# ariasanovsky/azdopt

Measured on AMD Instinct MI355X. Metric: node_expansions_per_s, higher is better.
Workload: dtype f32

## Files before the change

azdopt_amd/__init__.py:

```python
from ._lib import ACT_NONE, ACT_RELU, ACT_SIGMOID, AzdError, build, lib
from .model import ActionModel, HashStreamModel, NablaModel, TrivialModel
from .optimizer import ArgminData, DenseAhArgminData, DenseArgminData, DenseInvArgminData, DenseInvsArgminData, DenseInvxArgminData, NablaOptimizer, RamseyArgminData, TreeView, tree_capacities
from . import sinks
from .space import Layered
from .space import DenseGraphSpace, InvariantCost, InvariantCostS, InvariantCostX
from .space import ActionMultiset, ActionOrderIndependent, ActionSequence, ActionSet, OrderedActionSet, ActionsNeverRepeat, RamseySpaceNoEdgeRecolor, ROTModifyParentsOnce


def device_count():
    return lib().azd_device_count()
```

azdopt_amd/_lib.py:

```python
import ctypes as C
import os
import subprocess

_HERE = os.path.dirname(os.path.abspath(__file__))
LIB_PATH = os.environ.get("AZD_LIB", os.path.join(_HERE, "libazdopt_amd.so"))
_LIB = None

CTR = dict(EXPANSIONS=0, TERMINALS=1, TRANSPOSITIONS=2, VISITED_STEPS=3, SELECT_CALLS=4, SUM_DEG=5,
           SUM_ACTIONS=6, CASCADE_NODES=7, NEW_PREDS=8, ROOT_EXHAUSTED=9, MAX_FRONTIER=10, MAX_DEPTH=11,
           CURIOSITY_PAIRS=12, EVAL_LAYER_CLOCKS=13, TICKS_ADD_ACTIONS=14, FAILED=15, TICKS_TOTAL=16, TICKS_SELECT=17, TICKS_LOOKUP=18, TICKS_NEWNODE=19,
           TICKS_CASCADE=20, TICKS_MAX_CALL=21, TICKS_LAMBDA=22, TICKS_MATCHING=23, TICKS_WAIT=24, EVAL_BATCHES=25, EVAL_ROWS=26, EVAL_TILES=27, TICKS_TILES=28, TICKS_BATCH=29, TICKS_TILE_SETUP=30, TICKS_TILE_KLOOP=31)
CTR_COUNT = 32

ACT_NONE, ACT_RELU, ACT_SIGMOID = 0, 1, 2
ENGINE_NO_PERSISTENT_STEP = 1
ENGINE_ASYNC_STEP = 2
ENGINE_BARRIER_STEP = 4
ENGINE_POOL_STEP = 8
ENGINE_DENSE_AH = 32
ENGINE_RAMSEY_U64 = 16
ENGINE_EXT_POOL_STEP = 64
ENGINE_DENSE_AH_WIDE = 256
ENGINE_EXT_POOL_F32 = 128
ENGINE_DENSE_INV = 1024
# ... 192 lines not shown
    sig("azd_device_count", C.c_int)
    sig("azd_c21_state_dim", C.c_int, C.c_int)
    sig("azd_c21_action_dim", C.c_int, C.c_int)
    sig("azd_c21_key_words", C.c_int, C.c_int)
    sig("azd_c21_generate_roots", C.c_int, C.c_uint64, C.c_uint64, C.c_uint64, C.c_int, C.c_int, C.c_int, C.c_int, vp, vp)
    sig("azd_evaluator_create_mlp", C.c_int, C.POINTER(vp), C.c_int, C.c_int, C.c_int, C.c_int, vp, C.c_int, C.c_int,
        C.POINTER(AdamConfig), C.c_uint64)
    sig("azd_evaluator_create_trivial", C.c_int, C.POINTER(vp), C.c_int, C.c_int, C.c_int)
    sig("azd_evaluator_create_hash_stream", C.c_int, C.POINTER(vp), C.c_int, C.c_int, C.c_int, C.c_uint64, C.c_uint64)
    sig("azd_evaluator_destroy", C.c_int, vp)
    sig("azd_evaluator_write_predictions", C.c_int, vp, C.c_int, vp, vp)
    sig("azd_evaluator_update_model", C.c_int, vp, C.c_int, vp, vp, vp, f32p)
    sig("azd_evaluator_write_predictions_dev", C.c_int, vp, C.c_int, vp, vp, vp)
    sig("azd_evaluator_update_model_dev", C.c_int, vp, C.c_int, vp, vp, vp, f32p, vp)
    sig("azd_evaluator_set_weight_storage", C.c_int, vp, C.c_int)
    sig("azd_evaluator_num_params", C.c_int64, vp)
    sig("azd_evaluator_get_params", C.c_int, vp, vp)
    sig("azd_evaluator_set_params", C.c_int, vp, vp)
    sig("azd_evaluator_calls", C.c_uint64, vp)
    sig("azd_engine_create", C.c_int, C.POINTER(vp), C.POINTER(EngineConfig), vp)
    sig("azd_engine_destroy", C.c_int, vp)
    sig("azd_engine_par_new", C.c_int, vp, vp, vp)
    sig("azd_engine_par_roll_out_episodes", C.c_int, vp, vp, C.c_int, C.c_uint32, C.c_int, i32p)
    sig("azd_engine_run_ahead", C.c_int, vp, vp, C.c_int, C.c_uint32, C.c_int, i32p)
    sig("azd_engine_par_update_model", C.c_int, vp, C.c_uint32, f32p)
    sig("azd_engine_par_update_model_sharded", C.c_int, vp, C.c_uint32, vp, f32p)
    sig("azd_engine_par_reset_trees", C.c_int, vp, vp, vp)
    sig("azd_engine_argmin_data", C.c_int, vp, C.POINTER(Argmin))
    sig("azd_engine_agent_counters", C.c_int, vp, vp)
    sig("azd_engine_agent_counters_per_agent", C.c_int, vp)
    sig("azd_engine_pool_agent_finish", C.c_int, vp, vp)
    sig("azd_engine_pool_groups", C.c_int, vp, vp, vp, vp)
    sig("azd_engine_ramsey_argmin_data", C.c_int, vp, C.POINTER(RamseyArgmin))
    sig("azd_engine_ramsey_wide_argmin_data", C.c_int, vp, C.POINTER(RamseyWideArgmin))
    sig("azd_engine_ramsey_argmin_any", C.c_int, vp, vp, C.c_int, vp, C.c_int, vp, f32p, i32p, C.POINTER(C.c_uint32))
    sig("azd_engine_ramsey_agent_counts", C.c_int, vp, C.c_int, vp, vp)
    sig("azd_ramsey_state_dim", C.c_int, C.c_int, C.c_int)
    sig("azd_ramsey_action_dim", C.c_int, C.c_int, C.c_int)
    sig("azd_ramsey_key_words", C.c_int, C.c_int, C.c_int)
    sig("azd_ramsey_generate_roots", C.c_int, C.c_uint64, C.c_uint64, C.c_uint64, C.c_int, C.c_int, C.c_int, C.c_int,
        C.c_int, vp, vp)
    sig("azd_ramsey_generate_roots_weighted", C.c_int, C.c_uint64, C.c_uint64, C.c_uint64, C.c_int, C.c_int, C.c_int, C.c_int,
        C.c_int, vp, vp, vp)
    sig("azd_engine_set_root_policy", C.c_int, vp, C.POINTER(RootPolicy))
    sig("azd_engine_get_root_policy", C.c_int, vp, C.POINTER(RootPolicy))
    sig("azd_root_policy_check", C.c_int, C.c_int, C.c_int, C.POINTER(RootPolicy))
    sig("azd_engine_root_policy_report", C.c_int, vp, vp, vp, vp)
    sig("azd_dense_state_dim", C.c_int, C.c_int)
    sig("azd_dense_action_dim", C.c_int, C.c_int)
    sig("azd_dense_key_words", C.c_int, C.c_int)
    sig("azd_dense_generate_roots", C.c_int, C.c_uint64, C.c_uint64, C.c_uint64, C.c_int, C.c_int, C.c_int, C.c_int, C.c_double, vp, vp)
    sig("azd_engine_dense_argmin_data", C.c_int, vp, C.POINTER(DenseArgmin))
    sig("azd_c21_modify_roots", C.c_int, vp, C.c_uint64, C.c_uint64, C.c_int, C.c_int, vp, vp)
    sig("azd_c21_modify_roots_dev", C.c_int, vp, C.c_uint64, C.c_uint64, C.c_int, C.c_int, vp, vp)
    sig("azd_engine_par_reset_trees_c21", C.c_int, vp, C.c_uint64, C.c_uint64, C.c_int, C.c_int)
    sig("azd_engine_modify_roots_dev", C.c_int, vp, C.c_uint64, C.c_uint64, C.c_int, C.c_int, vp, vp)
    sig("azd_engine_par_reset_trees_policy", C.c_int, vp, C.c_uint64, C.c_uint64, C.c_int, C.c_int)
    sig("azd_engine_par_new_begin", C.c_int, vp, vp, vp)
    sig("azd_engine_par_new_end", C.c_int, vp, vp)
    sig("azd_engine_roll_out_begin", C.c_int, vp, vp, C.c_int, C.c_uint32)
    sig("azd_engine_roll_out_end", C.c_int, vp, vp, i32p)
    sig("azd_engine_reset_begin", C.c_int, vp, vp, vp)
    sig("azd_engine_reset_end", C.c_int, vp, vp)
    sig("azd_engine_observe", C.c_int, vp, C.c_uint32, vp, vp, vp)
    sig("azd_engine_observe_dev", C.c_int, vp, C.c_uint32, C.POINTER(vp), C.POINTER(vp), C.POINTER(vp))
    sig("azd_engine_read_state_vecs", C.c_int, vp, vp)
    sig("azd_engine_read_predictions", C.c_int, vp, vp)
    sig("azd_engine_debug_tile_forward", C.c_int, vp, vp, vp, C.c_int)
    sig("azd_engine_tree_sizes", C.c_int, vp, C.c_int, i32p, i32p, i32p)
    sig("azd_engine_export_tree", C.c_int, vp, C.c_int, *([vp] * 13))
    sig("azd_engine_agent_state", C.c_int, vp, C.c_int, vp, vp, vp, C.POINTER(C.c_uint32), C.POINTER(C.c_double), i32p)
    sig("azd_engine_counters", C.c_int, vp, vp)
    sig("azd_engine_set_timing", C.c_int, vp, C.c_int)
    sig("azd_engine_timing", C.c_int, vp, C.POINTER(C.c_double), C.POINTER(C.c_double), u64p)
    sig("azd_engine_stream", vp, vp)
    sig("azd_engine_step_form", C.c_int, vp, i32p, C.POINTER(C.c_char_p))
    sig("azd_engine_pool_split", C.c_int, vp, i32p, i32p)
    sig("azd_engine_pool_utilisation", C.c_int, vp, C.POINTER(C.c_double), C.POINTER(C.c_double))
    sig("azd_debug_probe_xcc", C.c_int, C.c_int, vp, C.c_int)
    sig("azd_debug_hash_stream_via_evaluators", C.c_int, vp, C.c_int)
    sig("azd_debug_ext_pool_plan", C.c_int, C.POINTER(EngineConfig), i32p, C.POINTER(C.c_size_t))
    sig("azd_debug_mlp_gradients", C.c_int, vp, C.c_int, vp, vp, vp, vp, f32p)
    sig("azd_debug_write_predictions_gathered", C.c_int, vp, C.c_int, vp, C.c_int, vp, C.c_int, vp)
    sig("azd_debug_probe_math", C.c_int, C.c_int, vp, vp, C.c_int)
    sig("azd_debug_gemm_bf16", C.c_int, C.c_int, C.c_int, C.c_int, C.c_int, vp, vp, vp, vp, C.c_int, C.c_int, C.c_int, C.c_int, f32p)
    sig("azd_debug_probe_cost", C.c_int, C.c_int, vp, C.c_int, C.c_int, C.c_int, C.c_int, vp, vp, f32p)
    sig("azd_debug_probe_dense_cost", C.c_int, C.c_int, vp, C.c_int, C.c_int, vp, C.c_int, vp, vp, vp, vp)
    sig("azd_dense_ah_cost", C.c_int, vp, C.c_int, C.POINTER(DenseAhCost))
    sig("azd_engine_dense_ah_argmin_data", C.c_int, vp, C.POINTER(DenseAhArgmin))
    sig("azd_engine_dense_ah_agent_cost", C.c_int, vp, C.c_int, C.POINTER(DenseAhCost))
    sig("azd_debug_probe_ah_cost", C.c_int, C.c_int, vp, C.c_int, C.c_int, C.c_int, vp, f32p)
    sig("azd_dense_ah_cost_wide", C.c_int, vp, C.c_int, C.POINTER(DenseAhCost))
    sig("azd_engine_dense_ah_wide_argmin_data", C.c_int, vp, C.POINTER(DenseAhWideArgmin))
    sig("azd_debug_probe_ah_cost_wide", C.c_int, C.c_int, vp, C.c_int, C.c_int, C.c_int, vp, f32p)
    sig("azd_dense_inv_cost", C.c_int, vp, C.c_int, C.POINTER(DenseInvRecipe), C.POINTER(DenseInvCost))
    sig("azd_debug_probe_inv_cost", C.c_int, C.c_int, vp, C.c_int, C.c_int, C.c_int, C.POINTER(DenseInvRecipe), vp, f32p)
    sig("azd_dense_inv_cost_wide", C.c_int, vp, C.c_int, C.POINTER(DenseInvRecipe), C.POINTER(DenseInvCost))
    sig("azd_debug_probe_inv_cost_wide", C.c_int, C.c_int, vp, C.c_int, C.c_int, C.c_int, C.POINTER(DenseInvRecipe), vp, f32p)
    sig("azd_engine_dense_inv_wide_argmin_data", C.c_int, vp, C.POINTER(DenseInvWideArgmin))
    sig("azd_dense_invx_cost", C.c_int, vp, C.c_int, C.POINTER(DenseInvxRecipe), C.POINTER(DenseInvxCost))
    sig("azd_debug_probe_invx_cost", C.c_int, C.c_int, vp, C.c_int, C.c_int, C.c_int, C.POINTER(DenseInvxRecipe), vp, f32p)
    sig("azd_dense_invx_cost_wide", C.c_int, vp, C.c_int, C.POINTER(DenseInvxRecipe), C.POINTER(DenseInvxCost))
    sig("azd_debug_probe_invx_cost_wide", C.c_int, C.c_int, vp, C.c_int, C.c_int, C.c_int, C.POINTER(DenseInvxRecipe), vp, f32p)
    sig("azd_engine_dense_invx_wide_argmin_data", C.c_int, vp, C.POINTER(DenseInvxWideArgmin))
    sig("azd_engine_set_dense_invx_recipe", C.c_int, vp, C.POINTER(DenseInvxRecipe))
    sig("azd_engine_dense_invx_argmin_data", C.c_int, vp, C.POINTER(DenseInvxArgmin))
    sig("azd_engine_dense_invx_agent_cost", C.c_int, vp, C.c_int, C.POINTER(DenseInvxCost))
    sig("azd_dense_invs_cost", C.c_int, vp, C.c_int, C.POINTER(DenseInvsRecipe), C.POINTER(DenseInvsCost))
    sig("azd_dense_invs_spectrum", C.c_int, vp, C.c_int, C.c_int, vp)
    sig("azd_debug_probe_invs_cost", C.c_int, C.c_int, vp, C.c_int, C.c_int, C.c_int, C.POINTER(DenseInvsRecipe), vp, f32p)
    sig("azd_dense_invs_cost_wide", C.c_int, vp, C.c_int, C.POINTER(DenseInvsRecipe), C.POINTER(DenseInvsCost))
    sig("azd_dense_invs_spectrum_wide", C.c_int, vp, C.c_int, C.c_int, vp)
    sig("azd_debug_probe_invs_cost_wide", C.c_int, C.c_int, vp, C.c_int, C.c_int, C.c_int, C.POINTER(DenseInvsRecipe), vp, f32p)
    sig("azd_engine_dense_invs_wide_argmin_data", C.c_int, vp, C.POINTER(DenseInvsWideArgmin))
    sig("azd_engine_set_dense_invs_recipe", C.c_int, vp, C.POINTER(DenseInvsRecipe))
    sig("azd_engine_dense_invs_argmin_data", C.c_int, vp, C.POINTER(DenseInvsArgmin))
    sig("azd_engine_dense_invs_agent_cost", C.c_int, vp, C.c_int, C.POINTER(DenseInvsCost))
    sig("azd_engine_set_dense_inv_recipe", C.c_int, vp, C.POINTER(DenseInvRecipe))
    sig("azd_engine_dense_inv_argmin_data", C.c_int, vp, C.POINTER(DenseInvArgmin))
    sig("azd_engine_dense_inv_agent_cost", C.c_int, vp, C.c_int, C.POINTER(DenseInvCost))
    sig("azd_debug_probe_math_f64", C.c_int, C.c_int, vp, vp, C.c_int)
    _LIB = L
    return L


def check(status, where):
    if status != 0:
        raise AzdError(status, where)


def ptr(a):
    return a.ctypes.data_as(C.c_void_p)
```

azdopt_amd/csrc/dense_kernels.hip:

```cpp
#include <hip/hip_runtime.h>

#include "bf16.h"
#include "space_ops.h"

namespace azd {

#include "tree_core.inc"
#include "space_dense.inc"

#include "root_policy.inc"

#define AZD_TU_POOL_EXT 1
#define AZD_TU_POOL_SEARCH 1
#include "persistent_step.inc"
#include "async_step.inc"
#include "pool_step.inc"

#include "launchers.inc"

AZD_PHASE_ENTRIES(DISPATCH_DKW)
AZD_DENSE_NO_RESIDENT_ENTRIES
#define DENSE_POOL_LDS "pool step: 16 searcher waves' blocks and scratch do not fit the CU's 160 KB of LDS (more than 640 slots per root)"
AZD_POOL_SEARCH_ENTRIES(DISPATCH_DKW, PERSIST_WAVES, "pool step: more than 65536 agents or nodes per tree", DENSE_POOL_LDS, DENSE_POOL_LDS)
const SpaceOps &dense_ops() {
    static const SpaceOps ops = {{AZD_PHASE_OPS, no_argmin_one, no_resident, nullptr}, {no_resident, nullptr}, {no_pool, nullptr, nullptr},
                                 {AZD_POOL_SEARCH_OPS(PERSIST_WAVES)}};
    return ops;
}

void launch_ext_take(const PoolArgs &pool, uint32_t *rows, uint32_t *home, uint32_t *n, unsigned long long *t0, void *stream) {
    k_ext_take<<<dim3(1), dim3(POOL_XCDS * 64), 0, (hipStream_t)stream>>>(pool, rows, home, n, t0);
}
__global__ void k_park(Arenas a, const uint32_t *__restrict__ resume, const int n_calls, const int round, const int park) {
    const int t = blockIdx.x * blockDim.x + threadIdx.x;
    if (t >= a.B) return;
    uint32_t f = a.flags[t] & ~(uint32_t)FLAG_PARKED;
    if (park) {
        const uint32_t r = resume[t];
        const bool sits_out = round < 0 ? (r >> 31) == 0u : (int)(r & 0x7FFFFFFFu) + round >= n_calls;
        if (sits_out) f |= (uint32_t)FLAG_PARKED;
    }
    a.flags[t] = f;
}
void launch_park(const Arenas &a, const uint32_t *resume, int n_calls, int round, int park, void *stream) {
    k_park<<<dim3((a.B + 255) / 256), dim3(256), 0, (hipStream_t)stream>>>(a, resume, n_calls, round, park);
}
__global__ void k_log_candidates_resume(Arenas a, unsigned long long *__restrict__ log_key, const uint32_t *__restrict__ resume, const int n_calls,
                                        const int round) {
    const int t = blockIdx.x * blockDim.x + threadIdx.x;
    if (t >= a.B) return;
    const uint32_t node = a.cand_node[t];
    const int call = (int)(resume[t] & 0x7FFFFFFFu) + round;
    if (node != NONE && a.flags[t] == 0 && call < n_calls) {
        const unsigned long long key = ((unsigned long long)ordf(a.cand_c[t]) << 32) | ((unsigned long long)((uint32_t)t & 0xFFFFu) << 16) |
                                       (unsigned long long)(node & 0xFFFFu);
        atomicMin(&log_key[call], key);
        a.cand_node[t] = NONE;
    }
}
void launch_log_candidates_resume(const Arenas &a, unsigned long long *log_key, const uint32_t *resume, int n_calls, int round, void *stream) {
    k_log_candidates_resume<<<dim3((a.B + 255) / 256), dim3(256), 0, (hipStream_t)stream>>>(a, log_key, resume, n_calls, round);
}
void launch_ext_hash_rows(const PersistArgs *d_args, const uint32_t *rows, const uint32_t *n, uint32_t cap, float *h_theta, void *stream) {
    k_ext_hash_rows<<<dim3(cap), dim3(256), 0, (hipStream_t)stream>>>(d_args, rows, n, h_theta);
}
void launch_ext_deliver(const PoolArgs &pool, const Arenas &a, const uint32_t *rows, const uint32_t *home, const uint32_t *n, uint32_t cap,
                        const unsigned long long *t0, void *stream) {
    k_ext_deliver<<<dim3((cap + 255) / 256), dim3(256), 0, (hipStream_t)stream>>>(pool, a, rows, home, n, t0);
}
void launch_probe_dense_cost(const uint64_t *d_adj, int n, int count, const uint16_t *d_toggles, int n_toggles, double *d_lam, int *d_mu,
                             uint8_t *d_mate, int *d_hooks, void *stream) {
    k_probe_dense_cost<2><<<dim3(count), dim3(64), 0, (hipStream_t)stream>>>(d_adj, n, count, d_toggles, n_toggles, d_lam, d_mu, d_mate, d_hooks);
}

}
```

azdopt_amd/csrc/engine.hip:

```cpp
#include "engine_impl.h"

namespace azd {
thread_local std::string g_last_error;

int hip_fail(hipError_t e, const char *what) {
    g_last_error = std::string(what) + ": " + hipGetErrorString(e);
    if (e == hipErrorNoDevice || e == hipErrorInvalidDevice) return AZD_ERR_NO_DEVICE;
    if (e == hipErrorOutOfMemory) return AZD_ERR_OUT_OF_MEMORY;
    return AZD_ERR_HIP;
}

int device_ok(int device) {
    int n = 0;
    hipError_t e = hipGetDeviceCount(&n);
    if (e != hipSuccess || n <= 0) {
        g_last_error = "no HIP device visible (this library has no CPU fallback)";
        return AZD_ERR_NO_DEVICE;
    }
    if (device < 0 || device >= n) {
        g_last_error = "device ordinal out of range";
        return AZD_ERR_INVALID_ARGUMENT;
    }
    return AZD_OK;
}
// ... 700 lines not shown
    if (dense) {
        e->dense_slots = 64 * a.KW;
        e->kw_host = azd::dense_key_words(cfg->n);
    } else if (ramsey) {
        e->kw_host = azd::ramsey_key_words(cfg->n, a.C);
        e->ramsey_slots = tier->cap_from_slots ? cfg->max_slots : azd::MAX_NODE_ACTIONS / (a.C - 1);
    }
    if (dense || (cfg->flags & AZD_ENGINE_EXT_POOL_STEP)) e->ext = tier->ext;
    e->ext_f32 = (cfg->flags & AZD_ENGINE_EXT_POOL_F32) != 0;
    if (ev && (ev->state_dim != a.S || ev->action_dim != a.A)) {
        azd::g_last_error = "evaluator dimensions do not match the space";
        return AZD_ERR_INVALID_ARGUMENT;
    }
    static_assert(AZD_RAMSEY_U64_NODE_ACTIONS == 64 * azd::RAMSEY_U64_CH, "node capacity of the 64-bit Ramsey tier");
    static_assert(AZD_DENSE_MAX_SLOTS <= 2047 && azd::MAX_NODE_ACTIONS <= 2047, "actions per node must fit PredRec's 11-bit count");
    static_assert(AZD_MAX_NODE_CAPACITY == 65536 && AZD_MAX_ARC_CAPACITY == 65535 && AZD_MAX_PREDICTION_CAPACITY == (1 << 20), "limits of the packed records");
    {
        const char *bad = nullptr;
        static thread_local char msg[256];
        const long per_node = dense ? (long)e->dense_slots : ramsey ? (long)std::min(a.E, e->ramsey_slots) * (a.C - 1) : (long)a.A;
        if (a.node_cap > (uint32_t)AZD_MAX_NODE_CAPACITY) snprintf(msg, sizeof msg, "node_capacity %u is beyond the record format (<= %d)", a.node_cap, AZD_MAX_NODE_CAPACITY), bad = msg;
        else if (a.arc_cap > (uint32_t)AZD_MAX_ARC_CAPACITY) snprintf(msg, sizeof msg, "arc_capacity %u is beyond the record format (<= %d)", a.arc_cap, AZD_MAX_ARC_CAPACITY), bad = msg;
        else if (a.pred_cap > (uint32_t)AZD_MAX_PREDICTION_CAPACITY) snprintf(msg, sizeof msg, "prediction_capacity %u is beyond the record format (<= %d)", a.pred_cap, AZD_MAX_PREDICTION_CAPACITY), bad = msg;
        else if (a.A > 4096) snprintf(msg, sizeof msg, "ACTION_DIM %d is beyond the record format (<= 4096)", a.A), bad = msg;
        else if (per_node > 2047) snprintf(msg, sizeof msg, "%ld legal actions per node are beyond the record format (<= 2047)", per_node), bad = msg;
        if (bad) {
            azd::g_last_error = bad;
            return AZD_ERR_INVALID_ARGUMENT;
        }
    }
    const size_t B = (size_t)a.B;
    AZD_ST(e->stream.create());
    AZD_ST(e->alloc(&a.nodes, B * a.node_cap));
    AZD_ST(e->alloc(&a.keys, B * a.node_cap * a.KW));
    AZD_ST(e->alloc(&a.arcs, B * a.arc_cap));
    AZD_ST(e->alloc(&a.preds, B * a.pred_cap));
    AZD_ST(e->alloc(&a.pred_g, B * a.pred_cap));
    AZD_ST(e->alloc(&a.ht, B * a.ht_cap));
    AZD_ST(e->alloc(&a.root_parents, B * azd::PARENTS_STRIDE));
    AZD_ST(e->alloc(&a.cur_parents, B * azd::PARENTS_STRIDE));
    AZD_ST(e->alloc(&a.root_perm, B * a.KW));
    AZD_ST(e->alloc(&a.cur_perm, B * a.KW));
    AZD_ST(e->alloc(&a.cur_path, B * a.KW));
    AZD_ST(e->alloc(&a.cur_lambda, (size_t)tier->cost_f64 * B + (size_t)tier->cost_tail_f64));
    AZD_ST(e->alloc(&a.cur_mu, (size_t)tier->cost_i32 * B));
    AZD_ST(e->alloc(&a.state_pos, B));
    AZD_ST(e->alloc(&a.n_nodes, B));
    AZD_ST(e->alloc(&a.n_arcs, B));
    AZD_ST(e->alloc(&a.n_preds, B));
    AZD_ST(e->alloc(&a.flags, B));
    a.fr_lds = (uint32_t)azd::FRONTIER_CAP;
    if (const char *v = getenv("AZD_DEBUG_FRONTIER_LDS")) {
        const int k = atoi(v);
        if (k >= 64 && k <= azd::FRONTIER_CAP && k % 64 == 0) a.fr_lds = (uint32_t)k;
    }
    if (ramsey) AZD_ST(e->alloc(&a.fr_spill, B * 4 * a.node_cap));
    AZD_ST(e->alloc(&a.cand_c, B));
    AZD_ST(e->alloc(&a.cand_node, B));
    AZD_ST(e->alloc(&a.counters, B * azd::NUM_COUNTERS));
    AZD_ST(e->alloc(&a.state_vecs, B * a.S));
    AZD_ST(e->alloc(&a.h_theta, B * a.A));
    a.obs = a.h_theta;
    AZD_ST(e->alloc(&a.weights, B * a.A));
    AZD_ST(e->alloc(&a.argmin, 1));
    AZD_ST(e->alloc(&a.status, 1));
    if (a.layers > 1) AZD_ST(e->alloc(&a.cur_seq, B * azd::MAX_NODE_ACTIONS));
    AZD_ST(e->alloc(&a.cur_stack, B * azd::PATH_STACK));
    if (dense) {
        AZD_ST(e->alloc(&a.root_adj, B * 64));
        AZD_ST(e->alloc(&a.cur_adj, B * 64));
        AZD_ST(e->alloc(&a.root_aid, B * (size_t)e->dense_slots));
        AZD_ST(e->alloc(&e->d_stage_slots, B * (size_t)((a.E + 63) / 64)));
        static_assert(sizeof(azd::DenseAhArgminRec) <= sizeof(azd::DenseArgminRec) && sizeof(azd::DenseAhWideArgminRec) <= sizeof(azd::DenseArgminRec) &&
                          sizeof(azd::DenseInvArgminRec) <= sizeof(azd::DenseArgminRec) && sizeof(azd::DenseInvWideArgminRec) <= 2 * sizeof(azd::DenseArgminRec) &&
                          sizeof(azd::DenseInvxArgminRec) <= sizeof(azd::DenseArgminRec) && sizeof(azd::DenseInvxWideArgminRec) <= 2 * sizeof(azd::DenseArgminRec) &&
                          sizeof(azd::DenseInvsArgminRec) <= sizeof(azd::DenseArgminRec) && sizeof(azd::DenseInvsWideArgminRec) <= 2 * sizeof(azd::DenseArgminRec),
                      "an AH or INV engine's argmin record lives in argmin_d's allocation");
        AZD_ST(e->alloc(&a.argmin_d, (tier->argmin_bytes + sizeof(azd::DenseArgminRec) - 1) / sizeof(azd::DenseArgminRec)));
        if (tier->id == TIER_DENSE) AZD_ST(e->alloc(&a.node_mate, B * (size_t)a.node_cap * 64));
        if (ev && ev->input16_pitch() >= a.S) {
            a.S16 = ev->input16_pitch();
            AZD_ST(e->alloc(&a.state_vecs16, B * (size_t)a.S16));
            if (hipMemset(a.state_vecs16, 0, B * (size_t)a.S16 * 2) != hipSuccess) return AZD_ERR_HIP;
        }
    }
    if (ramsey) {
        AZD_ST(e->alloc(&a.root_nbr, B * tier->nbr_words));
        AZD_ST(e->alloc(&a.cur_nbr, B * tier->nbr_words));
        AZD_ST(e->alloc(&a.root_counts, B * (size_t)a.C * a.E));
        AZD_ST(e->alloc(&a.cur_counts, B * (size_t)a.C * a.E));
        AZD_ST(e->alloc(&a.root_tot, B * 4));
        AZD_ST(e->alloc(&a.cur_tot, B * 4));
        AZD_ST(e->alloc(&a.argmin_r, e->argmin_r_recs()));
        if (e->ext && ev && ev->input16_pitch() >= a.S && ev->input16_pitch() % 8 == 0) {
            e->ext_s16_pitch = ev->input16_pitch();
            AZD_ST(e->alloc(&e->ext_s16, B * (size_t)e->ext_s16_pitch));
            if (hipMemset(e->ext_s16, 0, B * (size_t)e->ext_s16_pitch * 2) != hipSuccess) return AZD_ERR_HIP;
        }
    }
    e->persist_enabled = (cfg->flags & AZD_ENGINE_NO_PERSISTENT_STEP) == 0;
    e->barrier_step = (cfg->flags & AZD_ENGINE_BARRIER_STEP) != 0;
    e->graph_enabled = getenv("AZD_NO_CALL_GRAPH") == nullptr;
    e->pool_step = (cfg->flags & AZD_ENGINE_POOL_STEP) != 0 ||
                   ((cfg->flags & (AZD_ENGINE_ASYNC_STEP | AZD_ENGINE_BARRIER_STEP)) == 0 && cfg->batch >= 256);
    if (const char *env = getenv("AZD_STEP_FORM")) {
        if (!strcmp(env, "pool")) e->pool_step = true, e->barrier_step = false;
        else if (!strcmp(env, "async")) e->pool_step = false, e->barrier_step = false;
        else if (!strcmp(env, "barrier")) e->pool_step = false, e->barrier_step = true;
    }
    {
        hipDeviceProp_t prop;
        e->n_cus = hipGetDeviceProperties(&prop, cfg->device) == hipSuccess ? prop.multiProcessorCount : 256;
        uint32_t qcap = 128;
        while (qcap < 2u * (uint32_t)a.B) qcap <<= 1;
        e->pool.qcap = qcap;
        e->pool_slot_words = (size_t)4 * azd::POOL_XCDS * qcap;
        AZD_ST(e->alloc(&e->pool.ctl, 1));
        AZD_ST(e->alloc(&e->pool.ready_slots, e->pool_slot_words));
        e->pool.eval_slots = e->pool.ready_slots + (size_t)2 * azd::POOL_XCDS * qcap;
        AZD_ST(e->alloc(&e->pool.join, B));
        AZD_ST(e->alloc(&e->pool.pend, B));
        AZD_ST(e->alloc(&e->pool.stamp, B));
        AZD_ST(e->alloc(&e->pool.post_call, B));
        AZD_ST(e->alloc(&e->d_resume, B));
        AZD_ST(e->alloc(&e->d_call_ctr, (size_t)azd_engine::MAX_SUBS));
        if (e->ext) {
            AZD_ST(e->alloc(&e->d_ext_rows, B * azd_engine::EXT_STREAMS));
            AZD_ST(e->alloc(&e->d_ext_home, B * azd_engine::EXT_STREAMS));
            AZD_ST(e->alloc(&e->d_ext_n, (size_t)azd_engine::EXT_STREAMS));
            AZD_ST(e->alloc(&e->d_ext_t0, (size_t)azd_engine::EXT_STREAMS));
        }
    }
    e->log_calls = 1024;
    {
        const size_t n_wg = (B + 15) / 16;
        AZD_ST(e->alloc(&e->d_pargs, 1));
        AZD_ST(e->h_pargs.alloc(1));
        AZD_ST(e->alloc(&e->d_log_key, (size_t)e->log_calls * n_wg));
        AZD_ST(e->alloc(&e->d_log_node, (size_t)e->log_calls * n_wg));
        AZD_ST(e->alloc(&e->pool.win_count, (size_t)e->log_calls));
        AZD_ST(e->alloc(&e->d_argmin_side, 1));
        if (ramsey) AZD_ST(e->alloc(&e->d_argmin_r_side, e->argmin_r_recs()));
        AZD_ST(e->h_win_log.alloc((size_t)e->log_calls, hipHostMallocCoherent));
        AZD_ST(e->h_win_flag.alloc((size_t)e->log_calls, hipHostMallocCoherent));
        e->pool.win_log = e->h_win_log;
        e->pool.win_flag = e->h_win_flag;
    }
    AZD_ST(e->alloc(&e->d_stage_parents, B * (size_t)(dense ? 8 * a.n : ramsey ? a.E : a.n)));
    AZD_ST(e->alloc(&e->d_stage_perm, B * (size_t)(dense ? 17 * a.KW : a.KW)));
    if (!dense) e->d_stage_slots = e->d_stage_perm;
    AZD_ST(e->alloc(&e->d_root_report, B * 3));
    e->root_args.report = e->d_root_report;
    AZD_ST(e->h_status.alloc(1));
    AZD_ST(e->root_report.alloc(B * 3));
    AZD_ST(e->h_argmin.alloc(1));
    hipError_t he = hipMemsetAsync(a.counters, 0, B * azd::NUM_COUNTERS * 8, e->stream);
    if (he == hipSuccess) he = hipMemsetAsync(a.status, 0, sizeof(azd::StatusRec), e->stream);
    if (he == hipSuccess) he = hipMemsetAsync(a.argmin, 0, sizeof(azd::ArgminRec), e->stream);
    if (he == hipSuccess) he = hipMemsetAsync(a.flags, 0, B * 4, e->stream);
    if (he == hipSuccess) he = hipMemsetAsync(a.h_theta, 0, B * a.A * 4, e->stream);
    if (he == hipSuccess) he = hipMemsetAsync(a.state_vecs, 0, B * a.S * 4, e->stream);
    if (he == hipSuccess) he = hipMemsetAsync(a.weights, 0, B * a.A * 4, e->stream);
    if (he == hipSuccess && ramsey) he = hipMemsetAsync(a.argmin_r, 0, e->argmin_r_recs() * sizeof(azd::RamseyArgminRec), e->stream);
    if (he == hipSuccess && ramsey) he = hipMemsetAsync(e->d_argmin_r_side, 0, e->argmin_r_recs() * sizeof(azd::RamseyArgminRec), e->stream);
    if (he == hipSuccess) he = hipStreamSynchronize(e->stream);
    if (he != hipSuccess) return azd::hip_fail(he, "engine init memset");
// ... 195 lines not shown
```

azdopt_amd/csrc/engine_impl.h:

```cpp
#pragma once
#include <hip/hip_runtime.h>

#include <dlfcn.h>

#include <algorithm>
#include <climits>
#include <cstdio>
#include <cstring>
#include <functional>
#include <memory>
#include <new>
#include <string>
#include <vector>

#include "../../include/azdopt_amd.h"
#include "c21_host.h"
#include "engine_types.h"
#include "evaluator.h"
#include "space_ops.h"

struct ExtPoolForm {
    int waves_min, waves_knob_max;
    bool needs_pool_step;
    bool keep_quarter_free;
// ... 34 lines not shown
    std::vector<int16_t> tile_host;
    std::vector<uint32_t> lds_host;
    int ensure(hipStream_t stream, size_t want_slots, size_t want_x_floats, size_t want_flag_words) {
        if (!tile || !lds) {
            tile_host.clear(), lds_host.clear();
            AZD_ST(azd::alloc_set(tile, (size_t)8 * 128 * 4, lds, (size_t)8 * 128 * 4));
        }
        if (want_slots > slots || want_x_floats > x_floats || want_flag_words > flag_words) {
            AZD_HIP(hipStreamSynchronize(stream));
            slots = x_floats = flag_words = 0;
            AZD_ST(azd::alloc_set(desc, want_slots * 64, cnt, want_slots * 8 * 32, x, want_x_floats, flag, want_flag_words));
            slots = want_slots, x_floats = want_x_floats, flag_words = want_flag_words;
        }
        return AZD_OK;
    }
};

struct azd_engine {
    azd_engine_config cfg;
    azd::Arenas a;
    const azd::SpaceOps *ops = nullptr;
    const TierDesc *tier = nullptr;
    bool inv_recipe_set = false;
    azd::DenseInvRecipe inv_recipe{};
    azd::DenseInvxRecipe invx_recipe{};
    azd::DenseInvsRecipe invs_recipe{};
    bool inv_recipe_locked = false;
    azd_evaluator *ev = nullptr;
    azd::Stream stream;
    azd::DevArena allocs;
    uint8_t *d_stage_parents = nullptr;
    uint64_t *d_stage_perm = nullptr;
    azd::Pinned<azd::StatusRec> h_status;
    azd::Pinned<azd::ArgminRec> h_argmin;
    unsigned long long seen_improved = 0;
    bool timing = false;
    double rollout_ms = 0, evaluator_ms = 0;
    uint64_t rollout_launches = 0;
    std::vector<azd::Event> ev_pool;
    std::vector<std::pair<int, std::pair<azd::Event, azd::Event>>> ev_inflight;
    bool initialised = false;
    bool persist_enabled = true;
    bool barrier_step = false;
    azd::PersistArgs *d_pargs = nullptr;
    azd::Pinned<azd::PersistArgs> h_pargs;
    azd::PersistArgs pargs_sent{};
    bool pargs_valid = false;
    bool log_clean = false;
    bool pool_clean = false;
    bool pool_failed = false;
    bool counters_by_wave = false;
    uint32_t *d_resume = nullptr;
    EvalGroupMem grp;
    unsigned long long *d_log_key = nullptr;
    uint32_t *d_log_node = nullptr;
    int log_calls = 0;
    azd::GraphExec call_graph;
    azd::TolTable call_graph_tol{};
    uint64_t call_graph_layout = 0;
    bool graph_enabled = true;
    static constexpr int MAX_SUBS = 8;
    azd::Stream sub_stream[MAX_SUBS];
    azd::Event sub_fork, sub_join[MAX_SUBS];
    azd::GraphExec sub_graph[MAX_SUBS];
    int sub_graph_n = 0;
    uint32_t *d_call_ctr = nullptr;
    static constexpr int EXT_STREAMS = 2;
    static constexpr int EXT_IN_FLIGHT = 4;
    azd::Stream ext_stream[EXT_STREAMS];
    azd::GraphExec ext_graph[EXT_STREAMS];
    uint64_t ext_graph_layout = 0;
    int ext_graph_n = 0;
    bool ext_unsupported = false;
    bool ext_f32 = false;
    uint64_t ext_unsupported_layout = 0;
    uint32_t *d_ext_rows = nullptr, *d_ext_home = nullptr, *d_ext_n = nullptr;
    unsigned long long *d_ext_t0 = nullptr;
    int ext_depth = 2;
    azd::Event ext_done, ext_fork, ext_ring[EXT_STREAMS][EXT_IN_FLIGHT];
    unsigned long long ext_iterations = 0;
    const struct ExtPoolForm *ext = nullptr;
    uint16_t *ext_s16 = nullptr;
    int ext_s16_pitch = 0;
    int kw_host = 0;
    int ramsey_slots = 0;
    int dense_slots = 0;
    uint64_t *d_stage_slots = nullptr;
    azd_root_policy root_policy{AZD_ROOT_RULE_THRESHOLD, 0, {0.0, 0.0, 0.0, 0.0}};
    azd::RootPolicyArgs root_args{};
    uint32_t *d_root_report = nullptr;
    azd::Pinned<uint32_t> root_report;
    bool root_report_valid = false;
    std::vector<uint64_t> dense_packed;
    std::vector<uint64_t> ramsey_perm_pad;
    bool pool_step = false;
    azd::PoolArgs pool{};
    size_t pool_slot_words = 0;
    int n_cus = 0;
    int pool_eval_wgs = 0, pool_search_wgs = 0;
    int pool_grp_g = 0, pool_grp_groups = 0, pool_grp_w = 0;
    int pool_search_waves = 0;
    double pool_util_eval = 0, pool_util_search = 0;
    struct {
        int n_eval = 0;
        int updates = 0;
    } pool_fb;
    struct Window {
        bool open = false;
        bool drained = false;
        bool lumped = false;
        int n = 0, consumed = 0;
        azd::TolTable tol{};
        uint32_t best_ord = 0;
        unsigned long long best_key = ~0ull;
        unsigned long long side_key = ~0ull;
        unsigned long long base_improved = 0;
        unsigned long long reported = 0;
        azd::FusedEval fe{};
        azd::PoolArgs pool{};
    } win;
    azd::Pinned<unsigned long long> h_win_log;
    azd::Pinned<uint32_t> h_win_flag;
    azd::ArgminRec *d_argmin_side = nullptr;
    azd::RamseyArgminRec *d_argmin_r_side = nullptr;
    size_t argmin_r_recs() const { return (tier->argmin_bytes + sizeof(azd::RamseyArgminRec) - 1) / sizeof(azd::RamseyArgminRec); }
    azd::DevBuf<float> d_pool;
    size_t pool_rows = 0;
    int step_form = 0;
    std::string step_reason;

    ~azd_engine() {
        (void)hipSetDevice(cfg.device);
        for (const azd::Stream &s : sub_stream)
            if (s) (void)hipStreamSynchronize(s);
        for (const azd::Stream &s : ext_stream)
            if (s) (void)hipStreamSynchronize(s);
        if (stream) (void)hipStreamSynchronize(stream);
    }
    template <typename T>
    int alloc(T **p, size_t count) {
        return allocs.alloc(p, count);
    }
    azd::Event get_event() {
        azd::Event e;
        if (!ev_pool.empty()) {
            e = std::move(ev_pool.back());
            ev_pool.pop_back();
        } else (void)e.create();
        return e;
    }
    void time_begin(int kind) {
        if (!timing) return;
        azd::Event b = get_event(), en = get_event();
        (void)hipEventRecord(b, stream);
        ev_inflight.emplace_back(kind, std::make_pair(std::move(b), std::move(en)));
    }
    void time_end() {
        if (!timing) return;
        (void)hipEventRecord(ev_inflight.back().second.second, stream);
    }
    void time_collect() {
        for (auto &it : ev_inflight) {
            float ms = 0.f;
            (void)hipEventElapsedTime(&ms, it.second.first, it.second.second);
            if (it.first == 0) {
                rollout_ms += ms;
// ... 43 lines not shown
```

azdopt_amd/csrc/engine_probes.hip:

```cpp
#include "engine_impl.h"

template <class Cost, class Recipe, class Check, class Launch>
static int probe_dense_cost(const char *name, const char *tag, int device, const uint64_t *adj, int n, int count, int reps, const Recipe *recipe,
                            void *out, float *ms, Check check, Launch launch) {
    if (!out || count <= 0 || reps <= 0) {
        azd::g_last_error = std::string(name) + ": out / count / reps";
        return AZD_ERR_INVALID_ARGUMENT;
    }
    for (int i = 0; i < count; ++i)
        AZD_ST(check(adj ? adj + (size_t)i * (n > 0 ? n : 0) : nullptr, i));
    AZD_ST(azd::device_ok(device));
    AZD_HIP(hipSetDevice(device));
    azd::DevBuf<uint64_t> d_adj;
    azd::DevBuf<Cost> d_out;
    azd::DevBuf<Recipe> d_recipe;
    azd::Event e0, e1;
    AZD_ST(azd::alloc_set(d_adj, (size_t)count * n, d_out, (size_t)count, d_recipe, (size_t)(recipe ? 1 : 0)));
    AZD_ST(e0.create());
    AZD_ST(e1.create());
    AZD_HIP(hipMemcpy(d_adj, adj, (size_t)count * n * 8, hipMemcpyHostToDevice));
    if (recipe) {
        AZD_HIP(hipMemcpy(d_recipe, recipe, sizeof(Recipe), hipMemcpyHostToDevice));
    }
    launch(d_adj, n, count, 1, d_recipe, d_out, nullptr);
    AZD_HIP(hipEventRecord(e0, nullptr));
    launch(d_adj, n, count, reps, d_recipe, d_out, nullptr);
    AZD_HIP(hipEventRecord(e1, nullptr));
    hipError_t he = hipDeviceSynchronize();
    float t = 0.f;
    if (he == hipSuccess) he = hipEventElapsedTime(&t, e0, e1);
    if (he == hipSuccess) he = hipMemcpy(out, d_out, (size_t)count * sizeof(Cost), hipMemcpyDeviceToHost);
    if (he != hipSuccess) return azd::hip_fail(he, tag);
    if (ms) *ms = t;
    return AZD_OK;
}

extern "C" {

int azd_debug_mlp_gradients(azd_evaluator *ev, int batch, const float *states, const float *observations, const float *action_weights,
                            float *grads_out, float *loss) {
    if (!ev || batch <= 0 || !states || !observations || !action_weights || !grads_out) return AZD_ERR_INVALID_ARGUMENT;
    AZD_ST(ev->ensure_staging(batch));
    size_t sb = (size_t)batch * ev->state_dim * 4, pb = (size_t)batch * ev->action_dim * 4;
    AZD_HIP(hipMemcpyAsync(ev->d_states, states, sb, hipMemcpyHostToDevice, ev->own_stream));
    AZD_HIP(hipMemcpyAsync(ev->d_obs, observations, pb, hipMemcpyHostToDevice, ev->own_stream));
    AZD_HIP(hipMemcpyAsync(ev->d_w, action_weights, pb, hipMemcpyHostToDevice, ev->own_stream));
    return ev->debug_gradients(batch, ev->d_states, ev->d_obs, ev->d_w, grads_out, loss, ev->own_stream);
}
int azd_debug_write_predictions_gathered(azd_evaluator *ev, int max_rows, const uint32_t *rows, int n_rows, const float *states, int n_state_rows,
                                         float *predictions) {
    if (!ev || max_rows < 1 || n_rows < 0 || n_rows > max_rows || (n_rows > 0 && !rows) || !states || n_state_rows < 1 || !predictions)
        return AZD_ERR_INVALID_ARGUMENT;
    for (int i = 0; i < n_rows; ++i)
        if (rows[i] >= (uint32_t)n_state_rows) {
            azd::g_last_error = "azd_debug_write_predictions_gathered: a row index is not below n_state_rows";
            return AZD_ERR_INVALID_ARGUMENT;
        }
    return ev->debug_write_predictions_gathered(max_rows, rows, n_rows, states, n_state_rows, predictions);
}
int azd_debug_hash_stream_via_evaluators(azd_evaluator *ev, int on) { return ev ? ev->debug_serve_from_pool(on) : AZD_ERR_INVALID_ARGUMENT; }
int azd_engine_debug_tile_forward(azd_engine *e, const float *states, float *predictions, int rows) {
    if (!e || !states || !predictions || rows < 1) return AZD_ERR_INVALID_ARGUMENT;
    AZD_ENTER(e);
    azd::FusedEval fe;
    azd::PoolArgs pool = e->pool;
    uint32_t dyn_stride = 0;
    size_t dyn_bytes = 0;
    const char *why = "";
    if (e->a.space == azd::SPACE_DENSE || !e->ev->fused_desc(&fe) || fe.kind != 3 || !e->ops->pool_plan(e->a, fe, &pool, &dyn_stride, &dyn_bytes, &why)) {
        azd::g_last_error = "debug_tile_forward: needs the c21 or the Ramsey space with an MLP evaluator the pool step can serve";
        return AZD_ERR_INVALID_ARGUMENT;
    }
    azd::DevBuf<float> d_in, d_out;
    AZD_ST(azd::alloc_set(d_in, (size_t)rows * e->a.S, d_out, (size_t)rows * e->a.A));
    const char *what = "hipMemcpyAsync";
    hipError_t he = hipMemcpyAsync(d_in, states, (size_t)rows * e->a.S * 4, hipMemcpyHostToDevice, e->stream);
    if (he == hipSuccess) what = "k_tile_forward", he = azd::launch_tile_forward(fe, pool, rows, d_in, d_out, e->stream);
    if (he == hipSuccess) what = "hipMemcpyAsync", he = hipMemcpyAsync(predictions, d_out, (size_t)rows * e->a.A * 4, hipMemcpyDeviceToHost, e->stream);
    if (he == hipSuccess) what = "hipStreamSynchronize", he = hipStreamSynchronize(e->stream);
    else (void)hipStreamSynchronize(e->stream);
    return he == hipSuccess ? AZD_OK : azd::hip_fail(he, what);
}
int azd_debug_probe_xcc(int device, uint32_t *out, int n_blocks) {
    if (!out || n_blocks <= 0) return AZD_ERR_INVALID_ARGUMENT;
    AZD_ST(azd::device_ok(device));
    AZD_HIP(hipSetDevice(device));
    azd::DevBuf<uint32_t> d;
    AZD_ST(d.alloc((size_t)n_blocks));
    azd::launch_probe_xcc(d, n_blocks, nullptr);
    hipError_t he = hipDeviceSynchronize();
    if (he == hipSuccess) he = hipMemcpy(out, d, (size_t)n_blocks * 4, hipMemcpyDeviceToHost);
    if (he != hipSuccess) return azd::hip_fail(he, "probe_xcc");
    return AZD_OK;
}
int azd_debug_ext_pool_plan(const azd_engine_config *cfg, int *waves, size_t *lds_bytes) {
    if (!cfg || !waves || !lds_bytes) return AZD_ERR_INVALID_ARGUMENT;
    AZD_ST(check_engine_config(cfg));
    const bool ah_wide = (cfg->flags & (AZD_ENGINE_DENSE_AH_WIDE | AZD_ENGINE_DENSE_INV_WIDE | AZD_ENGINE_DENSE_INVX_WIDE | AZD_ENGINE_DENSE_INVS_WIDE)) != 0;
    const bool dense_f32 = cfg->space_id == AZD_SPACE_DENSE && (cfg->flags & AZD_ENGINE_EXT_POOL_F32) != 0;
    if (!(cfg->flags & AZD_ENGINE_EXT_POOL_STEP) && !ah_wide && !dense_f32) {
        azd::g_last_error = "azd_debug_ext_pool_plan: the configuration does not set AZD_ENGINE_EXT_POOL_STEP";
        return AZD_ERR_INVALID_ARGUMENT;
    }
    const TierDesc *const tier = engine_tier(cfg);
    azd::Arenas a;
    engine_shape(cfg, tier, &a);
    const azd::SpaceOps *ops = tier->ops;
    const ExtPoolForm *xf = tier->ext;
    if (!xf) {
        azd::g_last_error = "azd_debug_ext_pool_plan: the configuration's tier has no searcher-only pool step";
        return AZD_ERR_UNSUPPORTED;
    }
    const char *why = "";
    uint32_t dyn_stride = 0;
    size_t dyn_bytes = 0;
    int w = ops->waves_max;
    while (w > xf->waves_min && !ops->pool_search_plan(a, w, &dyn_stride, &dyn_bytes, &why)) w -= 1;
    if (!ops->pool_search_plan(a, w, &dyn_stride, &dyn_bytes, &why)) {
        azd::g_last_error = why;
        return AZD_ERR_UNSUPPORTED;
    }
    *waves = w;
    *lds_bytes = dyn_bytes + azd::POOL_SEARCH_STATIC_LDS;
    return AZD_OK;
}
int azd_debug_probe_math(int device, const float *in, float *out, int n) {
    if (!in || !out || n <= 0) return AZD_ERR_INVALID_ARGUMENT;
    AZD_ST(azd::device_ok(device));
    AZD_HIP(hipSetDevice(device));
    azd::DevBuf<float> d_in, d_out;
    AZD_ST(azd::alloc_set(d_in, (size_t)n * 2, d_out, (size_t)n * 4));
    AZD_HIP(hipMemcpy(d_in, in, (size_t)n * 8, hipMemcpyHostToDevice));
    azd::launch_probe_math(d_in, d_out, n, nullptr);
    hipError_t he = hipDeviceSynchronize();
    if (he == hipSuccess) he = hipMemcpy(out, d_out, (size_t)n * 16, hipMemcpyDeviceToHost);
    if (he != hipSuccess) return azd::hip_fail(he, "probe_math");
    return AZD_OK;
}

int azd_debug_probe_cost(int device, const uint8_t *parents, int n, int count, int reps, int full, double *lambda_1,
                         int *matching_size, float *ms) {
// ... 297 lines not shown
```

azdopt_amd/csrc/engine_rollout.hip:

```cpp
#include "engine_impl.h"

static uint32_t host_ordf(float f) {
    f = f + 0.0f;
    uint32_t u;
    memcpy(&u, &f, 4);
    return (u & 0x80000000u) ? ~u : (u | 0x80000000u);
}
static bool pool_feedback_on() { return knob_int("AZD_POOL_FEEDBACK", 1) != 0; }
static int fill_tol(TolTable &t, const uint32_t *tol, int n_tol, uint32_t dflt) {
    if (n_tol < 0 || n_tol > MAX_TOL || (n_tol > 0 && !tol)) return AZD_ERR_INVALID_ARGUMENT;
    for (int i = 0; i < MAX_TOL; ++i) t.tol[i] = i < n_tol ? tol[i] : dflt;
    t.n_tol = n_tol;
    t.tol_default = dflt;
    return AZD_OK;
}

extern "C" {

int azd_engine_roll_out_begin(azd_engine *e, const uint32_t *tol, int n_tol, uint32_t dflt) {
    if (!e || !e->initialised) return AZD_ERR_INVALID_ARGUMENT;
    AZD_ENTER(e);
    azd::TolTable t;
    AZD_ST(fill_tol(t, tol, n_tol, dflt));
    e->time_begin(0);
// ... 99 lines not shown
    e->log_clean = true;
    return AZD_OK;
}
static azd::StepLaunch step_launch(const azd_engine *e, int k, azd::PoolCtl *ctl, const uint32_t *resume, bool hashed, bool window = false, bool groups = false) {
    azd::StepLaunch sl;
    sl.n_calls = k;
    sl.log_key = e->d_log_key;
    sl.resume = resume;
    sl.ctl = ctl;
    sl.hashed = hashed ? 1 : 0;
    sl.window = window ? 1 : 0;
    sl.groups = groups ? 1 : 0;
    return sl;
}
static int capture_graph(hipStream_t stream, const std::function<int()> &body, azd::GraphExec *exec) {
    hipGraph_t g = nullptr;
    hipGraphExec_t x = nullptr;
    AZD_HIP(hipStreamBeginCapture(stream, hipStreamCaptureModeThreadLocal));
    const int st = body();
    const hipError_t he = hipStreamEndCapture(stream, &g);
    if (st) {
        if (g) (void)hipGraphDestroy(g);
        return st;
    }
    if (he != hipSuccess) return azd::hip_fail(he, "hipStreamEndCapture");
    const hipError_t hi = hipGraphInstantiate(&x, g, nullptr, nullptr, 0);
    (void)hipGraphDestroy(g);
    if (hi != hipSuccess) return azd::hip_fail(hi, "hipGraphInstantiate");
    exec->adopt(x);
    return AZD_OK;
}

static int pool_clear(azd_engine *e, const azd::PoolArgs &pool) {
    AZD_HIP(hipMemsetAsync(pool.ctl, 0, sizeof(azd::PoolCtl), e->stream));
    AZD_HIP(hipMemsetAsync(pool.ready_slots, 0, e->pool_slot_words * sizeof(uint32_t), e->stream));
    AZD_HIP(hipMemsetAsync(pool.join, 0, (size_t)e->a.B * sizeof(uint32_t), e->stream));
    e->pool_clean = true;
    return AZD_OK;
}

static int pool_finish_launch(azd_engine *e, const azd::FusedEval &fe, const azd::PoolArgs &pool, int k, bool *took_over,
                              uint32_t *as_out, size_t *ab_out) {
    *took_over = false;
    AZD_ST(fetch_status(e));
    if (e->h_status->pool_ticks > 0 && !e->h_status->pool_abort) {
        const double T = (double)e->h_status->pool_ticks;
        e->pool_util_eval = e->pool_eval_wgs > 0 ? (double)e->h_status->pool_eval_busy / (T * e->pool_eval_wgs) : 0.0;
        e->pool_util_search = e->pool_search_waves > 0 ? (double)e->h_status->pool_search_busy / (T * e->pool_search_waves) : 0.0;
    }
    if (!e->h_status->pool_abort) return AZD_OK;
    e->pool_clean = false;
    e->log_clean = false;
    e->pool_failed = true;
    e->pool_step = false;
    uint32_t as = 0;
    size_t ab = 0;
    const char *why_t = "";
    if (!e->ops->async_plan(e->a, fe, &as, &ab, &why_t)) {
        e->time_collect();
        azd::g_last_error = std::string("pool step: a queue wait ran into its bound, and the asynchronous step cannot take over: ") + why_t;
        return AZD_ERR_UNREACHABLE;
    }
    azd::launch_pool_resume_scan(e->a, pool, k, e->d_resume, e->stream);
    AZD_ST(pool_clear(e, pool));
    const azd::StepLaunch sl = step_launch(e, k, nullptr, e->d_resume, fe.kind == 4);
    e->time_begin(0);
    e->ops->launch_async(e->a, e->d_pargs, sl, fe.params, fe.wpk, as, ab, e->stream);
    e->time_end();
    e->log_clean = true;
    e->step_form = AZD_STEP_ASYNC;
    e->step_reason = "pool step aborted (a queue wait ran into its bound: no evaluator or searcher workgroup made progress); "
                     "the asynchronous step took the launch over and serves this engine from here on";
    *took_over = true;
    *as_out = as;
    *ab_out = ab;
    return AZD_OK;
}

struct ExtPlan {
    azd::Arenas a;
    azd::FusedEval fe;
    azd::PoolArgs pool;
    bool hashed, f32_rows;
    const char *r_needs_rows;
    int waves, n_search, n_ext;
    uint32_t dyn_stride;
    size_t dyn_bytes;
};
static int ext_plan(azd_engine *e, int n_calls, ExtPlan *out, bool *runs) {
    *runs = false;
    const ExtPoolForm &xf = *e->ext;
    azd::Arenas ax = e->a;
    if (e->ext_s16) {
        ax.state_vecs16 = e->ext_s16;
        ax.S16 = e->ext_s16_pitch;
    }
    const azd::Arenas &a = ax;
    const bool f32_rows = e->ext_f32;
    const char *const r_needs_rows = f32_rows ? xf.r_needs_rows : xf.r_needs_bf16;
    if (f32_rows && e->ext_unsupported && e->ext_unsupported_layout != e->ev->layout_version) e->ext_unsupported = false;
    const char *why = "";
    uint32_t dyn_stride = 0;
    size_t dyn_bytes = 0;
    int waves = knob_int(xf.env_waves, e->ops->waves_max);
    if (waves < xf.waves_min || waves > xf.waves_knob_max) {
        azd::g_last_error = xf.e_waves_range;
        return AZD_ERR_INVALID_ARGUMENT;
    }
    const bool knobs = getenv(xf.env_wgs) || getenv(xf.env_waves);
    auto pool_plan = e->ops->pool_search_plan;
    while (waves > xf.waves_min && !pool_plan(a, waves, &dyn_stride, &dyn_bytes, &why)) waves -= 1;
    azd::FusedEval fe;
    const bool hashed = e->ev->fused_desc(&fe) && fe.kind == 4;
    const bool configured = (e->pool_step || !xf.needs_pool_step) && e->persist_enabled;
    if (!configured || e->pool_failed || e->ext_unsupported || (!a.state_vecs16 && !hashed && !f32_rows) ||
        n_calls < 1 || !pool_plan(a, waves, &dyn_stride, &dyn_bytes, &why)) {
        e->step_reason = !configured       ? xf.r_not_configured
                         : e->pool_failed ? xf.r_failed_before
                         : ((!a.state_vecs16 && !hashed && !f32_rows) || e->ext_unsupported) ? r_needs_rows
                                                                                 : why;
        return AZD_OK;
    }
    const int per_cu = e->ops->pool_search_resident(a, waves, dyn_bytes);
    int n_search = (2 * a.B + waves - 1) / waves;
    if (n_search > e->n_cus * 8 / waves) n_search = e->n_cus * 8 / waves;
    if (xf.keep_quarter_free && n_search > e->n_cus - e->n_cus / 4) n_search = e->n_cus - e->n_cus / 4;
    n_search = knob_pos(xf.env_wgs, n_search);
    if (per_cu >= 1 && knobs && n_search > e->n_cus - e->n_cus / 4) {
        static thread_local char msg[256];
        snprintf(msg, sizeof msg, "%s / %s: %d searcher workgroups of %d waves would sit on %d of %d CUs; "
                 "the evaluator's GEMM launches need at least a quarter of the chip free (at most %d workgroups)", xf.env_wgs, xf.env_waves, n_search, waves,
                 n_search < e->n_cus ? n_search : e->n_cus, e->n_cus, e->n_cus - e->n_cus / 4);
        azd::g_last_error = msg;
        return AZD_ERR_INVALID_ARGUMENT;
    }
    if (per_cu < 1 || n_search > e->n_cus * per_cu * 7 / 8) n_search = per_cu < 1 ? 0 : e->n_cus * per_cu * 7 / 8;
    if (n_search < 1) {
        e->step_reason = xf.r_no_wg;
        return AZD_OK;
    }
    int n_ext = knob_int(xf.env_streams, xf.streams);
    n_ext = n_ext < 1 ? 1 : n_ext > azd_engine::EXT_STREAMS ? azd_engine::EXT_STREAMS : n_ext;
    azd::PoolArgs pool = e->pool;
    pool.n_eval = 0;
    pool.ready_lanes = 0;
    pool.n_express = 0;
    pool.express_waves = 0;
    pool.express_shift = 0;
    pool.early_post = knob_int("AZD_POOL_EARLY_POST", xf.early_post);
    pool.eval_stride = pool.eval_out_off = 0;
    pool.eval_rows = 0;
    pool.debug_abort_call = (uint32_t)knob_int("AZD_POOL_DEBUG_ABORT_CALL", 0);
    if (!hashed) {
        memset(&fe, 0, sizeof(fe));
        fe.kind = 3;
    }
    *out = ExtPlan{ax, fe, pool, hashed, f32_rows, r_needs_rows, waves, n_search, n_ext, dyn_stride, dyn_bytes};
    *runs = true;
    return AZD_OK;
}
static int ext_graphs(azd_engine *e, const ExtPlan &xp, bool *served) {
    *served = true;
    if (!xp.hashed) AZD_ST(e->ev->ensure_rows(xp.n_ext * xp.a.B));
    int rounds = knob_int(e->ext->env_rounds, 4);
    rounds = rounds < 1 ? 1 : rounds > 16 ? 16 : rounds;
    const uint64_t layout = e->ev->layout_version + (xp.hashed ? 1ull << 63 : 0ull) + ((uint64_t)rounds << 56);
    if (e->ext_graph_n != xp.n_ext || e->ext_graph_layout != layout) {
        for (azd::GraphExec &g : e->ext_graph) g.reset();
        e->ext_graph_n = 0;
        for (int x = 0; x < xp.n_ext; ++x) {
            uint32_t *rows = e->d_ext_rows + (size_t)x * xp.a.B, *home = e->d_ext_home + (size_t)x * xp.a.B, *cnt = e->d_ext_n + x;
            const int st_x = capture_graph(e->ext_stream[x], [&]() -> int {
                int st_g = AZD_OK;
                for (int r = 0; r < rounds && st_g == AZD_OK; ++r) {
                    azd::launch_ext_take(xp.pool, rows, home, cnt, e->d_ext_t0 + x, e->ext_stream[x]);
                    if (xp.hashed) azd::launch_ext_hash_rows(e->d_pargs, rows, cnt, (uint32_t)xp.a.B, xp.a.h_theta, e->ext_stream[x]);
                    else {
                        st_g = xp.a.state_vecs16 ? e->ev->write_predictions_gathered(rows, cnt, xp.a.B, xp.a.state_vecs16, xp.a.S16, xp.a.h_theta, e->ext_stream[x], x * xp.a.B)
                                              : AZD_ERR_UNSUPPORTED;
                        if (st_g == AZD_ERR_UNSUPPORTED && xp.f32_rows)
                            st_g = e->ev->write_predictions_gathered_f32(rows, cnt, xp.a.B, xp.a.state_vecs, xp.a.S, xp.a.h_theta, e->ext_stream[x], x * xp.a.B);
                    }
                    azd::launch_ext_deliver(xp.pool, xp.a, rows, home, cnt, (uint32_t)xp.a.B, e->d_ext_t0 + x, e->ext_stream[x]);
                }
                return st_g;
            }, &e->ext_graph[x]);
            if (st_x == AZD_ERR_UNSUPPORTED) {
                e->ext_unsupported = true;
                e->ext_unsupported_layout = e->ev->layout_version;
                e->step_reason = xp.r_needs_rows;
                *served = false;
                return AZD_OK;
            }
            if (st_x) return st_x;
        }
        e->ext_graph_n = xp.n_ext;
        e->ext_graph_layout = layout;
    }
    return AZD_OK;
}
static int ext_recover(azd_engine *e, const azd::TolTable &t, const ExtPlan &xp, int k) {
    const azd::Arenas &a = e->a;
    e->pool_failed = true;
    e->log_clean = false;
    azd::launch_pool_resume_scan(a, xp.pool, k, e->d_resume, e->stream);
    std::vector<uint32_t> res((size_t)a.B);
    AZD_HIP(hipMemcpyAsync(res.data(), e->d_resume, res.size() * 4, hipMemcpyDeviceToHost, e->stream));
    AZD_HIP(hipStreamSynchronize(e->stream));
    AZD_ST(pool_clear(e, xp.pool));
    int rounds = 0;
    bool any_pending = false;
    for (uint32_t r : res) {
        const int rem = k - (int)(r & 0x7FFFFFFFu);
        rounds = rem > rounds ? rem : rounds;
        any_pending = any_pending || (r >> 31) != 0u;
    }
    auto evaluate_rows = [&]() -> int {
        if (xp.hashed) {
            azd::g_last_error = e->ext->e_abort_hashed;
            return AZD_ERR_UNREACHABLE;
        }
        const uint64_t calls_before = e->ev->calls;
        const int s2 = e->ev->write_predictions_dev16(a.B, a.state_vecs, a.state_vecs16, a.S16, a.h_theta, e->stream);
        e->ev->calls = calls_before;
        return s2;
    };
    if (any_pending) {
        azd::launch_park(a, e->d_resume, k, -1, 1, e->stream);
        AZD_ST(evaluate_rows());
        e->ops->add_actions(a, 0, e->stream);
    }
    for (int r = 0; r < rounds; ++r) {
        azd::launch_park(a, e->d_resume, k, r, 1, e->stream);
        e->ops->rollout(a, t, e->stream);
        AZD_ST(evaluate_rows());
        e->ops->add_actions(a, 0, e->stream);
        azd::launch_log_candidates_resume(a, e->d_log_key, e->d_resume, k, r, e->stream);
    }
    azd::launch_park(a, e->d_resume, k, 0, 0, e->stream);
    e->ops->argmin_log(a, k, e->d_log_key, e->stream);
    e->log_clean = true;
    AZD_HIP(hipGetLastError());
    AZD_ST(fetch_status(e));
    e->step_form = AZD_STEP_PER_CALL;
    e->step_reason = e->ext->r_aborted;
    return AZD_OK;
}
static int ext_run_launches(azd_engine *e, const azd::TolTable &t, int n_calls, const ExtPlan &xp, int *left_out) {
    const ExtPoolForm &xf = *e->ext;
    int depth = knob_int(xf.env_depth, e->ext_depth);
    depth = depth < 1 ? 1 : depth > azd_engine::EXT_IN_FLIGHT ? azd_engine::EXT_IN_FLIGHT : depth;
    int left = n_calls;
    while (left > 0) {
        const int k = left < e->log_calls ? left : e->log_calls;
        AZD_ST(send_pargs(e, xp.a, t, xp.fe, xp.pool));
        AZD_ST(pool_clear(e, xp.pool));
        AZD_ST(ensure_log_clean(e));
        AZD_HIP(hipMemsetAsync(e->d_ext_n, 0, sizeof(uint32_t) * azd_engine::EXT_STREAMS, e->stream));
        AZD_HIP(hipEventRecord(e->ext_fork, e->stream));
        for (int x = 0; x < xp.n_ext; ++x) AZD_HIP(hipStreamWaitEvent(e->ext_stream[x], e->ext_fork, 0));
        const azd::StepLaunch sl = step_launch(e, k, xp.pool.ctl, nullptr, xp.hashed);
        e->time_begin(0);
        e->ops->launch_pool_search(xp.a, e->d_pargs, sl, xp.n_search, xp.waves, xp.dyn_stride, xp.dyn_bytes, e->stream);
#ifndef AZD_PHASE_PROFILE
        e->counters_by_wave = true;
#endif
        e->time_end();
        AZD_HIP(hipGetLastError());
        AZD_HIP(hipEventRecord(e->ext_done, e->stream));
        e->pool_clean = false;
        unsigned long long it = 0;
        for (;;) {
            const hipError_t q = hipEventQuery(e->ext_done);
            if (q == hipSuccess) break;
            if (q != hipErrorNotReady) return azd::hip_fail(q, "hipEventQuery");
            const int x = (int)(it % (unsigned long long)xp.n_ext);
            const unsigned long long round = it / (unsigned long long)xp.n_ext;
            hipEvent_t slot = e->ext_ring[x][round % (unsigned long long)depth];
            if (round >= (unsigned long long)depth) AZD_HIP(hipEventSynchronize(slot));
            AZD_HIP(hipGraphLaunch(e->ext_graph[x], e->ext_stream[x]));
            AZD_HIP(hipEventRecord(slot, e->ext_stream[x]));
            it += 1;
        }
        for (int x = 0; x < xp.n_ext; ++x) AZD_HIP(hipStreamSynchronize(e->ext_stream[x]));
        e->ext_iterations += it;
        if (getenv(xf.env_debug)) fprintf(stderr, "%s: %d calls, %d searcher workgroups, %llu evaluator replays\n", xf.debug_tag, k, xp.n_search, it);
        left -= k;
        e->ev->calls += (uint64_t)k;
        AZD_ST(fetch_status(e));
        if (e->h_status->pool_ticks > 0) {
            const double T = (double)e->h_status->pool_ticks;
            e->pool_util_eval = (double)e->h_status->pool_eval_busy / (T * xp.n_ext);
            e->pool_util_search = (double)e->h_status->pool_search_busy / (T * e->pool_search_waves);
        }
        if (e->h_status->pool_abort) {
            *left_out = left;
            return ext_recover(e, t, xp, k);
        }
    }
    return AZD_OK;
}
static int ext_pool_run(azd_engine *e, const azd::TolTable &t, int n_calls, bool *ran, int *left_out) {
    *ran = false;
    *left_out = 0;
    ExtPlan xp;
    bool go = false;
    int st = ext_plan(e, n_calls, &xp, &go);
    if (st || !go) return st;
    if (!e->ext_done) AZD_ST(e->ext_done.create(hipEventDisableTiming));
    if (!e->ext_fork) AZD_ST(e->ext_fork.create(hipEventDisableTiming));
    for (int x = 0; x < xp.n_ext; ++x) {
        if (!e->ext_stream[x]) AZD_ST(e->ext_stream[x].create(hipStreamNonBlocking));
        for (int i = 0; i < azd_engine::EXT_IN_FLIGHT; ++i)
            if (!e->ext_ring[x][i]) AZD_ST(e->ext_ring[x][i].create(hipEventDisableTiming));
    }
    st = ext_graphs(e, xp, &go);
    if (st || !go) return st;
    e->step_form = AZD_STEP_POOL;
    e->step_reason.clear();
    e->pool_eval_wgs = 0;
    e->pool_search_wgs = xp.n_search;
    e->pool_search_waves = xp.n_search * xp.waves;
    e->ext_iterations = 0;
    AZD_ST(ext_run_launches(e, t, n_calls, xp, left_out));
    *ran = true;
    return AZD_OK;
}
struct PoolKnobs { int eval_wgs, search_wgs, ready_lanes, express_wgs, express_waves, express_shift, early_post; };
static int pool_split(int n_cus, const azd::Arenas &a, const azd::FusedEval &fe, int n_calls, int capacity, int fb_n_eval, const PoolKnobs &k, azd::PoolArgs *pool) {
    const int B = a.B;
    int cap = 0;
    auto clamp_eval = [&](int v) {
        const int want_search = (B + 7) / 8;
        const int most = want_search < n_cus / 2 ? n_cus - want_search : n_cus / 2;
        v = v > cap ? cap : v;
        v = v > most ? most : v;
        return v < 1 ? 1 : v;
    };
    int n_eval = 0;
    if (fe.kind >= 3) {
        double flop = 0;
        if (fe.kind == 3)
            for (int l = 0; l < fe.n_layers; ++l) flop += 2.0 * fe.dims[l] * fe.dims[l + 1];
        else flop = 2.0 * 256.0 * (a.S + 512.0 + a.A);
        const double eval_us_per_row = flop / (256.0 * 2400.0) / (fe.bf16 ? 1.85 : 1.0) / 0.33;
        const double search_us_per_call = a.space == azd::SPACE_RAMSEY ? 3.6 : 3.65;
        n_eval = (int)(n_cus * eval_us_per_row / (eval_us_per_row + search_us_per_call) + 0.5);
        if (pool->eval_rows > 16 && B >= 6144) n_eval = (int)(n_eval * 0.91 + 0.5);
        cap = (B + 3) / 4 + 1;
        n_eval = clamp_eval(n_eval);
        if (fb_n_eval > 0) n_eval = clamp_eval(fb_n_eval);
        if (n_calls <= 64 && fe.kind == 3) n_eval = clamp_eval(n_eval + n_eval / 7);
        if (k.eval_wgs > 0) n_eval = k.eval_wgs;
    }
    int n_search = n_cus - n_eval;
    const int want = (B + 7) / 8;
    n_search = n_search > want ? want : n_search;
    n_search = n_search < 1 ? 1 : n_search;
    if (k.search_wgs > 0) n_search = k.search_wgs;
    if (fe.kind < 3) n_eval = 0;
    if (n_eval + n_search > capacity) {
        if (n_eval > capacity / 2) n_eval = capacity / 2;
        if (fe.kind >= 3 && n_eval < 1) n_eval = 1;
        n_search = capacity - n_eval;
    }
    pool->n_eval = n_eval;
    pool->ready_lanes = k.ready_lanes;
// ... 465 lines not shown
```

azdopt_amd/csrc/engine_types.h:

```cpp
#pragma once
#include <stddef.h>
#include <stdint.h>

namespace azd {

constexpr uint32_t NONE = 0xFFFFFFFFu;
constexpr int PARENTS_STRIDE = 32;
constexpr int MAX_N = 24;
constexpr int MAX_KW = 6;
constexpr int PATH_SET = 0, PATH_SEQUENCE = 1;
constexpr int SPACE_C21 = 1, SPACE_RAMSEY = 2, SPACE_DENSE = 3;
constexpr int PRED_CHUNKS = 2;
constexpr int MAX_NODE_ACTIONS = 64 * PRED_CHUNKS;
constexpr int RAMSEY_U64_KW = 36;
constexpr int RAMSEY_U64_CH = 8;
constexpr int FRONTIER_CAP = 256;
constexpr int PATH_STACK = 32;
constexpr int MAX_TOL = 32;
constexpr int NUM_COUNTERS = 32;

struct __attribute__((aligned(16))) NodeRec {
    float c_star;
    uint32_t nt_ex;
    float c;
// ... 163 lines not shown
struct DenseInvsArgminRec {
    uint64_t adj[32];
    uint64_t permitted[8];
    double inv[21];
    int32_t dist_k;
    uint32_t computed;
    float cost, eval;
    int32_t agent;
    uint32_t node;
};
struct DenseInvsWideArgminRec {
    uint64_t adj[64];
    uint64_t permitted[32];
    double inv[21];
    int32_t dist_k;
    uint32_t computed;
    float cost, eval;
    int32_t agent;
    uint32_t node;
};
static_assert(sizeof(DenseInvxWideArgminRec) == 920 && sizeof(DenseInvsWideArgminRec) == 960,
              "the largest dense argmin records: argmin_d is sized from the tier's argmin_bytes");

struct StatusRec {
    unsigned long long improved;
    unsigned long long expansions;
    unsigned long long failed;
    unsigned long long pool_abort;
    unsigned long long pool_eval_busy, pool_search_busy, pool_ticks, pool_pad;
};

struct Arenas {
    NodeRec *nodes;
    uint64_t *keys;
    ArcRec *arcs;
    PredRec *preds;
    float *pred_g;
    uint32_t *ht;
    uint32_t node_cap, arc_cap, pred_cap, ht_cap;
    uint8_t *root_parents;
    uint64_t *root_perm;
    uint8_t *cur_parents;
    uint64_t *cur_perm;
    uint64_t *cur_path;
    double *cur_lambda;
    int32_t *cur_mu;
    uint32_t *state_pos;
    uint32_t *n_nodes, *n_arcs, *n_preds;
    uint32_t *flags;
    uint32_t fr_lds;
    uint32_t *fr_spill;
    float *cand_c;
    uint32_t *cand_node;
    unsigned long long *counters;
    float *state_vecs;
    uint16_t *state_vecs16;
    int S16;
    float *h_theta;
    float *obs;
    float *weights;
    ArgminRec *argmin;
    StatusRec *status;
    int n, A, S, KW, B;
    int t0, tn;
    float eval_slope;
    double lam_lo, lam_hi;
    int space;
    int C, E;
    int sizes[4];
    float cweights[4];
    uint32_t *root_nbr, *cur_nbr;
    int32_t *root_counts, *cur_counts;
    int32_t *root_tot, *cur_tot;
    RamseyArgminRec *argmin_r;
    uint64_t *root_adj, *cur_adj;
    uint16_t *root_aid;
    uint32_t dense_p24;
    DenseArgminRec *argmin_d;
    uint8_t *node_mate;
    int path_kind;
    int layers, S_inner;
    uint16_t *cur_seq;
    uint32_t *cur_stack;
};

constexpr int ROOT_RULE_THRESHOLD = 0, ROOT_RULE_BEST = 1;
constexpr int ROOT_BRANCH_FRESH = 0, ROOT_BRANCH_STAGNANT = 1, ROOT_BRANCH_IMPROVED = 2;
struct RootPolicyArgs {
    int rule;
    int weighted;
    uint64_t color_thr[3];
    uint32_t *report;
};

struct FusedEval {
    int kind;
    uint64_t seed, first_agent, call_base;
    const float *params;
    int n_layers;
    int dims[8];
    int final_act;
    int max_hidden;
    int hid[2];
    long long w_off[7], b_off[7];
    int bf16;
    const uint16_t *w16;
    const void *wpk;
    long long p_off[7];
};

struct TolTable {
    uint32_t tol[MAX_TOL];
    int n_tol;
    uint32_t tol_default;
};

constexpr int POOL_XCDS = 8;
struct PoolQ {
    uint32_t head, pad0[31];
    uint32_t tail, pad1[31];
};
struct PoolCtl {
    uint32_t claim_next, pad0[31];
    uint32_t done_agents, pad1[31];
    uint32_t abort, pad2[31];
    PoolQ ready[2][POOL_XCDS];
    PoolQ evalq[2][POOL_XCDS];
    struct {
        uint32_t v, pad[31];
    } sum_calls[POOL_XCDS], claimed[POOL_XCDS],
      done_x[POOL_XCDS],
      max_lag[POOL_XCDS];
    unsigned long long eval_busy;
    unsigned long long search_busy;
    unsigned long long t_first;
    unsigned long long t_last;
};
struct PendRec {
    uint32_t pos;
    float c;
    uint32_t n_preds;
    uint32_t call;
};
struct PoolArgs {
    PoolCtl *ctl;
    uint32_t *ready_slots;
    uint32_t *eval_slots;
    int ready_lanes;
    int n_express;
    uint32_t express_waves;
    uint32_t express_shift;
    int early_post;
    uint32_t qcap;
    uint32_t *join;
    PendRec *pend;
    unsigned long long *stamp;
    int n_eval;
    uint32_t eval_stride;
    uint32_t eval_out_off;
    uint32_t eval_rows;
    uint32_t *post_call;
    int grp_g, grp_w, grp_groups;
    const int16_t *grp_tile;
    const uint32_t *grp_lds;
    uint32_t *grp_desc;
    uint32_t *grp_cnt;
// ... 28 lines not shown
```

azdopt_amd/csrc/evaluator.h:

```cpp
#pragma once
#include <hip/hip_runtime.h>
#include <stdint.h>

#include <string>

#include "../../include/azdopt_amd.h"
#include "engine_types.h"
#include "hip_own.h"

struct azd_evaluator {
    int device = 0;
    int state_dim = 0;
    int action_dim = 0;
    uint64_t calls = 0;
    uint64_t layout_version = 0;
    azd::DevBuf<float> d_states, d_preds, d_obs, d_w;
    int staged_batch = 0;
    azd::Stream own_stream;

    virtual ~azd_evaluator() = default;
    virtual int write_predictions_dev(int batch, const float *d_s, float *d_p, hipStream_t st) = 0;
    virtual int update_model_dev(int batch, const float *d_s, const float *d_o, const float *d_w, float *loss,
                                 hipStream_t st) = 0;
    virtual int write_predictions_dev16(int batch, const float *d_s, const uint16_t * , int , float *d_p, hipStream_t st) {
        return write_predictions_dev(batch, d_s, d_p, st);
    }
    virtual int input16_pitch() { return 0; }
    virtual int write_predictions_rows(int row0, int count, const float *d_s, const uint16_t *d_s16, int pitch16, float *d_p, hipStream_t st) {
        return write_predictions_dev16(count, d_s + (size_t)row0 * state_dim, d_s16 ? d_s16 + (size_t)row0 * pitch16 : nullptr, pitch16,
                                       d_p + (size_t)row0 * action_dim, st);
    }
    virtual bool rows_concurrent() { return false; }
    virtual int ensure_rows(int ) { return AZD_OK; }
    virtual int write_predictions_gathered(const uint32_t * , const uint32_t * , int , const uint16_t * ,
                                           int , float * , hipStream_t , int  = 0) {
        return AZD_ERR_UNSUPPORTED;
    }
    virtual int write_predictions_gathered_f32(const uint32_t * , const uint32_t * , int , const float * ,
                                               int , float * , hipStream_t , int  = 0) {
        return AZD_ERR_UNSUPPORTED;
    }
    virtual int debug_write_predictions_gathered(int , const uint32_t * , int , const float * ,
                                                 int , float * ) {
        return AZD_ERR_UNSUPPORTED;
    }
    virtual bool fused_desc(azd::FusedEval *) { return false; }
    virtual bool replayable(int ) { return false; }
    virtual int64_t num_params() { return 0; }
    virtual int get_params(float *) { return AZD_ERR_UNSUPPORTED; }
    virtual int set_params(const float *) { return AZD_ERR_UNSUPPORTED; }
    virtual int set_weight_storage(int) { return AZD_ERR_UNSUPPORTED; }
    virtual int debug_serve_from_pool(int) { return AZD_ERR_UNSUPPORTED; }
    virtual int debug_gradients(int, const float *, const float *, const float *, float *, float *, hipStream_t) { return AZD_ERR_UNSUPPORTED; }
    int ensure_staging(int batch);
};

namespace azd {
azd_evaluator *make_mlp_evaluator(int device, int max_batch, int state_dim, int action_dim, const int *hidden,
                                  int n_hidden, int final_act, const azd_adam_config *adam, uint64_t seed, int *status);
}
```

azdopt_amd/csrc/mlp_kernels.hip:

```cpp
#include <hip/hip_runtime.h>

#include <cmath>
#include <cstring>
#include <new>
#include <vector>

#include "c21_host.h"
#include "bf16.h"
#include "evaluator.h"

namespace azd {

typedef float f32x16 __attribute__((ext_vector_type(16)));

constexpr int BM = 64, BN = 64, BK = 16;
constexpr int LDS_LD = BM + 4;

enum { EPI_NONE = 0, EPI_BIAS_ACT = 1, EPI_RELU_MASK = 2, EPI_BIAS_ACT_BF16 = 3 };

template <bool A_KC, bool B_KC>
__global__ __launch_bounds__(256) void k_gemm(const float *__restrict__ A, int lda, const float *__restrict__ B, int ldb,
                                              float *__restrict__ C, int ldc, int M, int N, int K_all, int epi, int act,
                                              const float *__restrict__ bias, const float *__restrict__ aux, int ldaux,
                                              int k_split, size_t c_split_stride) {
// ... 130 lines not shown
    const float *xa = X + (size_t)(m0 + arow) * ldx + akof;
    const uint16_t *wb = W + (size_t)(n0 + srow) * ldw + skof;
    const bool a_ok = m0 + arow < M, b_ok = n0 + srow < N;
    float4 ra[AQ];
    uint2 rb[4];
    auto fetch = [&](int k0) {
#pragma unroll
        for (int q = 0; q < AQ; ++q)
            ra[q] = (a_ok && k0 + akof + 4 * q < K) ? *reinterpret_cast<const float4 *>(xa + k0 + 4 * q) : make_float4(0.f, 0.f, 0.f, 0.f);
#pragma unroll
        for (int q = 0; q < 4; ++q)
            rb[q] = (b_ok && k0 + skof + 4 * q < K) ? *reinterpret_cast<const uint2 *>(wb + k0 + 4 * q) : make_uint2(0u, 0u);
    };
    auto stash = [&]() {
        uint32_t pa[2 * AQ];
#pragma unroll
        for (int q = 0; q < AQ; ++q) {
            pa[2 * q] = bf16_bits(ra[q].x) | (bf16_bits(ra[q].y) << 16);
            pa[2 * q + 1] = bf16_bits(ra[q].z) | (bf16_bits(ra[q].w) << 16);
        }
        uint4 *da = reinterpret_cast<uint4 *>(sA + arow * GB_LD + akof);
#pragma unroll
        for (int q = 0; q < AQ / 2; ++q) da[q] = make_uint4(pa[4 * q], pa[4 * q + 1], pa[4 * q + 2], pa[4 * q + 3]);
        uint4 *db = reinterpret_cast<uint4 *>(sB + srow * GB_LD + skof);
        db[0] = make_uint4(rb[0].x, rb[0].y, rb[1].x, rb[1].y);
        db[1] = make_uint4(rb[2].x, rb[2].y, rb[3].x, rb[3].y);
    };
    f32x16 acc[MI][2];
#pragma unroll
    for (int i = 0; i < MI; ++i)
#pragma unroll
        for (int j = 0; j < 2; ++j)
#pragma unroll
            for (int r = 0; r < 16; ++r) acc[i][j][r] = 0.f;
    fetch(0);
    for (int k0 = 0; k0 < K; k0 += GB_K) {
        stash();
        __syncthreads();
        if (k0 + GB_K < K) fetch(k0 + GB_K);
        const int fr = lane & 31, fh = (lane >> 5) * 8;
#pragma unroll
        for (int ks = 0; ks < GB_K; ks += 16) {
            bf16x8_t fa[MI], fb[2];
#pragma unroll
            for (int i = 0; i < MI; ++i) {
                const uint4 va = *reinterpret_cast<const uint4 *>(sA + (wm * 32 * MI + i * 32 + fr) * GB_LD + ks + fh);
                __builtin_memcpy(&fa[i], &va, 16);
            }
#pragma unroll
            for (int j = 0; j < 2; ++j) {
                const uint4 vb = *reinterpret_cast<const uint4 *>(sB + (wn * 64 + j * 32 + fr) * GB_LD + ks + fh);
                __builtin_memcpy(&fb[j], &vb, 16);
            }
#pragma unroll
            for (int i = 0; i < MI; ++i)
#pragma unroll
                for (int j = 0; j < 2; ++j) acc[i][j] = __builtin_amdgcn_mfma_f32_32x32x16_bf16(fa[i], fb[j], acc[i][j], 0, 0, 0);
        }
        __syncthreads();
    }
#pragma unroll
    for (int j = 0; j < 2; ++j) {
        const int col = n0 + wn * 64 + j * 32 + (lane & 31);
        if (col >= N) continue;
        const float bj = bias ? bias[col] : 0.f;
#pragma unroll
        for (int i = 0; i < MI; ++i)
#pragma unroll
            for (int r = 0; r < 16; ++r) {
                const int row = m0 + wm * 32 * MI + i * 32 + (r & 3) + 8 * (r >> 2) + 4 * (lane >> 5);
                if (row < M) {
                    float v = acc[i][j][r] + bj;
                    if (act == AZD_ACT_RELU) v = v > 0.f ? v : 0.f;
                    else if (act == AZD_ACT_SIGMOID) v = 1.0f / (1.0f + expf(-v));
                    if (round_out) v = bf16_round(v);
                    Y[(size_t)row * ldy + col] = v;
                }
            }
    }
}

#include "gemm_bf16_glds.inc"
#include "gemm_bf16_hidden2.inc"
#include "gemm_f32_gathered.inc"

__global__ void k_quantize_bf16(const float *__restrict__ p, size_t n, uint16_t *__restrict__ w16, float *__restrict__ q) {
    size_t i = (size_t)blockIdx.x * blockDim.x + threadIdx.x;
    if (i >= n) return;
    const uint32_t b = bf16_bits(p[i]);
    w16[i] = (uint16_t)b;
    q[i] = __uint_as_float(b << 16);
}
__global__ void k_pack_weights(const float *__restrict__ W, int K, int N, float *__restrict__ dst32, uint16_t *__restrict__ dst16) {
    const int steps = (K + 15) >> 4, tiles = (N + 15) >> 4;
    const size_t n = (size_t)tiles * steps * 256;
    const size_t e = (size_t)blockIdx.x * blockDim.x + threadIdx.x;
    if (e >= n) return;
    const int i = (int)(e & 3), lane = (int)((e >> 2) & 63);
    const size_t js = e >> 8;
    const int s = (int)(js % (size_t)steps), j = (int)(js / (size_t)steps);
    const int row = 16 * j + (lane & 15), k = 16 * s + 4 * (lane >> 4) + i;
    const float v = (row < N && k < K) ? W[(size_t)row * K + k] : 0.f;
    if (dst16) dst16[e] = (uint16_t)bf16_bits(v);
    else dst32[e] = v;
}
__global__ void k_round_bf16(const float *__restrict__ in, size_t n, float *__restrict__ out) {
    size_t i = (size_t)blockIdx.x * blockDim.x + threadIdx.x;
    if (i < n) out[i] = bf16_round(in[i]);
}

__global__ void k_block_sum(const float *__restrict__ x, size_t n, float *__restrict__ partial) {
    __shared__ float s[256];
    float acc = 0.f;
    for (size_t i = (size_t)blockIdx.x * blockDim.x + threadIdx.x; i < n; i += (size_t)gridDim.x * blockDim.x) acc += x[i];
    s[threadIdx.x] = acc;
    __syncthreads();
    for (int off = 128; off > 0; off >>= 1) {
        if ((int)threadIdx.x < off) s[threadIdx.x] += s[threadIdx.x + off];
        __syncthreads();
    }
    if (threadIdx.x == 0) partial[blockIdx.x] = s[0];
}
__global__ void k_final_sum(const float *__restrict__ partial, int n, float *__restrict__ out) {
    __shared__ float s[256];
    float acc = 0.f;
    for (int i = threadIdx.x; i < n; i += blockDim.x) acc += partial[i];
    s[threadIdx.x] = acc;
    __syncthreads();
    for (int off = 128; off > 0; off >>= 1) {
        if ((int)threadIdx.x < off) s[threadIdx.x] += s[threadIdx.x + off];
        __syncthreads();
    }
    if (threadIdx.x == 0) *out = s[0];
}
__global__ void k_loss_delta(const float *__restrict__ pred, const float *__restrict__ obs, const float *__restrict__ w,
                             const float *__restrict__ wsum, size_t n, int act, float *__restrict__ delta,
                             float *__restrict__ partial) {
    __shared__ float s[256];
    const float ws = *wsum;
    float acc = 0.f;
    for (size_t i = (size_t)blockIdx.x * blockDim.x + threadIdx.x; i < n; i += (size_t)gridDim.x * blockDim.x) {
        float wt = w[i] / ws;
        float p = pred[i];
        float d = p - obs[i];
        acc += wt * d * d;
        float dp = 2.0f * wt * d;
        if (act == AZD_ACT_SIGMOID) dp *= p * (1.0f - p);
        else if (act == AZD_ACT_RELU) dp = p > 0.f ? dp : 0.f;
        delta[i] = dp;
    }
    s[threadIdx.x] = acc;
    __syncthreads();
    for (int off = 128; off > 0; off >>= 1) {
        if ((int)threadIdx.x < off) s[threadIdx.x] += s[threadIdx.x + off];
        __syncthreads();
    }
    if (threadIdx.x == 0) partial[blockIdx.x] = s[0];
}
__global__ __launch_bounds__(1024) void k_col_sum(const float *__restrict__ dz, int M, int N, float *__restrict__ out, int rows_per) {
    __shared__ float s[16][65];
    const int tx = threadIdx.x & 63, ty = threadIdx.x >> 6;
    const int j = blockIdx.x * 64 + tx;
    const int r0 = (int)blockIdx.y * rows_per;
    const int r1 = (r0 + rows_per < M) ? r0 + rows_per : M;
    out += (size_t)blockIdx.y * N;
    float acc = 0.f;
// ... 151 lines not shown
                l += 1;
                continue;
            }
            void *y = last ? (void *)d_p : (void *)(d_act16[(size_t)l + 1] + (size_t)act_row0 * kp[(size_t)l + 1]);
            launch_gemm16(st, x16, kp[(size_t)l], d_w16p + wp_off[(size_t)l], kp[(size_t)l], y, last ? dims[(size_t)L] : kp[(size_t)l + 1], batch,
                          dims[(size_t)l + 1], kp[(size_t)l], last ? final_act : AZD_ACT_RELU, last ? 0 : 1, d_params + b_off[(size_t)l], n_cus, 0,
                          (!last && d_part) ? d_part + (size_t)act_row0 * kp[(size_t)l + 1] : nullptr, part_stride);
            if (!last) x16 = d_act16[(size_t)l + 1] + (size_t)act_row0 * kp[(size_t)l + 1];
        }
        AZD_HIP(hipGetLastError());
        return AZD_OK;
    }
    int forward(int batch, const float *d_s, float *d_p, hipStream_t st, bool quant = false) {
        const float *x = d_s;
        const float *P = quant ? d_params_q : d_params;
        if (quant && d_w16p && !getenv("AZD_GEMM_OLD")) return forward16(batch, d_s, nullptr, d_p, st);
        bool mfma16 = quant;
        for (int l = 0; l < L && mfma16; ++l) mfma16 = dims[(size_t)l] % 4 == 0 && w_off[(size_t)l] % 4 == 0;
        if (mfma16) {
            for (int l = 0; l < L; ++l) {
                float *y = (l == L - 1) ? d_p : d_act[(size_t)l + 1];
                const int K = dims[(size_t)l], N = dims[(size_t)l + 1];
                const int nb = (N + GB_N - 1) / GB_N;
                const bool small = (size_t)nb * ((batch + 127) / 128) < (size_t)gemm_small_below;
                if (small)
                    k_gemm_bf16<1><<<dim3(nb, (batch + 63) / 64), dim3(256), 0, st>>>(x, K, d_w16 + w_off[(size_t)l], K, y, N, batch, N, K,
                                                                                     (l == L - 1) ? final_act : AZD_ACT_RELU, l < L - 1 ? 1 : 0,
                                                                                     d_params + b_off[(size_t)l]);
                else
                    k_gemm_bf16<2><<<dim3(nb, (batch + 127) / 128), dim3(256), 0, st>>>(x, K, d_w16 + w_off[(size_t)l], K, y, N, batch, N, K,
                                                                                       (l == L - 1) ? final_act : AZD_ACT_RELU, l < L - 1 ? 1 : 0,
                                                                                       d_params + b_off[(size_t)l]);
                x = y;
            }
            AZD_HIP(hipGetLastError());
            return AZD_OK;
        }
        if (quant) {
            const size_t n = (size_t)batch * dims[0];
            k_round_bf16<<<(unsigned)((n + 255) / 256), 256, 0, st>>>(d_s, n, d_xq);
            x = d_xq;
        }
        for (int l = 0; l < L; ++l) {
            float *y = (l == L - 1) ? d_p : d_act[(size_t)l + 1];
            int act = (l == L - 1) ? final_act : AZD_ACT_RELU;
            const int epi = (quant && l < L - 1) ? EPI_BIAS_ACT_BF16 : EPI_BIAS_ACT;
            gemm<true, true>(st, x, dims[(size_t)l], P + w_off[(size_t)l], dims[(size_t)l], y, dims[(size_t)l + 1], batch,
                             dims[(size_t)l + 1], dims[(size_t)l], epi, act, d_params + b_off[(size_t)l], nullptr, 0);
            x = y;
        }
        AZD_HIP(hipGetLastError());
        return AZD_OK;
    }

    int write_predictions_dev(int batch, const float *d_s, float *d_p, hipStream_t st) override {
        AZD_HIP(hipSetDevice(device));
        int s = ensure_batch(batch);
        if (s) return s;
        calls += 1;
        return forward(batch, d_s, d_p, st, bf16);
    }

    int write_predictions_dev16(int batch, const float *d_s, const uint16_t *d_s16, int pitch16, float *d_p, hipStream_t st) override {
        if (!bf16 || !d_w16p || !d_s16 || pitch16 != kp[0] || getenv("AZD_GEMM_OLD")) return write_predictions_dev(batch, d_s, d_p, st);
        AZD_HIP(hipSetDevice(device));
        int s = ensure_batch(batch);
        if (s) return s;
        calls += 1;
        return forward16(batch, d_s, d_s16, d_p, st);
    }
    int input16_pitch() override { return (bf16 && d_w16p) ? kp[0] : 0; }
    int write_predictions_rows(int row0, int count, const float *d_s, const uint16_t *d_s16, int pitch16, float *d_p, hipStream_t st) override {
        if (!rows_concurrent() || row0 + count > cap_batch) return azd_evaluator::write_predictions_rows(row0, count, d_s, d_s16, pitch16, d_p, st);
        AZD_HIP(hipSetDevice(device));
        const uint16_t *x16 = (d_s16 && pitch16 == kp[0]) ? d_s16 + (size_t)row0 * pitch16 : nullptr;
        return forward16(count, d_s + (size_t)row0 * state_dim, x16, d_p + (size_t)row0 * action_dim, st, row0);
    }
    bool rows_concurrent() override { return bf16 && d_w16p && !getenv("AZD_GEMM_OLD"); }
    int ensure_rows(int rows) override {
        AZD_HIP(hipSetDevice(device));
        return ensure_batch(rows);
    }
    int write_predictions_gathered(const uint32_t *d_rows, const uint32_t *d_count, int max_rows, const uint16_t *d_s16, int pitch16, float *d_p,
                                   hipStream_t st, int act_row0) override {
        if (!rows_concurrent() || !d_s16 || pitch16 != kp[0]) return AZD_ERR_UNSUPPORTED;
        if (act_row0 + max_rows > cap_batch) return AZD_ERR_CAPACITY;
        AZD_HIP(hipSetDevice(device));
        const uint16_t *x16 = d_s16;
        for (int l = 0; l < L; ++l) {
            const bool last = l == L - 1;
            if (hidden_pair(l)) {
                uint16_t *y2 = d_act16[(size_t)l + 2] + (size_t)act_row0 * HF_H;
                launch_hidden2<true>(st, x16, HF_H, d_w16p + wp_off[(size_t)l], d_w16p + wp_off[(size_t)l + 1], HF_H, d_params + b_off[(size_t)l],
                                     d_params + b_off[(size_t)l + 1], y2, HF_H, max_rows, d_count);
                x16 = y2;
                l += 1;
                continue;
            }
            void *y = last ? (void *)d_p : (void *)(d_act16[(size_t)l + 1] + (size_t)act_row0 * kp[(size_t)l + 1]);
            launch_gemm16_ext(st, x16, kp[(size_t)l], d_w16p + wp_off[(size_t)l], kp[(size_t)l], y, last ? dims[(size_t)L] : kp[(size_t)l + 1], max_rows,
                              dims[(size_t)l + 1], kp[(size_t)l], last ? final_act : AZD_ACT_RELU, last ? 0 : 1, d_params + b_off[(size_t)l], n_cus, d_count,
                              l == 0 ? d_rows : nullptr, last ? d_rows : nullptr,
                              (!last && d_part) ? d_part + (size_t)act_row0 * kp[(size_t)l + 1] : nullptr, part_stride);
            if (!last) x16 = d_act16[(size_t)l + 1] + (size_t)act_row0 * kp[(size_t)l + 1];
        }
        AZD_HIP(hipGetLastError());
        return AZD_OK;
    }

    int write_predictions_gathered_f32(const uint32_t *d_rows, const uint32_t *d_count, int max_rows, const float *d_s, int pitch, float *d_p,
                                       hipStream_t st, int act_row0) override {
        if (bf16) return AZD_ERR_UNSUPPORTED;
        if (!d_s || !d_p || max_rows < 1 || act_row0 < 0 || pitch < dims[0]) return AZD_ERR_INVALID_ARGUMENT;
        if (act_row0 + max_rows > cap_batch) return AZD_ERR_CAPACITY;
        AZD_HIP(hipSetDevice(device));
        const float *x = d_s;
        int ldx = pitch;
        for (int l = 0; l < L; ++l) {
            const bool last = l == L - 1;
            const int N = dims[(size_t)l + 1];
            float *y = last ? d_p : d_act[(size_t)l + 1] + (size_t)act_row0 * N;
            launch_gemm_f32_gathered(st, x, ldx, d_params + w_off[(size_t)l], dims[(size_t)l], y, N, max_rows, N, dims[(size_t)l], last ? final_act : AZD_ACT_RELU,
                                     d_params + b_off[(size_t)l], d_count, l == 0 ? d_rows : nullptr, last ? d_rows : nullptr);
            x = y;
            ldx = N;
        }
        AZD_HIP(hipGetLastError());
        return AZD_OK;
    }
    int debug_write_predictions_gathered(int max_rows, const uint32_t *rows, int n_rows, const float *states, int n_state_rows, float *predictions) override {
        AZD_HIP(hipSetDevice(device));
        int s = ensure_batch(max_rows);
        if (s) return s;
        const size_t sb = (size_t)n_state_rows * dims[0] * 4, pb = (size_t)n_state_rows * dims[(size_t)L] * 4;
        DevBuf<float> d_s, d_p;
        DevBuf<uint32_t> d_r;
        DevBuf<uint16_t> d_s16;
        const uint32_t count = (uint32_t)n_rows;
        AZD_ST(alloc_set(d_s, sb / 4, d_p, pb / 4, d_r, (size_t)max_rows + 1));
        hipError_t he = hipMemcpy(d_s, states, sb, hipMemcpyHostToDevice);
        if (he == hipSuccess) he = hipMemcpy(d_p, predictions, pb, hipMemcpyHostToDevice);
        if (he == hipSuccess && n_rows > 0) he = hipMemcpy(d_r, rows, (size_t)n_rows * 4, hipMemcpyHostToDevice);
        if (he == hipSuccess) he = hipMemcpy(d_r + max_rows, &count, 4, hipMemcpyHostToDevice);
        if (he != hipSuccess) return hip_fail(he, "azd_debug_write_predictions_gathered: staging");
        if (bf16) {
            AZD_ST(d_s16.alloc((size_t)n_state_rows * kp[0]));
            const size_t n = (size_t)n_state_rows * (kp[0] / 4);
            k_rows_to_bf16<<<(unsigned)((n + 255) / 256), 256, 0, nullptr>>>(d_s, dims[0], n_state_rows, dims[0], d_s16, kp[0]);
        }
        s = bf16 ? write_predictions_gathered(d_r, d_r + max_rows, max_rows, d_s16, kp[0], d_p, nullptr, 0)
                 : write_predictions_gathered_f32(d_r, d_r + max_rows, max_rows, d_s, dims[0], d_p, nullptr, 0);
        if (s == AZD_OK) {
            he = hipDeviceSynchronize();
            if (he == hipSuccess) he = hipMemcpy(predictions, d_p, pb, hipMemcpyDeviceToHost);
            if (he != hipSuccess) s = hip_fail(he, "azd_debug_write_predictions_gathered");
        }
        return s;
    }

    int update_model_dev(int batch, const float *d_s, const float *d_o, const float *d_w, float *loss, hipStream_t st) override {
        AZD_HIP(hipSetDevice(device));
        int s = gradients(batch, d_s, d_o, d_w, st);
        if (s) return s;
        return adam_step(loss, st);
    }
    int gradients(int batch, const float *d_s, const float *d_o, const float *d_w, hipStream_t st) {
        int s = ensure_batch(batch);
        if (s) return s;
        s = forward(batch, d_s, d_pred_train, st);
        if (s) return s;
        const int A = dims[(size_t)L];
        const size_t n = (size_t)batch * A;
        const int nb = 256;
        k_block_sum<<<nb, 256, 0, st>>>(d_w, n, d_partial);
        k_final_sum<<<1, 256, 0, st>>>(d_partial, nb, d_scalars);
        k_loss_delta<<<nb, 256, 0, st>>>(d_pred_train, d_o, d_w, d_scalars, n, final_act, d_delta_a, d_partial);
        k_final_sum<<<1, 256, 0, st>>>(d_partial, nb, d_scalars + 1);
        float *dz = d_delta_a, *dx = d_delta_b;
        for (int l = L - 1; l >= 0; --l) {
            const int in = dims[(size_t)l], out = dims[(size_t)l + 1];
            const float *x = (l == 0) ? d_s : d_act[(size_t)l];
            gemm_dw(st, dz, out, x, in, d_grads + w_off[(size_t)l], batch, d_split, MAX_SPLITS);
            {
                int parts = (batch + GEMM_SPLIT_K - 1) / GEMM_SPLIT_K;
                parts = parts > MAX_SPLITS ? MAX_SPLITS : parts;
                if (parts <= 1) k_col_sum<<<(out + 63) / 64, 1024, 0, st>>>(dz, batch, out, d_grads + b_off[(size_t)l], batch);
                else {
                    const int rows_per = (batch + parts - 1) / parts;
                    parts = (batch + rows_per - 1) / rows_per;
                    k_col_sum<<<dim3((out + 63) / 64, parts), 1024, 0, st>>>(dz, batch, out, d_split, rows_per);
                    k_sum_splits<<<(out + 255) / 256, 256, 0, st>>>(d_split, (size_t)out, parts, d_grads + b_off[(size_t)l]);
                }
            }
            if (l > 0) {
                gemm<true, false>(st, dz, out, d_params + w_off[(size_t)l], in, dx, in, batch, in, out, EPI_RELU_MASK, 0, nullptr, x, in);
                float *tmp = dz;
                dz = dx;
                dx = tmp;
            }
        }
        AZD_HIP(hipGetLastError());
        return AZD_OK;
    }
    int adam_step(float *loss, hipStream_t st) {
        t += 1;
        float bc1 = 1.0f - std::pow(adam.beta1, (float)t), bc2 = 1.0f - std::pow(adam.beta2, (float)t);
        k_adam<<<(unsigned)((n_params + 255) / 256), 256, 0, st>>>(d_params, d_grads, d_m, d_v, (size_t)n_params, adam.lr, adam.beta1,
                                                                  adam.beta2, adam.eps, adam.l2, bc1, bc2);
        if (bf16) requantize(st);
        repack(st);
        AZD_HIP(hipGetLastError());
        AZD_HIP(hipMemcpyAsync(h_scalars, d_scalars, 2 * sizeof(float), hipMemcpyDeviceToHost, st));
        AZD_HIP(hipStreamSynchronize(st));
        if (loss) *loss = h_scalars[1];
        return AZD_OK;
    }
    int debug_gradients(int batch, const float *d_s, const float *d_o, const float *d_w, float *grads_out, float *loss, hipStream_t st) override {
        AZD_HIP(hipSetDevice(device));
        int s = gradients(batch, d_s, d_o, d_w, st);
        if (s) return s;
        AZD_HIP(hipMemcpyAsync(grads_out, d_grads, (size_t)n_params * 4, hipMemcpyDeviceToHost, st));
        AZD_HIP(hipMemcpyAsync(h_scalars, d_scalars, 2 * sizeof(float), hipMemcpyDeviceToHost, st));
        AZD_HIP(hipStreamSynchronize(st));
        if (loss) *loss = h_scalars[1];
        return AZD_OK;
    }

    bool replayable(int batch) override { return batch <= cap_batch; }
    bool fused_desc(FusedEval *f) override {
        memset(f, 0, sizeof(*f));
        if (L > 7) return false;
        f->kind = 3;
        f->params = d_params;
// ... 90 lines not shown
static int mlp_init(MlpEvaluator *m, uint64_t seed) {
    AZD_HIP(hipSetDevice(m->device));
    const size_t np = (size_t)m->n_params;
    AZD_ST(alloc_set(m->d_params, np, m->d_grads, np, m->d_m, np, m->d_v, np, m->d_partial, 256, m->d_scalars, 4, m->h_scalars, 4));
    AZD_HIP(hipMemset(m->d_grads, 0, (size_t)m->n_params * 4));
    AZD_HIP(hipMemset(m->d_m, 0, (size_t)m->n_params * 4));
    AZD_HIP(hipMemset(m->d_v, 0, (size_t)m->n_params * 4));
    std::vector<float> h((size_t)m->n_params);
    for (int l = 0; l < m->L; ++l) {
        int in = m->dims[(size_t)l], out = m->dims[(size_t)l + 1];
        float bound = 1.0f / std::sqrt((float)in);
        for (int64_t i = 0; i < (int64_t)in * out; ++i) {
            uint64_t r = stream_key(seed, 0x6d6c7057ull, (uint64_t)l, (uint64_t)i);
            float u = (float)(r >> 40) * (1.0f / 16777216.0f);
            h[(size_t)(m->w_off[(size_t)l] + i)] = (2.0f * u - 1.0f) * bound;
        }
        for (int i = 0; i < out; ++i) {
            uint64_t r = stream_key(seed, 0x6d6c7062ull, (uint64_t)l, (uint64_t)i);
            float u = (float)(r >> 40) * (1.0f / 16777216.0f);
            h[(size_t)(m->b_off[(size_t)l] + i)] = (2.0f * u - 1.0f) * bound;
        }
    }
    AZD_HIP(hipMemcpy(m->d_params, h.data(), h.size() * 4, hipMemcpyHostToDevice));
    m->p_off.assign((size_t)m->L, 0);
    m->n_packed = 0;
    for (int l = 0; l < m->L; ++l) {
        m->p_off[(size_t)l] = m->n_packed;
        m->n_packed += (int64_t)((m->dims[(size_t)l + 1] + 15) / 16) * ((m->dims[(size_t)l] + 15) / 16) * 256;
    }
    AZD_ST(m->d_wpk.alloc((size_t)m->n_packed + 2048));
    AZD_HIP(hipMemset(m->d_wpk, 0, (size_t)m->n_packed * 4 + 8192));
    {
        size_t big = 0;
        for (int l = 0; l < m->L; ++l) {
            const size_t n = (size_t)m->dims[(size_t)l] * m->dims[(size_t)l + 1];
            big = n > big ? n : big;
        }
        AZD_ST(m->d_split.alloc(big * MlpEvaluator::MAX_SPLITS));
    }
    m->repack(nullptr);
    AZD_HIP(hipDeviceSynchronize());
    return m->ensure_batch(m->max_batch);
}

azd_evaluator *make_mlp_evaluator(int device, int max_batch, int state_dim, int action_dim, const int *hidden, int n_hidden,
                                  int final_act, const azd_adam_config *adam, uint64_t seed, int *status) {
    MlpEvaluator *m = new (std::nothrow) MlpEvaluator();
    if (!m) {
        *status = AZD_ERR_OUT_OF_MEMORY;
        return nullptr;
    }
    m->device = device;
    m->state_dim = state_dim;
    m->action_dim = action_dim;
    m->L = n_hidden + 1;
    m->dims.push_back(state_dim);
    for (int i = 0; i < n_hidden; ++i) m->dims.push_back(hidden[i]);
    m->dims.push_back(action_dim);
    m->final_act = final_act;
    if (const char *env = getenv("AZD_GEMM_SMALL_BELOW")) m->gemm_small_below = atoi(env);
    if (const char *env = getenv("AZD_MLP_FUSE_HIDDEN")) m->fuse_hidden2 = atoi(env) != 0;
    m->adam = *adam;
    m->max_batch = max_batch;
    int64_t off = 0;
    for (int l = 0; l < m->L; ++l) {
        m->w_off.push_back(off);
        off += (int64_t)m->dims[(size_t)l] * m->dims[(size_t)l + 1];
        m->b_off.push_back(off);
        off += m->dims[(size_t)l + 1];
    }
    m->n_params = off;
    int st = mlp_init(m, seed);
    if (st) {
        delete m;
        *status = st;
        return nullptr;
    }
    *status = AZD_OK;
    return m;
}

}

extern "C" int azd_debug_gemm_bf16(int device, int M, int N, int Kp, const void *d_a, const void *d_w, const float *d_bias, void *d_y, int ldy,
                                   int out_bf16, int act, int reps, float *ms) {
    if (M <= 0 || N <= 0 || Kp <= 0 || Kp % 64 != 0 || !d_a || !d_w || !d_y || reps < 1) return AZD_ERR_INVALID_ARGUMENT;
    AZD_HIP(hipSetDevice(device));
    hipDeviceProp_t prop;
    AZD_HIP(hipGetDeviceProperties(&prop, device));
    azd::Stream st;
    AZD_ST(st.create());
    azd::Event e0, e1;
    AZD_ST(e0.create());
    AZD_ST(e1.create());
    const int force_bn = getenv("AZD_GEMM16_BN") ? atoi(getenv("AZD_GEMM16_BN")) : 0;
    azd::launch_gemm16(st, (const uint16_t *)d_a, Kp, (const uint16_t *)d_w, Kp, d_y, ldy, M, N, Kp, act, out_bf16, d_bias, prop.multiProcessorCount, force_bn);
    AZD_HIP(hipEventRecord(e0, st));
    for (int r = 0; r < reps; ++r)
        azd::launch_gemm16(st, (const uint16_t *)d_a, Kp, (const uint16_t *)d_w, Kp, d_y, ldy, M, N, Kp, act, out_bf16, d_bias, prop.multiProcessorCount, force_bn);
    AZD_HIP(hipEventRecord(e1, st));
    AZD_HIP(hipStreamSynchronize(st));
    AZD_HIP(hipGetLastError());
    float t = 0.f;
    AZD_HIP(hipEventElapsedTime(&t, e0, e1));
    if (ms) *ms = t / (float)reps;
    return AZD_OK;
}
```

azdopt_amd/csrc/space_dense.inc:

```

constexpr int DENSE_MAX_N = 64;

template <int KW_>
struct DenseLds {
    uint64_t adj[DENSE_MAX_N];
    double x[DENSE_MAX_N];
    uint64_t slotmask[32];
    uint16_t aid[64 * KW_];
    uint8_t mate[DENSE_MAX_N];
    unsigned long long ctr[NUM_COUNTERS];
    uint16_t seq[4];
    uint32_t stack[PATH_STACK];
};

__device__ __forceinline__ void dense_from_colex(const int pos, int &mx, int &mn) {
    int v = (int)((sqrtf(8.0f * (float)pos + 1.0f) + 1.0f) * 0.5f);
    while (v * (v - 1) / 2 > pos) --v;
    while (v * (v + 1) / 2 <= pos) ++v;
    mx = v;
    mn = pos - v * (v - 1) / 2;
}
__device__ __forceinline__ int dense_colex(const int mx, const int mn) { return mx * (mx - 1) / 2 + mn; }

template <class L>
// ... 359 lines not shown
    }
    __device__ static __forceinline__ uint32_t bit_action(const Lds &s, const uint32_t bit) { return s.aid[bit]; }
    __device__ static __forceinline__ void act(const Arenas &a, Lds &s, const uint32_t, St &st, const uint32_t aid) {
        const uint32_t r = key_bit(s, aid);
        int mx, mn;
        dense_from_colex((int)(aid % (uint32_t)a.E), mx, mn);
        if (LANE == 0) {
            s.adj[mx] ^= 1ull << mn;
            s.adj[mn] ^= 1ull << mx;
        }
#pragma unroll
        for (int w = 0; w < KW; ++w)
            if ((int)(r >> 6) == w) st.rem[w] &= ~(1ull << (r & 63u));
        WAVE_SYNC();
    }
    static constexpr bool EVALUATE_TAKES_HOOK = true;
    __device__ static __forceinline__ float evaluate(const Arenas &a, Lds &s, const uint32_t dyn, St &st, const int t) {
        return evaluate_hooked(a, s, dyn, st, t, DenseNoHook{});
    }
    template <class Hook>
    __device__ static __forceinline__ float evaluate_hooked(const Arenas &a, Lds &s, const uint32_t dyn, St &st, const int t, Hook &&hook) {
        return Cost::evaluate(a, s, st, t, hook);
    }
    __device__ static __forceinline__ void legal_ranks(const Arenas &a, const Lds &s, const St &st, uint64_t (&legal)[KW]) {
#pragma unroll
        for (int w = 0; w < KW; ++w) {
            bool ok = false;
            if ((st.rem[w] >> LANE) & 1ull) {
                const uint32_t aid = s.aid[w * 64 + LANE];
                if (aid < (uint32_t)a.E) ok = true;
                else {
                    int mx, mn;
                    dense_from_colex((int)(aid - (uint32_t)a.E), mx, mn);
                    ok = !dense_is_cut_edge(s, mx, mn);
                }
            }
            legal[w] = __ballot(ok);
        }
    }
    __device__ static __forceinline__ bool terminal(const Arenas &a, Lds &s, const uint32_t, const St &st) {
        uint64_t legal[KW];
        legal_ranks(a, s, st, legal);
        return mask_empty<KW>(legal);
    }
    __device__ static __forceinline__ void open_slots(const Arenas &a, Lds &s, const St &st) {
        if (LANE < 32) s.slotmask[LANE] = 0;
        LDS_SYNC();
#pragma unroll
        for (int w = 0; w < KW; ++w)
            if ((st.rem[w] >> LANE) & 1ull) {
                const uint32_t slot = (uint32_t)s.aid[w * 64 + LANE] % (uint32_t)a.E;
                atomicOr((unsigned long long *)&s.slotmask[slot >> 6], 1ull << (slot & 63u));
            }
        LDS_SYNC();
    }
    __device__ static void write_vec(const Arenas &a, Lds &s, const uint32_t, const St &st, float *row) {
        const int E = a.E;
        open_slots(a, s, st);
        for (int e = LANE; e < E; e += 64) {
            int mx, mn;
            dense_from_colex(e, mx, mn);
            const bool present = (s.adj[mx] >> mn) & 1ull;
            const bool open = (s.slotmask[e >> 6] >> (e & 63)) & 1ull;
            row[e] = present ? 1.0f : 0.0f;
            row[E + e] = (open && !present) ? 1.0f : 0.0f;
            row[2 * E + e] = (open && present) ? 1.0f : 0.0f;
        }
        if (LANE == 0) row[3 * E] = (float)mask_count<KW>(st.rem) / (float)E;
    }
    __device__ static void write_vec16(const Arenas &a, Lds &s, const uint32_t, const St &st, uint16_t *row) {
        const int E = a.E;
        for (int e = LANE; e < E; e += 64) {
            int mx, mn;
            dense_from_colex(e, mx, mn);
            const bool present = (s.adj[mx] >> mn) & 1ull;
            const bool open = (s.slotmask[e >> 6] >> (e & 63)) & 1ull;
            row[e] = present ? (uint16_t)0x3F80u : (uint16_t)0;
            row[E + e] = (open && !present) ? (uint16_t)0x3F80u : (uint16_t)0;
            row[2 * E + e] = (open && present) ? (uint16_t)0x3F80u : (uint16_t)0;
        }
        if (LANE == 0) row[3 * E] = (uint16_t)bf16_bits((float)mask_count<KW>(st.rem) / (float)E);
    }
    static constexpr bool ROWS_DIRECT = true;
    __device__ static void write_rows_direct(const Arenas &a, Lds &s, const uint32_t, const St &st, float *row, uint16_t *row16) {
        const int E = a.E, S = 3 * E + 1;
        open_slots(a, s, st);
        unsigned long long *P = reinterpret_cast<unsigned long long *>(s.x);
        if (LANE < 32) P[LANE] = 0ull;
        LDS_SYNC();
        if (LANE >= 1 && LANE < a.n) {
            const unsigned long long bits = s.adj[LANE] & ((1ull << LANE) - 1ull);
            const int base = LANE * (LANE - 1) / 2, w = base >> 6, sh = base & 63;
            if (bits) {
                atomicOr(&P[w], bits << sh);
                if (sh && (bits >> (64 - sh))) atomicOr(&P[w + 1], bits >> (64 - sh));
            }
        }
        LDS_SYNC();
        const float last = (float)mask_count<KW>(st.rem) / (float)E;
        auto bits8 = [](const unsigned long long *map, const int e) __attribute__((always_inline)) -> uint32_t {
            const int w = e >> 6, sh = e & 63;
            const unsigned long long lo = map[w], hi = map[w + 1];
            return (uint32_t)((sh ? (lo >> sh) | (hi << (64 - sh)) : lo) & 0xFFull);
        };
        auto rule = [](const int sec, const uint32_t pb, const uint32_t ob) __attribute__((always_inline)) -> uint32_t {
            return sec == 0 ? pb : sec == 1 ? (ob & ~pb) : (ob & pb);
        };
        const unsigned long long *O = reinterpret_cast<const unsigned long long *>(s.slotmask);
        const uint32_t p_first = (uint32_t)(P[0] & 0xFFull), o_first = (uint32_t)(O[0] & 0xFFull);
        for (int i0 = 8 * LANE; i0 < S; i0 += 8 * 64) {
            const int sec0 = i0 >= 2 * E ? 2 : i0 >= E ? 1 : 0, e0 = i0 - sec0 * E;
            const int n_in = E - e0 < 8 ? E - e0 : 8;
            const int n_bits = 3 * E - i0 < 8 ? 3 * E - i0 : 8;
            uint32_t b = rule(sec0, bits8(P, e0), bits8(O, e0));
            if (n_in < 8) b = (b & ((1u << n_in) - 1u)) | (rule(sec0 + 1, p_first, o_first) << n_in);
            b &= (1u << n_bits) - 1u;
            if ((S & 3) == 0) {
#pragma unroll
                for (int h = 0; h < 2; ++h)
                    if (i0 + 4 * h < S) {
                        azd_f32x4 w;
#pragma unroll
                        for (int q = 0; q < 4; ++q) w[q] = i0 + 4 * h + q == 3 * E ? last : ((b >> (4 * h + q)) & 1u) ? 1.0f : 0.0f;
                        st_sc1_x4(row + i0 + 4 * h, w);
                    }
            } else if (i0 + 8 <= 3 * E) {
#pragma unroll
                for (int q = 0; q < 8; ++q) st_sc1_f32(row + i0 + q, __uint_as_float(((b >> q) & 1u) * 0x3F800000u));
            } else {
#pragma unroll
                for (int q = 0; q < 8; ++q)
                    if (i0 + q < S) st_sc1_f32(row + i0 + q, i0 + q == 3 * E ? last : ((b >> q) & 1u) ? 1.0f : 0.0f);
            }
            if (row16) {
                azd_f32x4 w;
                uint32_t h[4];
#pragma unroll
                for (int q = 0; q < 4; ++q) h[q] = ((((b >> (2 * q)) & 3u) * 0x8001u) & 0x10001u) * 0x3F80u;
                if (i0 <= 3 * E && 3 * E < i0 + 8) {
                    const int q = 3 * E - i0;
#pragma unroll
                    for (int qq = 0; qq < 4; ++qq)
                        if (qq == (q >> 1)) h[qq] |= bf16_bits(last) << (16 * (q & 1));
                }
                __builtin_memcpy(&w, h, 16);
                st_sc1_x4(reinterpret_cast<float *>(row16 + i0), w);
            }
        }
        LDS_SYNC();
    }

    template <bool SC1 = false>
    __device__ static __forceinline__ void add_actions(const Arenas &a, Lds &s, const int t, const RolloutOut *hint, RolloutOut * ) {
        St st;
        s.adj[LANE] = a.cur_adj[(size_t)t * DENSE_MAX_N + LANE];
        load_tables(a, t, s);
#pragma unroll
        for (int w = 0; w < KW; ++w) st.rem[w] = a.cur_perm[(size_t)t * KW + w];
        WAVE_SYNC();
        uint64_t legal[KW];
        legal_ranks(a, s, st, legal);
        const uint32_t cnt = (uint32_t)mask_count<KW>(legal);
        const uint32_t begin = hint ? hint->n_preds : a.n_preds[t];
        if (!add_actions_fits(a, t, begin, cnt, (uint32_t)MAX_SLOTS)) return;
        const uint32_t node = hint ? hint->pos : a.state_pos[t];
        PredRec *preds = a.preds + (size_t)t * a.pred_cap;
        const float c = hint ? hint->c : a.nodes[(size_t)t * a.node_cap + node].c;
        const uint2 link = node_link(a, t, node);
        const float *h = a.h_theta + (size_t)t * a.A;
        uint32_t aidv[KW];
        float hv[KW];
#pragma unroll
        for (int w = 0; w < KW; ++w) {
            aidv[w] = s.aid[w * 64 + LANE];
            hv[w] = 0.f;
            if ((legal[w] >> LANE) & 1ull) hv[w] = SC1 ? ld_sc1_f32(h + aidv[w]) : h[aidv[w]];
        }
        uint32_t before = 0;
#pragma unroll
        for (int w = 0; w < KW; ++w) {
            if ((legal[w] >> LANE) & 1ull) {
// ... 172 lines not shown
```

azdopt_amd/csrc/space_ops.h:

```cpp
#pragma once
#include "engine_types.h"

namespace azd {

struct PhaseOps {
    void (*init_roots)(const Arenas &a, const uint8_t *d_roots, const uint64_t *d_permitted, void *stream);
    void (*add_actions)(const Arenas &a, int root_mode, void *stream);
    void (*rollout)(const Arenas &a, const TolTable &tol, void *stream);
    void (*argmin)(const Arenas &a, int init_mode, void *stream);
    void (*argmin_log)(const Arenas &a, int n_calls, unsigned long long *log_key, void *stream);
    void (*observe)(const Arenas &a, uint32_t n_obs_tol, void *stream);
    void (*modify_roots)(const Arenas &a, uint64_t seed, uint64_t epoch, uint64_t first_agent, int kmin, int kmax, uint8_t *d_roots,
                         uint64_t *d_perm, uint64_t *d_slots, const RootPolicyArgs &rp, void *stream);
    void (*argmin_one)(const Arenas &a, int agent, uint32_t node, void *stream);
    bool (*persist_plan)(const Arenas &a, const FusedEval &ev, uint32_t *dyn_stride, size_t *dyn_bytes, const char **why);
    void (*launch_persist)(const Arenas &a, const PersistArgs *d_args, const StepLaunch &sl, uint32_t *log_node, uint32_t dyn_stride,
                           size_t dyn_bytes, void *stream);
};
struct AsyncOps {
    bool (*async_plan)(const Arenas &a, const FusedEval &ev, uint32_t *dyn_stride, size_t *dyn_bytes, const char **why);
    void (*launch_async)(const Arenas &a, const PersistArgs *d_args, const StepLaunch &sl, const float *params, const void *wpk,
                         uint32_t dyn_stride, size_t dyn_bytes, void *stream);
};
struct PoolOps {
    bool (*pool_plan)(const Arenas &a, const FusedEval &ev, PoolArgs *pool, uint32_t *dyn_stride, size_t *dyn_bytes, const char **why);
    void (*launch_pool)(const Arenas &a, const PersistArgs *d_args, const StepLaunch &sl, const float *params, const void *wpk,
                        int n_blocks, uint32_t dyn_stride, size_t dyn_bytes, void *stream);
    int (*pool_max_resident)(const Arenas &a, size_t dyn_bytes, int n_cus);
};
struct PoolSearchOps {
    bool (*pool_search_plan)(const Arenas &a, int waves, uint32_t *dyn_stride, size_t *dyn_bytes, const char **why);
    void (*launch_pool_search)(const Arenas &a, const PersistArgs *d_args, const StepLaunch &sl, int n_blocks, int waves, uint32_t dyn_stride,
                               size_t dyn_bytes, void *stream);
    int (*pool_search_resident)(const Arenas &a, int waves, size_t dyn_bytes);
    int waves_max;
};
struct SpaceOps : PhaseOps, AsyncOps, PoolOps, PoolSearchOps {};

const PhaseOps &c21_phase_ops(), &ramsey_phase_ops();
const AsyncOps &c21_async_ops(), &ramsey_async_ops();
const PoolOps &c21_pool_ops(), &ramsey_pool_ops();
const PoolSearchOps &ramsey_pool_search_ops(), &ramsey64_pool_search_ops();
const SpaceOps &ramsey64_big_ops();
const PoolSearchOps &ramsey64_big_pool_search_ops();
const SpaceOps &ramsey64_ops(), &dense_ops(), &dense_ah_ops();
const SpaceOps &dense_ah_wide_ops();
const SpaceOps &dense_inv_ops();
const SpaceOps &dense_inv_wide_ops();
const SpaceOps &dense_invx_ops();
const SpaceOps &dense_invx_wide_ops();
constexpr size_t POOL_SEARCH_STATIC_LDS = 16;

void launch_log_candidates(const Arenas &a, unsigned long long *log_key, uint32_t *call_ctr, void *stream);
void launch_pool_resume_scan(const Arenas &a, const PoolArgs &pool, int n_calls, uint32_t *resume, void *stream);
hipError_t launch_tile_forward(const FusedEval &ev, const PoolArgs &pool, int n_rows, const float *states, float *out, void *stream);
void launch_probe_xcc(uint32_t *d_out, int n_blocks, void *stream);
void launch_hash_predictions(float *d_out, int batch, int action_dim, uint64_t seed, uint64_t first_agent,
                             uint64_t call, void *stream);
void launch_probe_cost(const uint8_t *d_parents, int n, int count, int reps, int full, double *d_lam, int *d_mu,
                       void *stream);
void launch_probe_math(const float *d_in, float *d_out, int n, void *stream);
void launch_probe_dense_cost(const uint64_t *d_adj, int n, int count, const uint16_t *d_toggles, int n_toggles, double *d_lam, int *d_mu,
                             uint8_t *d_mate, int *d_hooks, void *stream);
struct DenseAhCost;
void launch_probe_ah_cost(const uint64_t *d_adj, int n, int count, int reps, DenseAhCost *d_out, void *stream);
void launch_probe_math_f64(const double *d_in, double *d_out, int n, void *stream);
void launch_probe_ah_cost_wide(const uint64_t *d_adj, int n, int count, int reps, DenseAhCost *d_out, void *stream);
struct DenseInvRecipe;
struct DenseInvCost;
void launch_probe_inv_cost(const uint64_t *d_adj, int n, int count, int reps, const DenseInvRecipe *d_recipe, DenseInvCost *d_out, void *stream);
void launch_probe_inv_cost_wide(const uint64_t *d_adj, int n, int count, int reps, const DenseInvRecipe *d_recipe, DenseInvCost *d_out, void *stream);
const SpaceOps &dense_invs_ops();
const SpaceOps &dense_invs_wide_ops();
struct DenseInvxRecipe;
struct DenseInvxCost;
void launch_probe_invx_cost(const uint64_t *d_adj, int n, int count, int reps, const DenseInvxRecipe *d_recipe, DenseInvxCost *d_out, void *stream);
void launch_probe_invx_cost_wide(const uint64_t *d_adj, int n, int count, int reps, const DenseInvxRecipe *d_recipe, DenseInvxCost *d_out, void *stream);
struct DenseInvsRecipe;
struct DenseInvsCost;
void launch_probe_invs_cost(const uint64_t *d_adj, int n, int count, int reps, const DenseInvsRecipe *d_recipe, DenseInvsCost *d_out, void *stream);
void launch_probe_invs_cost_wide(const uint64_t *d_adj, int n, int count, int reps, const DenseInvsRecipe *d_recipe, DenseInvsCost *d_out, void *stream);

void launch_ext_take(const PoolArgs &pool, uint32_t *rows, uint32_t *home, uint32_t *n, unsigned long long *t0, void *stream);
void launch_park(const Arenas &a, const uint32_t *resume, int n_calls, int round, int park, void *stream);
void launch_log_candidates_resume(const Arenas &a, unsigned long long *log_key, const uint32_t *resume, int n_calls, int round, void *stream);
void launch_ext_hash_rows(const PersistArgs *d_args, const uint32_t *rows, const uint32_t *n, uint32_t cap, float *h_theta, void *stream);
void launch_ext_deliver(const PoolArgs &pool, const Arenas &a, const uint32_t *rows, const uint32_t *home, const uint32_t *n, uint32_t cap,
                        const unsigned long long *t0, void *stream);

}
```

azdopt_amd/csrc/tree_core.inc:

```

#define LANE ((int)(threadIdx.x & 63))
#define WAVE_SYNC()                                              \
    do {                                                         \
        __builtin_amdgcn_fence(__ATOMIC_RELEASE, "workgroup");   \
        __builtin_amdgcn_wave_barrier();                         \
        __builtin_amdgcn_fence(__ATOMIC_ACQUIRE, "workgroup");   \
    } while (0)

#ifdef AZD_PHASE_PROFILE
constexpr bool DIAG_PROFILE = true;
#else
constexpr bool DIAG_PROFILE = false;
#endif
#ifdef AZD_WAVE_PHASES
constexpr bool DIAG_WAVE = true;
#else
constexpr bool DIAG_WAVE = false;
#endif
#define PH_NOW() ((DIAG_PROFILE || DIAG_WAVE) ? (unsigned long long)wall_clock64() : 0ull)
#define PROF_NOW() (DIAG_PROFILE ? (unsigned long long)wall_clock64() : 0ull)
#define WAVE_NOW() (DIAG_WAVE ? (unsigned long long)wall_clock64() : 0ull)

#define CTR_ADD(K, V)                                            \
    do {                                                         \
// ... 417 lines not shown
                CTR_ADD(7, n_live);
                uint32_t pnt = live ? r.in_src : NONE, e = live ? r.first_in : NONE;
                if (pnt == NONE && e != NONE) {
                    const ArcRec ar = ag.arcs[e];
                    store_pair(&ag.preds[ar.pp], lw0, lw1);
                    pnt = ar.src;
                    e = ar.next_in;
                }
                const uint64_t ux_mask = __ballot(ux != 0u);
                for (;;) {
                    uint64_t todo = __ballot(pnt != NONE);
                    if (todo == 0ull) break;
                    while (todo) {
                        const int k = first_lane(todo);
                        const uint32_t pk = rdlane(pnt, k);
                        const uint64_t same = __ballot(pnt == pk) & todo;
                        const uint32_t xs = (uint32_t)__popcll(same & ux_mask);
                        int found = -1;
                        for (uint32_t b = 0; b < n_nxt; b += 64) {
                            const uint32_t j = b + (uint32_t)LANE;
                            const bool hit = (j < n_nxt) && (fr_id_at(nxt, b, j) == pk);
                            const uint64_t m = __ballot(hit);
                            if (m) {
                                found = (int)b + first_lane(m);
                                break;
                            }
                        }
                        if (found >= 0) {
                            if (LANE == 0) fr_add_x(nxt, (uint32_t)found, xs);
                        } else {
                            if (n_nxt >= fr_limit) {
                                ag.flags |= FLAG_FRONTIER_CAP;
                                return;
                            }
                            if (LANE == 0) fr_set(nxt, n_nxt, pk, xs);
                            n_nxt += 1;
                        }
                        fr_sync(n_nxt);
                        todo &= ~same;
                    }
                    const bool more = pnt != NONE && e != NONE;
                    if (more) {
                        const ArcRec ar = ag.arcs[e];
                        store_pair(&ag.preds[ar.pp], lw0, lw1);
                        pnt = ar.src;
                        e = ar.next_in;
                    } else pnt = NONE;
                }
            }
            fr_sync(n_nxt);
            cur = nxt;
            n_cur = n_nxt;
        }
        return;
    }
}

template <int KW>
__device__ __forceinline__ uint32_t add_arc(Agent<KW> &ag, uint32_t src, uint32_t dst, uint32_t pp, const uint32_t aid, const float g, bool creating,
                                            const NodeRec &child, const uint32_t child_begin) {
    uint32_t e = ag.n_arcs;
    if (LANE == 0) {
        ArcRec ar;
        ar.src = src;
        ar.dst = dst;
        ar.pp = pp;
        ar.next_in = creating ? NONE : child.first_in;
        ag.arcs[e] = ar;
        if (!creating) ag.nodes[dst].first_in = e;
        PredRec p;
        p.w0 = __float_as_uint(child.c_star);
        p.w1 = summary_w1(child);
        p.w2 = dst | (e << 16);
        p.w3 = aid | (child_begin << 12);
        ag.preds[pp] = p;
        ag.pred_g[pp] = g;
    }
    ag.n_arcs = e + 1;
    return e;
}

struct SpaceDefaults {
    static constexpr int CH = PRED_CHUNKS;
    static constexpr bool ROWS_DIRECT = false, DEFER_ACT = false, TWO_PHASE_LOAD = false, REPLAY_BY_WORD = false, FRONTIER_SPILL = false,
                          EVALUATE_TAKES_HOOK = false, WEIGHTED_ROOTS = false, POOL_EVAL_GROUPS = false;
    template <class... A> __device__ static __forceinline__ void write_vec16(A &&...) {}
    template <class... A> __device__ static __forceinline__ void new_node_begin(A &&...) {}
    template <class... A> __device__ static __forceinline__ void new_node_end(A &&...) {}
    template <class... A> __device__ static __forceinline__ void cache_root(A &&...) {}
    template <class... A> __device__ static __forceinline__ void finish_root(A &&...) {}
    template <class LDS> __device__ static __forceinline__ uint32_t key_bit(const LDS &, const uint32_t aid) { return aid; }
    template <class LDS> __device__ static __forceinline__ uint32_t bit_action(const LDS &, const uint32_t bit) { return bit; }
    __device__ static __forceinline__ int slot_words(const Arenas &a) { return a.KW; }
    __device__ static __forceinline__ float h_sa(float, float, float c_as_star) { return c_as_star; }
    template <class LDS> __device__ static __forceinline__ void prepare(const Arenas &, LDS &) {}
};
template <class SP, class Hook>
__device__ __forceinline__ float space_evaluate(const Arenas &a, typename SP::Lds &s, const uint32_t dyn, typename SP::St &st, const int t, Hook &hook) {
    if constexpr (SP::EVALUATE_TAKES_HOOK) return SP::evaluate_hooked(a, s, dyn, st, t, hook);
    else return SP::evaluate(a, s, dyn, st, t);
}
template <class SP, class... A> __device__ __forceinline__ void space_new_node_begin(A &&...x) { SP::new_node_begin(x...); }
template <class SP, class... A> __device__ __forceinline__ void space_new_node_end(A &&...x) { SP::new_node_end(x...); }

#ifndef AZD_TU_ASYNC
template <class SP>
__global__ __launch_bounds__(64) void k_init_roots(Arenas a, const uint8_t *__restrict__ root_bytes,
                                                   const uint64_t *__restrict__ permitted) {
    constexpr int KW = SP::KW;
    __shared__ typename SP::Lds s;
    const uint32_t dyn = 0;
    const int t = blockIdx.x;
    SP::prepare(a, s);
    WAVE_SYNC();
    typename SP::St st;
    const float c = SP::init_root(a, t, s, dyn, root_bytes, permitted, st);
    uint32_t *ht = a.ht + (size_t)t * a.ht_cap;
    for (uint32_t i = LANE; i < a.ht_cap; i += 64) ht[i] = NONE;
    WAVE_SYNC();
    uint64_t zero[KW];
#pragma unroll
    for (int w = 0; w < KW; ++w) zero[w] = 0;
    if (LANE == 0) {
        NodeRec r;
        r.c = c; r.c_star = c; r.nt_ex = 0; r.act_begin = 0; r.act_end = 0; r.first_in = NONE; r.in_src = NONE; r.in_pp = 0;
        a.nodes[(size_t)t * a.node_cap] = r;
#pragma unroll
        for (int w = 0; w < KW; ++w) {
            a.keys[((size_t)t * a.node_cap) * KW + w] = 0;
            a.cur_path[(size_t)t * KW + w] = 0;
        }
        ht[key_hash<KW>(zero) & (a.ht_cap - 1)] = ht_entry<KW>(zero, 0u);
        a.state_pos[t] = 0;
        a.n_nodes[t] = 1;
        a.n_arcs[t] = 0;
        a.n_preds[t] = 0;
        a.flags[t] = 0;
        a.cand_c[t] = c;
        a.cand_node[t] = 0;
    }
    SP::write_vec(a, s, dyn, st, a.state_vecs + (size_t)t * a.S);
    if (a.state_vecs16) SP::write_vec16(a, s, dyn, st, a.state_vecs16 + (size_t)t * a.S16);
}

#endif
struct RolloutOut {
    uint32_t flags;
    float cand_c;
    uint32_t cand_node;
    uint32_t pos;
    float c;
    uint32_t n_preds;
    uint32_t *post_tail, *post_slots;
    uint32_t post_mask, post_word;
    unsigned long long *post_stamp;
    uint32_t posted;
    uint32_t known_live;
    uint32_t first_nact, first_pp, first_aid;
    float first_g;
};
struct FirstPick {
    uint64_t key;
    uint32_t aid;
    float g;
};
__device__ __forceinline__ void pick_note(FirstPick &f, const float v, const float g, const uint32_t idx, const uint32_t aid) {
    const uint64_t key = ((uint64_t)(~ordf(v)) << 32) | (uint64_t)(0xFFFFFFFFu - idx);
// ... 320 lines not shown
            if (expd[ch] && k_arc[ch] == r_arc) { mine = true; w1 = p[ch].w1; w2 = p[ch].w2; w3 = p[ch].w3; }
        const int src_lane = first_lane(__ballot(mine));
        w1 = rdlane(w1, src_lane);
        w2 = rdlane(w2, src_lane);
        w3 = rdlane(w3, src_lane);
        sel_aid = w3 & 0xFFFu;
        sel_child = w2 & 0xFFFFu;
        next_begin = w3 >> 12;
        next_cnt = (w1 >> 20) & 0x7FFu;
    }
}

template <class LDS>
__device__ __forceinline__ void flush_counters(const Arenas &a, LDS &s, const int t) {
    if (LANE < 24) {
        const int k = LANE;
        const unsigned long long v = s.ctr[k];
        unsigned long long *ctr = a.counters + (size_t)t * NUM_COUNTERS;
        if (k == 10 || k == 11 || k == 21) {
            if (v > ctr[k]) ctr[k] = v;
        } else if (v) ctr[k] += v;
    }
}
template <class SP, bool DEFER = false, bool POOL = false>
__device__ __forceinline__ bool rollout_agent(const Arenas &a, const TolTable &tol, typename SP::Lds &s, const uint32_t dyn, const int t,
                              RolloutOut *out = nullptr) {
    constexpr int KW = SP::KW;
    if (!(POOL && out && out->known_live) && a.flags[t] != 0) {
        if (out) out->flags = 1u;
        return false;
    }
    Agent<KW> ag;
    ag.nodes = a.nodes + (size_t)t * a.node_cap;
    ag.keys = a.keys + (size_t)t * a.node_cap * KW;
    ag.arcs = a.arcs + (size_t)t * a.arc_cap;
    ag.preds = a.preds + (size_t)t * a.pred_cap;
    ag.pred_g = a.pred_g + (size_t)t * a.pred_cap;
    ag.ht = a.ht + (size_t)t * a.ht_cap;
    ag.fr_spill = a.fr_spill + (size_t)t * 4u * a.node_cap;
    const uint32_t nn_v = a.n_nodes[t], na_v = a.n_arcs[t], np_v = a.n_preds[t], cn_v = a.cand_node[t];
    const float cc_v = a.cand_c[t];
    uint64_t path_v[KW];
#pragma unroll
    for (int w = 0; w < KW; ++w) path_v[w] = a.cur_path[(size_t)t * KW + w];
    const uint32_t pos_v = a.state_pos[t];
    const uint32_t stack_v = a.cur_stack[(size_t)t * PATH_STACK + (LANE & (PATH_STACK - 1))];
    typename SP::St st;
    if constexpr (SP::TWO_PHASE_LOAD) {
        typename SP::Raw raw;
        SP::load_issue(a, t, raw);
        __builtin_amdgcn_sched_barrier(0);
        SP::load_finish(s, st, raw);
    } else {
        SP::load_cur(a, t, s, dyn, st);
        SP::cache_root(a, t, s);
    }
    ag.n_nodes = uni(nn_v);
    ag.n_arcs = uni(na_v);
    ag.n_preds = uni(np_v);
    ag.flags = 0;
    ag.cand_c = __uint_as_float(uni(__float_as_uint(cc_v)));
    ag.cand_node = uni(cn_v);
    if (!DEFER && LANE < 24) s.ctr[LANE] = 0;
    uint64_t path[KW];
#pragma unroll
    for (int w = 0; w < KW; ++w) path[w] = uni64(path_v[w]);
    uint32_t pos = uni(pos_v);
    const bool layered = a.layers > 1;
    if (layered) {
        const int d0 = mask_count<KW>(path);
        for (int i = LANE; i < d0; i += 64) s.seq[i] = a.cur_seq[(size_t)t * MAX_NODE_ACTIONS + i];
    }
    {
        const int d0 = mask_count<KW>(path);
        if (LANE < PATH_STACK) s.stack[LANE] = (LANE >= 1 && LANE <= d0) ? stack_v : 0u;
    }
    WAVE_SYNC();

    bool expanded_new = false;
    float new_c = 0.f;
    bool row_out = false;
    auto emit_row = [&]() __attribute__((always_inline)) {
        if constexpr (POOL && SP::ROWS_DIRECT) {
            SP::write_rows_direct(a, s, dyn, st, a.state_vecs + (size_t)t * a.S, a.state_vecs16 ? a.state_vecs16 + (size_t)t * a.S16 : nullptr);
            return;
        }
        float *row = POOL ? SP::row_stage(a, dyn) : a.state_vecs + (size_t)t * a.S;
        if (!layered) {
            SP::write_vec(a, s, dyn, st, row);
            if (!POOL && a.state_vecs16) SP::write_vec16(a, s, dyn, st, a.state_vecs16 + (size_t)t * a.S16);
        } else {
            const int d = mask_count<KW>(path);
            const int len = d + 1 < a.layers ? d + 1 : a.layers;
            const int first = d - len + 1;
            SP::load_root(a, t, s, dyn, st);
            WAVE_SYNC();
            for (int j = 0; j <= d; ++j) {
                if (j >= first) SP::write_vec(a, s, dyn, st, row + (size_t)(j - first) * a.S_inner);
                if (j < d) SP::act(a, s, dyn, st, (uint32_t)s.seq[j]);
            }
        }
        if (POOL) {
            WAVE_SYNC();
            float *dst = a.state_vecs + (size_t)t * a.S;
            if (layered) {
                const int d = mask_count<KW>(path);
                const int len = d + 1 < a.layers ? d + 1 : a.layers;
                for (int q = LANE; q < (len * a.S_inner) >> 2; q += 64) st_sc1_x4(dst + 4 * q, *reinterpret_cast<const azd_f32x4 *>(row + 4 * q));
            } else
                for (int q = LANE; q < a.S >> 2; q += 64) st_sc1_x4(dst + 4 * q, *reinterpret_cast<const azd_f32x4 *>(row + 4 * q));
            WAVE_SYNC();
        }
    };
    uint32_t next_begin = 0, next_cnt = 0;
    bool have_next = false;
    constexpr bool DEFER_ACT = SP::DEFER_ACT;
    const bool defer_act = DEFER_ACT && !layered;
    bool stale = false;
    auto state_now = [&]() __attribute__((always_inline)) {
        if constexpr (DEFER_ACT) {
            if (stale) {
                SP::load_root_cached(a, t, s, dyn, st);
                LDS_SYNC();
                SP::act_set(a, s, dyn, st, path);
                stale = false;
            }
        }
    };
    SelCtr sc;
    sc.visited = 0; sc.selects = 0; sc.deg = 0; sc.actions = 0; sc.pairs = 0;
    const unsigned long long ph_begin = PH_NOW();
    for (uint32_t guard = 0;; ++guard) {
        if (guard > (1u << 22)) {
            ag.flags |= FLAG_LOOP_GUARD;
            break;
        }
        const unsigned long long ph_sel0 = PH_NOW();
        const bool preselected = POOL && guard == 0 && out && out->first_nact != 0;
        uint32_t r_begin = 0, nact = 0;
        bool r_active = false;
        if (preselected) {
        } else if (have_next) {
            r_begin = next_begin;
            nact = next_cnt;
            r_active = true;
        } else {
            const NodeRec rec = uni_rec(ag.nodes[pos]);
            r_begin = rec.act_begin;
            nact = rec.act_end - rec.act_begin;
            r_active = node_active(rec);
        }
        have_next = false;
        const int depth = mask_count<KW>(path);
        const uint32_t tl = depth < tol.n_tol ? tol.tol[depth] : tol.tol_default;
        int kind = 0;
        uint32_t sel_pp = 0, sel_child = 0, sel_aid = 0;
        float sel_g = 0.f;
        if (preselected) {
            sc.selects += 1u;
            sc.actions += out->first_nact;
            kind = 2;
            sel_pp = out->first_pp;
            sel_aid = out->first_aid;
            sel_g = out->first_g;
        } else if (r_active) {
          if constexpr (SP::CH > PRED_CHUNKS) {
// ... 392 lines not shown
```

azdopt_amd/model.py:

```python
import ctypes as C

import numpy as np

from . import _lib


class NablaModel:

    def __init__(self):
        self._h = C.c_void_p()
        self.state_dim = self.action_dim = 0

    def __del__(self):
        if getattr(self, "_h", None) and self._h.value and _lib is not None and getattr(_lib, "lib", None):
            _lib.lib().azd_evaluator_destroy(self._h)
            self._h = C.c_void_p()

    def write_predictions(self, states, predictions):
        states = np.ascontiguousarray(states, np.float32).reshape(-1, self.state_dim)
        assert predictions.dtype == np.float32 and predictions.flags.c_contiguous
        assert predictions.size == states.shape[0] * self.action_dim
        _lib.check(_lib.lib().azd_evaluator_write_predictions(self._h, states.shape[0], _lib.ptr(states),
                                                              _lib.ptr(predictions)), "write_predictions")

    def update_model(self, states, observations, action_weights):
        states = np.ascontiguousarray(states, np.float32).reshape(-1, self.state_dim)
        obs = np.ascontiguousarray(observations, np.float32)
        w = np.ascontiguousarray(action_weights, np.float32)
        loss = C.c_float()
        _lib.check(_lib.lib().azd_evaluator_update_model(self._h, states.shape[0], _lib.ptr(states), _lib.ptr(obs),
                                                         _lib.ptr(w), C.byref(loss)), "update_model")
        return loss.value

    def write_predictions_dev(self, batch, d_states, d_predictions, stream=None):
        _lib.check(_lib.lib().azd_evaluator_write_predictions_dev(self._h, batch, d_states, d_predictions, stream),
                   "write_predictions_dev")

    def update_model_dev(self, batch, d_states, d_observations, d_weights, stream=None):
        loss = C.c_float()
        _lib.check(_lib.lib().azd_evaluator_update_model_dev(self._h, batch, d_states, d_observations, d_weights,
                                                             C.byref(loss), stream), "update_model_dev")
        return loss.value

    def calls(self):
        return _lib.lib().azd_evaluator_calls(self._h)


class TrivialModel(NablaModel):

    def __init__(self, state_dim, action_dim, device=0):
        super().__init__()
        self.state_dim, self.action_dim = state_dim, action_dim
        _lib.check(_lib.lib().azd_evaluator_create_trivial(C.byref(self._h), device, state_dim, action_dim),
                   "azd_evaluator_create_trivial")


class HashStreamModel(NablaModel):

    def __init__(self, state_dim, action_dim, seed, first_agent=0, device=0):
        super().__init__()
        self.state_dim, self.action_dim = state_dim, action_dim
        _lib.check(_lib.lib().azd_evaluator_create_hash_stream(C.byref(self._h), device, state_dim, action_dim, seed,
                                                               first_agent), "azd_evaluator_create_hash_stream")

    def serve_from_pool_evaluators(self, on=True):
        _lib.check(_lib.lib().azd_debug_hash_stream_via_evaluators(self._h, int(on)), "azd_debug_hash_stream_via_evaluators")
        return self


class ActionModel(NablaModel):

    def __init__(self, batch, state_dim, action_dim, hidden=(512, 1024, 512), final_act=_lib.ACT_SIGMOID,
                 lr=1e-4, betas=(0.9, 0.999), eps=1e-8, l2=1e-6, seed=0, device=0, dtype="f32"):
        super().__init__()
        self.state_dim, self.action_dim, self.hidden = state_dim, action_dim, tuple(hidden)
        cfg = _lib.AdamConfig(lr, betas[0], betas[1], eps, l2)
        hid = np.asarray(hidden, np.int32)
        _lib.check(_lib.lib().azd_evaluator_create_mlp(C.byref(self._h), device, batch, state_dim, action_dim,
                                                       _lib.ptr(hid), len(hidden), final_act, C.byref(cfg), seed),
                   "azd_evaluator_create_mlp")
        self.dtype = dtype
        if dtype == "bf16":
            _lib.check(_lib.lib().azd_evaluator_set_weight_storage(self._h, 1), "azd_evaluator_set_weight_storage")
        elif dtype != "f32":
            raise ValueError("dtype must be 'f32' or 'bf16'")

    def num_params(self):
        return _lib.lib().azd_evaluator_num_params(self._h)

    def get_params(self):
        out = np.zeros(self.num_params(), np.float32)
        _lib.check(_lib.lib().azd_evaluator_get_params(self._h, _lib.ptr(out)), "get_params")
        return out

    def debug_gradients(self, states, observations, action_weights):
        states = np.ascontiguousarray(states, np.float32).reshape(-1, self.state_dim)
        obs = np.ascontiguousarray(observations, np.float32)
        w = np.ascontiguousarray(action_weights, np.float32)
        assert obs.size == w.size == states.shape[0] * self.action_dim
        g = np.zeros(self.num_params(), np.float32)
        loss = C.c_float()
        _lib.check(_lib.lib().azd_debug_mlp_gradients(self._h, states.shape[0], _lib.ptr(states), _lib.ptr(obs), _lib.ptr(w),
                                                      _lib.ptr(g), C.byref(loss)), "azd_debug_mlp_gradients")
        return g, loss.value

    def debug_write_predictions_gathered(self, rows, states, predictions, max_rows=None):
        states = np.ascontiguousarray(states, np.float32).reshape(-1, self.state_dim)
        rows = np.ascontiguousarray(rows, np.uint32)
        assert predictions.dtype == np.float32 and predictions.flags.c_contiguous
        assert predictions.size == states.shape[0] * self.action_dim
        _lib.check(_lib.lib().azd_debug_write_predictions_gathered(self._h, states.shape[0] if max_rows is None else max_rows,
                                                                   _lib.ptr(rows) if rows.size else None, rows.size, _lib.ptr(states),
                                                                   states.shape[0], _lib.ptr(predictions)),
                   "azd_debug_write_predictions_gathered")

    def set_params(self, p):
        p = np.ascontiguousarray(p, np.float32)
        assert p.size == self.num_params()
        _lib.check(_lib.lib().azd_evaluator_set_params(self._h, _lib.ptr(p)), "set_params")
```

include/azdopt_amd.h:

```cpp
#ifndef AZDOPT_AMD_H
#define AZDOPT_AMD_H
#include <stdint.h>
#ifdef __cplusplus
extern "C" {
#endif

typedef enum azd_status {
    AZD_OK = 0,
    AZD_ERR_INVALID_ARGUMENT = 1,
    AZD_ERR_NO_DEVICE = 2,
    AZD_ERR_HIP = 3,
    AZD_ERR_CAPACITY = 4,
    AZD_ERR_UNREACHABLE = 5,
    AZD_ERR_NO_EVALUATOR = 6,
    AZD_ERR_OUT_OF_MEMORY = 7,
    AZD_ERR_UNSUPPORTED = 8
} azd_status;

const char *azd_status_string(int status);
const char *azd_last_error(void);
int azd_version(void);
int azd_device_count(void);

#define AZD_SPACE_C21 1
// ... 419 lines not shown
    uint32_t node;
} azd_dense_invx_argmin;
int azd_engine_dense_invx_argmin_data(azd_engine *e, azd_dense_invx_argmin *out);
typedef struct azd_dense_invx_wide_argmin {
    uint64_t adj[64];
    uint64_t permitted[32];
    double inv[AZD_DENSE_INVX_COUNT];
    int32_t dist_k;
    uint32_t computed;
    float cost;
    float eval;
    int32_t agent;
    uint32_t node;
} azd_dense_invx_wide_argmin;
int azd_engine_dense_invx_wide_argmin_data(azd_engine *e, azd_dense_invx_wide_argmin *out);
int azd_engine_dense_invx_agent_cost(azd_engine *e, int agent, azd_dense_invx_cost_t *out);

#define AZD_DENSE_INVS_MAX_N 32
#define AZD_DENSE_INVS_WIDE_MAX_N 64
#define AZD_DENSE_INVS_COUNT 21
#define AZD_DENSE_INVS_ROUNDS 67
#define AZD_DENSE_INVS_NAMES AZD_DENSE_INVX_NAMES, "adj_energy", "dist_energy", "lap_energy", "slap_energy", "adj_spread"
#define AZD_DENSE_INVS_MATRIX_ADJ 0
#define AZD_DENSE_INVS_MATRIX_DIST 1
#define AZD_DENSE_INVS_MATRIX_LAP 2
#define AZD_DENSE_INVS_MATRIX_SLAP 3
typedef struct azd_dense_invs_recipe {
    double weight[AZD_DENSE_INVS_COUNT];
    double bias;
    int adj_index;
    int dist_index;
    int lap_index;
    int slap_index;
    float eval_offset;
    float eval_scale;
    azd_dense_invx_term term[AZD_DENSE_INVX_MAX_TERMS];
    int n_terms;
} azd_dense_invs_recipe;
typedef struct azd_dense_invs_cost_t {
    double inv[AZD_DENSE_INVS_COUNT];
    int dist_k;
    uint32_t computed;
    float cost;
    float eval;
} azd_dense_invs_cost_t;
int azd_dense_invs_cost(const uint64_t *adj, int n, const azd_dense_invs_recipe *recipe, azd_dense_invs_cost_t *out);
int azd_dense_invs_cost_wide(const uint64_t *adj, int n, const azd_dense_invs_recipe *recipe, azd_dense_invs_cost_t *out);
int azd_dense_invs_spectrum(const uint64_t *adj, int n, int which, double *out);
int azd_dense_invs_spectrum_wide(const uint64_t *adj, int n, int which, double *out);
int azd_debug_probe_invs_cost(int device, const uint64_t *adj, int n, int count, int reps, const azd_dense_invs_recipe *recipe,
                              azd_dense_invs_cost_t *out, float *ms);
int azd_debug_probe_invs_cost_wide(int device, const uint64_t *adj, int n, int count, int reps, const azd_dense_invs_recipe *recipe,
                                   azd_dense_invs_cost_t *out, float *ms);
int azd_engine_set_dense_invs_recipe(azd_engine *e, const azd_dense_invs_recipe *recipe);
typedef struct azd_dense_invs_argmin {
    uint64_t adj[32];
    uint64_t permitted[8];
    double inv[AZD_DENSE_INVS_COUNT];
    int32_t dist_k;
    uint32_t computed;
    float cost;
    float eval;
    int32_t agent;
    uint32_t node;
} azd_dense_invs_argmin;
int azd_engine_dense_invs_argmin_data(azd_engine *e, azd_dense_invs_argmin *out);
typedef struct azd_dense_invs_wide_argmin {
    uint64_t adj[64];
    uint64_t permitted[32];
    double inv[AZD_DENSE_INVS_COUNT];
    int32_t dist_k;
    uint32_t computed;
    float cost;
    float eval;
    int32_t agent;
    uint32_t node;
} azd_dense_invs_wide_argmin;
int azd_engine_dense_invs_wide_argmin_data(azd_engine *e, azd_dense_invs_wide_argmin *out);
int azd_engine_dense_invs_agent_cost(azd_engine *e, int agent, azd_dense_invs_cost_t *out);
int azd_debug_probe_math_f64(int device, const double *in, double *out, int n);

int azd_debug_gemm_bf16(int device, int M, int N, int Kp, const void *d_a, const void *d_w, const float *d_bias, void *d_y, int ldy,
                        int out_bf16, int act, int reps, float *ms);

#ifdef __cplusplus
}
#endif
#endif
```

Baseline: 38.80 million.

## Stream dense-graph state rows as packed bits into the bf16 GEMM

In the dense-graph external pool step, searchers now write each state row as a packed bitmask plus one float, instead of full f32/bf16 vectors. A new GEMM kernel gathers these bit rows and expands them to bf16 in LDS using a lookup of fragments. Conversion kernels pack rows before the pool loop and unpack them afterwards, so the rest of the engine still sees full rows. This cuts the bytes written by searchers and read by the evaluator, at the cost of decode work inside the GEMM and two extra conversion launches per call.

```diff
diff --git a/azdopt_amd/__init__.py b/azdopt_amd/__init__.py
--- a/azdopt_amd/__init__.py
+++ b/azdopt_amd/__init__.py
@@ -1,5 +1,5 @@
 from ._lib import ACT_NONE, ACT_RELU, ACT_SIGMOID, AzdError, build, lib
-from .model import ActionModel, HashStreamModel, NablaModel, TrivialModel
+from .model import ActionModel, HashStreamModel, NablaModel, TrivialModel, dense_pack_rows
 from .optimizer import ArgminData, DenseAhArgminData, DenseArgminData, DenseInvArgminData, DenseInvsArgminData, DenseInvxArgminData, NablaOptimizer, RamseyArgminData, TreeView, tree_capacities
 from . import sinks
 from .space import Layered
diff --git a/azdopt_amd/_lib.py b/azdopt_amd/_lib.py
--- a/azdopt_amd/_lib.py
+++ b/azdopt_amd/_lib.py
@@ -298,6 +298,9 @@
     sig("azd_debug_ext_pool_plan", C.c_int, C.POINTER(EngineConfig), i32p, C.POINTER(C.c_size_t))
     sig("azd_debug_mlp_gradients", C.c_int, vp, C.c_int, vp, vp, vp, vp, f32p)
     sig("azd_debug_write_predictions_gathered", C.c_int, vp, C.c_int, vp, C.c_int, vp, C.c_int, vp)
+    sig("azd_dense_bits_pitch", C.c_int, C.c_int)
+    sig("azd_dense_pack_rows", C.c_int, C.c_int, C.c_int, vp, vp)
+    sig("azd_debug_gemm_bf16_bits", C.c_int, vp, C.c_int, C.c_int, vp, C.c_int, vp, C.c_int, vp, vp, vp)
     sig("azd_debug_probe_math", C.c_int, C.c_int, vp, vp, C.c_int)
     sig("azd_debug_gemm_bf16", C.c_int, C.c_int, C.c_int, C.c_int, C.c_int, vp, vp, vp, vp, C.c_int, C.c_int, C.c_int, C.c_int, f32p)
     sig("azd_debug_probe_cost", C.c_int, C.c_int, vp, C.c_int, C.c_int, C.c_int, C.c_int, vp, vp, f32p)
diff --git a/azdopt_amd/csrc/dense_kernels.hip b/azdopt_amd/csrc/dense_kernels.hip
--- a/azdopt_amd/csrc/dense_kernels.hip
+++ b/azdopt_amd/csrc/dense_kernels.hip
@@ -68,6 +68,50 @@
                         const unsigned long long *t0, void *stream) {
     k_ext_deliver<<<dim3((cap + 255) / 256), dim3(256), 0, (hipStream_t)stream>>>(pool, a, rows, home, n, t0);
 }
+__global__ __launch_bounds__(256) void k_dense_bits_from_rows(Arenas a) {
+    const int t = blockIdx.x, lane = threadIdx.x & 63, wave = threadIdx.x >> 6;
+    const int E = a.E, at_last = dense_bits_last(E);
+    const float *row = a.state_vecs + (size_t)t * a.S;
+    uint8_t *out = a.state_bits + (size_t)t * a.SB;
+    for (int w = wave; 8 * w < a.SB; w += 4) {
+        const int i = 64 * w + lane;
+        unsigned long long word = __ballot(i < 3 * E && row[i] != 0.f);
+        if (8 * w <= at_last && at_last < 8 * w + 8) word |= (unsigned long long)__float_as_uint(row[3 * E]) << (8 * (at_last - 8 * w));
+        if (lane == 0) *reinterpret_cast<unsigned long long *>(out + 8 * w) = word;
+    }
+}
+void launch_dense_bits_from_rows(const Arenas &a, void *stream) {
+    k_dense_bits_from_rows<<<dim3(a.B), dim3(256), 0, (hipStream_t)stream>>>(a);
+}
+__global__ __launch_bounds__(256) void k_dense_rows_from_bits(Arenas a) {
+    const int per = a.S16 >> 3;
+    const size_t idx = (size_t)blockIdx.x * blockDim.x + threadIdx.x;
+    if (idx >= (size_t)a.B * per) return;
+    const int t = (int)(idx / per), c = (int)(idx % per), i0 = 8 * c, E = a.E;
+    const uint8_t *in = a.state_bits + (size_t)t * a.SB;
+    const uint32_t b = c < dense_bits_bytes(E) ? in[c] : 0u;
+    const float last = *reinterpret_cast<const float *>(in + dense_bits_last(E));
+    float *row = a.state_vecs + (size_t)t * a.S;
+#pragma unroll
+    for (int q = 0; q < 8; ++q) {
+        if (i0 + q < 3 * E) row[i0 + q] = ((b >> q) & 1u) ? 1.0f : 0.0f;
+        else if (i0 + q == 3 * E) row[i0 + q] = last;
+    }
+    uint32_t h[4];
+#pragma unroll
+    for (int q = 0; q < 4; ++q) h[q] = ((((b >> (2 * q)) & 3u) * 0x8001u) & 0x10001u) * 0x3F80u;
+    if (i0 <= 3 * E && 3 * E < i0 + 8) {
+        const int q = 3 * E - i0;
+#pragma unroll
+        for (int qq = 0; qq < 4; ++qq)
+            if (qq == (q >> 1)) h[qq] |= bf16_bits(last) << (16 * (q & 1));
+    }
+    *reinterpret_cast<uint4 *>(a.state_vecs16 + (size_t)t * a.S16 + i0) = make_uint4(h[0], h[1], h[2], h[3]);
+}
+void launch_dense_rows_from_bits(const Arenas &a, void *stream) {
+    const size_t n = (size_t)a.B * (size_t)(a.S16 >> 3);
+    k_dense_rows_from_bits<<<dim3((unsigned)((n + 255) / 256)), dim3(256), 0, (hipStream_t)stream>>>(a);
+}
 void launch_probe_dense_cost(const uint64_t *d_adj, int n, int count, const uint16_t *d_toggles, int n_toggles, double *d_lam, int *d_mu,
                              uint8_t *d_mate, int *d_hooks, void *stream) {
     k_probe_dense_cost<2><<<dim3(count), dim3(64), 0, (hipStream_t)stream>>>(d_adj, n, count, d_toggles, n_toggles, d_lam, d_mu, d_mate, d_hooks);
diff --git a/azdopt_amd/csrc/engine.hip b/azdopt_amd/csrc/engine.hip
--- a/azdopt_amd/csrc/engine.hip
+++ b/azdopt_amd/csrc/engine.hip
@@ -806,6 +806,16 @@
             a.S16 = ev->input16_pitch();
             AZD_ST(e->alloc(&a.state_vecs16, B * (size_t)a.S16));
             if (hipMemset(a.state_vecs16, 0, B * (size_t)a.S16 * 2) != hipSuccess) return AZD_ERR_HIP;
+            if (const char *v = getenv("AZD_DENSE_PACKED_ROWS")) {
+                if (strcmp(v, "0") != 0 && strcmp(v, "1") != 0) {
+                    azd::g_last_error = "AZD_DENSE_PACKED_ROWS must be 0 or 1 (the dense-graph space's pool step: state rows as bits for the bf16 GEMM stream)";
+                    return AZD_ERR_INVALID_ARGUMENT;
+                }
+                e->ext_bits_on = v[0] == '1';
+            }
+            e->ext_bits_pitch = azd::dense_bits_pitch(a.E);
+            AZD_ST(e->alloc(&e->ext_bits, B * (size_t)e->ext_bits_pitch));
+            if (hipMemset(e->ext_bits, 0, B * (size_t)e->ext_bits_pitch) != hipSuccess) return AZD_ERR_HIP;
         }
     }
     if (ramsey) {
diff --git a/azdopt_amd/csrc/engine_impl.h b/azdopt_amd/csrc/engine_impl.h
--- a/azdopt_amd/csrc/engine_impl.h
+++ b/azdopt_amd/csrc/engine_impl.h
@@ -140,6 +140,9 @@
     const struct ExtPoolForm *ext = nullptr;
     uint16_t *ext_s16 = nullptr;
     int ext_s16_pitch = 0;
+    uint8_t *ext_bits = nullptr;
+    int ext_bits_pitch = 0;
+    bool ext_bits_on = true;
     int kw_host = 0;
     int ramsey_slots = 0;
     int dense_slots = 0;
diff --git a/azdopt_amd/csrc/engine_probes.hip b/azdopt_amd/csrc/engine_probes.hip
--- a/azdopt_amd/csrc/engine_probes.hip
+++ b/azdopt_amd/csrc/engine_probes.hip
@@ -57,6 +57,18 @@
             return AZD_ERR_INVALID_ARGUMENT;
         }
     return ev->debug_write_predictions_gathered(max_rows, rows, n_rows, states, n_state_rows, predictions);
+}
+int azd_debug_gemm_bf16_bits(azd_evaluator *ev, int n, int max_rows, const uint32_t *rows, int n_rows, const float *states, int n_state_rows,
+                             uint16_t *y_bits64, uint16_t *y_bits128, uint16_t *y_ref) {
+    if (!ev || n < 2 || n > 64 || max_rows < 1 || n_rows < 0 || n_rows > max_rows || (n_rows > 0 && !rows) || !states || n_state_rows < 1 || !y_bits64 ||
+        !y_bits128 || !y_ref)
+        return AZD_ERR_INVALID_ARGUMENT;
+    for (int i = 0; i < n_rows; ++i)
+        if (rows[i] >= (uint32_t)n_state_rows) {
+            azd::g_last_error = "azd_debug_gemm_bf16_bits: a row index is not below n_state_rows";
+            return AZD_ERR_INVALID_ARGUMENT;
+        }
+    return ev->debug_gemm_bits(n * (n - 1) / 2, max_rows, rows, n_rows, states, n_state_rows, y_bits64, y_bits128, y_ref);
 }
 int azd_debug_hash_stream_via_evaluators(azd_evaluator *ev, int on) { return ev ? ev->debug_serve_from_pool(on) : AZD_ERR_INVALID_ARGUMENT; }
 int azd_engine_debug_tile_forward(azd_engine *e, const float *states, float *predictions, int rows) {
diff --git a/azdopt_amd/csrc/engine_rollout.hip b/azdopt_amd/csrc/engine_rollout.hip
--- a/azdopt_amd/csrc/engine_rollout.hip
+++ b/azdopt_amd/csrc/engine_rollout.hip
@@ -205,6 +205,7 @@
     azd::FusedEval fe;
     azd::PoolArgs pool;
     bool hashed, f32_rows;
+    bool packed;
     const char *r_needs_rows;
     int waves, n_search, n_ext;
     uint32_t dyn_stride;
@@ -278,7 +279,12 @@
         memset(&fe, 0, sizeof(fe));
         fe.kind = 3;
     }
-    *out = ExtPlan{ax, fe, pool, hashed, f32_rows, r_needs_rows, waves, n_search, n_ext, dyn_stride, dyn_bytes};
+    const bool packed = e->ext_bits && e->ext_bits_on && !hashed && !f32_rows && a.state_vecs16 && e->ev->packed_rows_ok(a.E, e->ext_bits_pitch);
+    if (packed) {
+        ax.state_bits = e->ext_bits;
+        ax.SB = e->ext_bits_pitch;
+    }
+    *out = ExtPlan{ax, fe, pool, hashed, f32_rows, packed, r_needs_rows, waves, n_search, n_ext, dyn_stride, dyn_bytes};
     *runs = true;
     return AZD_OK;
 }
@@ -287,7 +293,8 @@
     if (!xp.hashed) AZD_ST(e->ev->ensure_rows(xp.n_ext * xp.a.B));
     int rounds = knob_int(e->ext->env_rounds, 4);
     rounds = rounds < 1 ? 1 : rounds > 16 ? 16 : rounds;
-    const uint64_t layout = e->ev->layout_version + (xp.hashed ? 1ull << 63 : 0ull) + ((uint64_t)rounds << 56);
+    const uint64_t layout = e->ev->layout_version + (xp.hashed ? 1ull << 63 : 0ull) + (xp.packed ? 1ull << 62 : 0ull) + ((uint64_t)rounds << 56);
+    const azd::PackedRows packed_rows = {xp.a.state_bits, xp.a.SB, xp.a.E};
     if (e->ext_graph_n != xp.n_ext || e->ext_graph_layout != layout) {
         for (azd::GraphExec &g : e->ext_graph) g.reset();
         e->ext_graph_n = 0;
@@ -299,7 +306,8 @@
                     azd::launch_ext_take(xp.pool, rows, home, cnt, e->d_ext_t0 + x, e->ext_stream[x]);
                     if (xp.hashed) azd::launch_ext_hash_rows(e->d_pargs, rows, cnt, (uint32_t)xp.a.B, xp.a.h_theta, e->ext_stream[x]);
                     else {
-                        st_g = xp.a.state_vecs16 ? e->ev->write_predictions_gathered(rows, cnt, xp.a.B, xp.a.state_vecs16, xp.a.S16, xp.a.h_theta, e->ext_stream[x], x * xp.a.B)
+                        st_g = xp.a.state_vecs16 ? e->ev->write_predictions_gathered(rows, cnt, xp.a.B, xp.a.state_vecs16, xp.a.S16, xp.a.h_theta, e->ext_stream[x], x * xp.a.B,
+                                                                                     xp.packed ? &packed_rows : nullptr)
                                               : AZD_ERR_UNSUPPORTED;
                         if (st_g == AZD_ERR_UNSUPPORTED && xp.f32_rows)
                             st_g = e->ev->write_predictions_gathered_f32(rows, cnt, xp.a.B, xp.a.state_vecs, xp.a.S, xp.a.h_theta, e->ext_stream[x], x * xp.a.B);
@@ -380,6 +388,7 @@
         AZD_ST(pool_clear(e, xp.pool));
         AZD_ST(ensure_log_clean(e));
         AZD_HIP(hipMemsetAsync(e->d_ext_n, 0, sizeof(uint32_t) * azd_engine::EXT_STREAMS, e->stream));
+        if (xp.packed) azd::launch_dense_bits_from_rows(xp.a, e->stream);
         AZD_HIP(hipEventRecord(e->ext_fork, e->stream));
         for (int x = 0; x < xp.n_ext; ++x) AZD_HIP(hipStreamWaitEvent(e->ext_stream[x], e->ext_fork, 0));
         const azd::StepLaunch sl = step_launch(e, k, xp.pool.ctl, nullptr, xp.hashed);
@@ -406,6 +415,7 @@
             it += 1;
         }
         for (int x = 0; x < xp.n_ext; ++x) AZD_HIP(hipStreamSynchronize(e->ext_stream[x]));
+        if (xp.packed) azd::launch_dense_rows_from_bits(xp.a, e->stream);
         e->ext_iterations += it;
         if (getenv(xf.env_debug)) fprintf(stderr, "%s: %d calls, %d searcher workgroups, %llu evaluator replays\n", xf.debug_tag, k, xp.n_search, it);
         left -= k;
diff --git a/azdopt_amd/csrc/engine_types.h b/azdopt_amd/csrc/engine_types.h
--- a/azdopt_amd/csrc/engine_types.h
+++ b/azdopt_amd/csrc/engine_types.h
@@ -269,6 +269,15 @@
     int layers, S_inner;
     uint16_t *cur_seq;
     uint32_t *cur_stack;
+    uint8_t *state_bits;
+    int SB;
+};
+constexpr int dense_bits_bytes(int E) { return (3 * E + 7) >> 3; }
+constexpr int dense_bits_last(int E) { return (dense_bits_bytes(E) + 3) & ~3; }
+constexpr int dense_bits_pitch(int E) { return (dense_bits_last(E) + 4 + 15) & ~15; }
+struct PackedRows {
+    const uint8_t *bits;
+    int pitch, E;
 };
 
 constexpr int ROOT_RULE_THRESHOLD = 0, ROOT_RULE_BEST = 1;
diff --git a/azdopt_amd/csrc/evaluator.h b/azdopt_amd/csrc/evaluator.h
--- a/azdopt_amd/csrc/evaluator.h
+++ b/azdopt_amd/csrc/evaluator.h
@@ -33,7 +33,13 @@
     virtual bool rows_concurrent() { return false; }
     virtual int ensure_rows(int ) { return AZD_OK; }
     virtual int write_predictions_gathered(const uint32_t * , const uint32_t * , int , const uint16_t * ,
-                                           int , float * , hipStream_t , int  = 0) {
+                                           int , float * , hipStream_t , int  = 0,
+                                           const azd::PackedRows *  = nullptr) {
+        return AZD_ERR_UNSUPPORTED;
+    }
+    virtual bool packed_rows_ok(int , int ) { return false; }
+    virtual int debug_gemm_bits(int , int , const uint32_t * , int , const float * , int ,
+                                uint16_t * , uint16_t * , uint16_t * ) {
         return AZD_ERR_UNSUPPORTED;
     }
     virtual int write_predictions_gathered_f32(const uint32_t * , const uint32_t * , int , const float * ,
diff --git a/azdopt_amd/csrc/gemm_bf16_bits.inc b/azdopt_amd/csrc/gemm_bf16_bits.inc
--- /dev/null
+++ b/azdopt_amd/csrc/gemm_bf16_bits.inc
@@ -0,0 +1,197 @@
+template <int BN>
+__global__ __launch_bounds__(256, 2) void k_gemm16_bits(const uint8_t *__restrict__ A, const int pitch, const int E, const uint16_t *__restrict__ W, const int ldw,
+                                                        uint16_t *__restrict__ Y, const int ldy, int M, const int N, const int Kp, const float *__restrict__ bias,
+                                                        const uint32_t *__restrict__ m_dev, const uint32_t *__restrict__ rows_in) {
+    if (m_dev) {
+        const int m = (int)*m_dev;
+        M = m < M ? m : M;
+    }
+    if (M <= 0) return;
+    constexpr int NI = BN / 64;
+    constexpr int TILE = BN * G16_BK;
+    __shared__ __attribute__((aligned(1024))) uint16_t lds0[TILE];
+    __shared__ __attribute__((aligned(1024))) uint16_t lds1[TILE];
+    __shared__ float lastv[G16_BM];
+    __shared__ uint4 frag_of[256];
+    extern __shared__ __attribute__((aligned(16))) uint8_t panel[];
+    const int tid = threadIdx.x, lane = tid & 63, wave = tid >> 6;
+    const int wm = wave >> 1, wn = wave & 1;
+    int bm, bn;
+    {
+        const int nbn = (N + BN - 1) / BN, bid = (int)blockIdx.x;
+        const int nwg = ((M + G16_BM - 1) / G16_BM) * nbn;
+        if (bid >= nwg) return;
+        const int q = nwg >> 3, r = nwg & 7, xcd = bid & 7;
+        const int swz = (xcd < r ? xcd * (q + 1) : r * (q + 1) + (xcd - r) * q) + (bid >> 3);
+        const int nbm = (M + G16_BM - 1) / G16_BM, width = 8 * nbn, grp = swz / width, first = grp * 8;
+        const int gsz = nbm - first < 8 ? nbm - first : 8, rem = swz - grp * width;
+        bm = first + rem % gsz;
+        bn = rem / gsz;
+    }
+    const int m0 = bm * G16_BM, n0 = bn * BN;
+    const int sr = lane >> 3, sc = (lane & 7) ^ sr;
+    auto stage = [&](uint16_t *base, const int kt) __attribute__((always_inline)) {
+#pragma unroll
+        for (int q = 0; q < BN / 32; ++q) {
+            const int j = wave + 4 * q;
+            int row = n0 + 8 * j + sr;
+            row = row < N ? row : N - 1;
+            __builtin_amdgcn_global_load_lds((const __attribute__((address_space(1))) void *)(W + (size_t)row * ldw + (size_t)kt * G16_BK + 8 * sc),
+                                             (__attribute__((address_space(3))) void *)(base + j * 512), 16, 0, 0);
+        }
+    };
+    const int nt = Kp / G16_BK;
+    stage(lds0, 0);
+    const int nbytes = dense_bits_bytes(E), at_last = dense_bits_last(E), cpr = pitch >> 4, pieces = G16_BM * cpr;
+    {
+        uint32_t h[4];
+#pragma unroll
+        for (int q = 0; q < 4; ++q) h[q] = (((((uint32_t)tid >> (2 * q)) & 3u) * 0x8001u) & 0x10001u) * 0x3F80u;
+        frag_of[tid] = make_uint4(h[0], h[1], h[2], h[3]);
+    }
+    constexpr int PF = 16;
+    for (int p0 = tid; p0 < pieces; p0 += PF * 256) {
+        uint4 v[PF];
+        int rr[PF], cc[PF];
+#pragma unroll
+        for (int u = 0; u < PF; ++u) {
+            const int p = p0 + 256 * u;
+            rr[u] = p / cpr;
+            cc[u] = p - rr[u] * cpr;
+            if (p < pieces) {
+                int row = m0 + rr[u];
+                row = row < M ? row : M - 1;
+                const size_t src = rows_in ? (size_t)rows_in[row] : (size_t)row;
+                v[u] = *reinterpret_cast<const uint4 *>(A + src * (size_t)pitch + 16 * cc[u]);
+            }
+        }
+#pragma unroll
+        for (int u = 0; u < PF; ++u) {
+            if (p0 + 256 * u >= pieces) continue;
+            uint32_t d[4] = {v[u].x, v[u].y, v[u].z, v[u].w};
+#pragma unroll
+            for (int q = 0; q < 4; ++q) {
+                const int at = 16 * cc[u] + 4 * q;
+                if (at == at_last) lastv[rr[u]] = __uint_as_float(d[q]);
+                if (at >= at_last) d[q] = 0u;
+                else if (at + 4 > nbytes) d[q] &= (1u << (8 * (nbytes - at))) - 1u;
+            }
+            *reinterpret_cast<uint4 *>(panel + (size_t)rr[u] * pitch + 16 * cc[u]) = make_uint4(d[0], d[1], d[2], d[3]);
+        }
+    }
+    asm volatile("s_waitcnt vmcnt(0)" ::: "memory");
+    __syncthreads();
+    f32x16 acc[2][NI];
+#pragma unroll
+    for (int i = 0; i < 2; ++i)
+#pragma unroll
+        for (int j = 0; j < NI; ++j)
+#pragma unroll
+            for (int r = 0; r < 16; ++r) acc[i][j][r] = 0.f;
+    const int fr = lane & 31, fh = lane >> 5;
+    const int k_n = 3 * E, kt_n = k_n >> 6, ks_n = (k_n >> 4) & 3, fh_n = (k_n >> 3) & 1, q_n = k_n & 7;
+    uint32_t num[2];
+    const uint8_t *prow[2];
+#pragma unroll
+    for (int i = 0; i < 2; ++i) {
+        const int R = wm * 64 + i * 32 + fr;
+        prow[i] = panel + (size_t)R * pitch;
+        num[i] = fh == fh_n ? bf16_bits(lastv[R]) << (16 * (q_n & 1)) : 0u;
+    }
+    auto compute = [&](const uint16_t *tb, const int kt) __attribute__((always_inline)) {
+        uint2 ab[2];
+#pragma unroll
+        for (int i = 0; i < 2; ++i) ab[i] = *reinterpret_cast<const uint2 *>(prow[i] + 8 * kt);
+#pragma unroll
+        for (int ks = 0; ks < G16_BK / 16; ++ks) {
+            g16_frag fa[2], fb[NI];
+#pragma unroll
+            for (int i = 0; i < 2; ++i) {
+                const uint32_t b = (((ks < 2 ? ab[i].x : ab[i].y) >> (16 * (ks & 1))) >> (8 * fh)) & 0xFFu;
+                const uint4 f = frag_of[b];
+                uint32_t h[4] = {f.x, f.y, f.z, f.w};
+                if (kt == kt_n && ks == ks_n) {
+#pragma unroll
+                    for (int q = 0; q < 4; ++q)
+                        if (q == (q_n >> 1)) h[q] |= num[i];
+                }
+                __builtin_memcpy(&fa[i], h, 16);
+            }
+#pragma unroll
+            for (int j = 0; j < NI; ++j) {
+                const int R = wn * (BN / 2) + j * 32 + fr;
+                const uint4 v = *reinterpret_cast<const uint4 *>(tb + R * G16_BK + 8 * ((2 * ks + fh) ^ (R & 7)));
+                __builtin_memcpy(&fb[j], &v, 16);
+            }
+            __builtin_amdgcn_s_setprio(1);
+#pragma unroll
+            for (int i = 0; i < 2; ++i)
+#pragma unroll
+                for (int j = 0; j < NI; ++j) acc[i][j] = __builtin_amdgcn_mfma_f32_32x32x16_bf16(fa[i], fb[j], acc[i][j], 0, 0, 0);
+            __builtin_amdgcn_s_setprio(0);
+        }
+    };
+    for (int kt = 0; kt < nt; kt += 2) {
+        if (kt + 1 < nt) stage(lds1, kt + 1);
+        compute(lds0, kt);
+        asm volatile("s_waitcnt vmcnt(0)" ::: "memory");
+        __syncthreads();
+        if (kt + 1 >= nt) break;
+        if (kt + 2 < nt) stage(lds0, kt + 2);
+        compute(lds1, kt + 1);
+        asm volatile("s_waitcnt vmcnt(0)" ::: "memory");
+        __syncthreads();
+    }
+#pragma unroll
+    for (int j = 0; j < NI; ++j) {
+        const int col = n0 + wn * (BN / 2) + j * 32 + (lane & 31);
+        if (col >= N) continue;
+        const float bj = bias ? bias[col] : 0.f;
+#pragma unroll
+        for (int i = 0; i < 2; ++i)
+#pragma unroll
+            for (int r = 0; r < 16; ++r) {
+                const int row = m0 + wm * 64 + i * 32 + (r & 3) + 8 * (r >> 2) + 4 * (lane >> 5);
+                if (row < M) {
+                    float v = acc[i][j][r] + bj;
+                    v = v > 0.f ? v : 0.f;
+                    Y[(size_t)row * ldy + col] = (uint16_t)bf16_bits(v);
+                }
+            }
+    }
+}
+static int gemm16_bits_bn() {
+    if (const char *env = getenv("AZD_GEMM16_BITS_BN")) {
+        const int k = atoi(env);
+        if (k == 64 || k == 128) return k;
+    }
+    return 64;
+}
+constexpr int DENSE_BITS_MAX_PITCH = dense_bits_pitch(2016);
+static bool gemm16_bits_prepare(int pitch) {
+    if (pitch < 16 || pitch % 16 != 0 || pitch > DENSE_BITS_MAX_PITCH) return false;
+    const int dyn = G16_BM * DENSE_BITS_MAX_PITCH;
+    return hipFuncSetAttribute((const void *)k_gemm16_bits<64>, hipFuncAttributeMaxDynamicSharedMemorySize, dyn) == hipSuccess &&
+           hipFuncSetAttribute((const void *)k_gemm16_bits<128>, hipFuncAttributeMaxDynamicSharedMemorySize, dyn) == hipSuccess;
+}
+static bool launch_gemm16_bits(hipStream_t st, const uint8_t *A, int pitch, int E, const uint16_t *W, int ldw, uint16_t *Y, int ldy, int max_rows, int N, int Kp,
+                               const float *bias, const uint32_t *m_dev, const uint32_t *rows_in, int bn = 0) {
+    if (pitch != dense_bits_pitch(E) || pitch > DENSE_BITS_MAX_PITCH || Kp % G16_BK != 0 || Kp / 8 > pitch || Kp <= 3 * E || max_rows < 1 || N < 1) return false;
+    if (!bn) bn = gemm16_bits_bn();
+    const size_t dyn = (size_t)G16_BM * (size_t)pitch;
+    const unsigned blocks = (unsigned)(((max_rows + G16_BM - 1) / G16_BM) * ((N + bn - 1) / bn));
+    if (bn == 128) k_gemm16_bits<128><<<dim3(blocks), dim3(256), dyn, st>>>(A, pitch, E, W, ldw, Y, ldy, max_rows, N, Kp, bias, m_dev, rows_in);
+    else k_gemm16_bits<64><<<dim3(blocks), dim3(256), dyn, st>>>(A, pitch, E, W, ldw, Y, ldy, max_rows, N, Kp, bias, m_dev, rows_in);
+    return true;
+}
+static void dense_pack_rows(int E, int n_rows, const float *rows, uint8_t *out) {
+    const int S = 3 * E + 1, pitch = dense_bits_pitch(E), at_last = dense_bits_last(E);
+    for (int r = 0; r < n_rows; ++r) {
+        const float *x = rows + (size_t)r * S;
+        uint8_t *o = out + (size_t)r * pitch;
+        memset(o, 0, (size_t)pitch);
+        for (int i = 0; i < 3 * E; ++i)
+            if (x[i] != 0.f) o[i >> 3] |= (uint8_t)(1u << (i & 7));
+        memcpy(o + at_last, x + 3 * E, 4);
+    }
+}
diff --git a/azdopt_amd/csrc/mlp_kernels.hip b/azdopt_amd/csrc/mlp_kernels.hip
--- a/azdopt_amd/csrc/mlp_kernels.hip
+++ b/azdopt_amd/csrc/mlp_kernels.hip
@@ -236,6 +236,7 @@
 
 #include "gemm_bf16_glds.inc"
 #include "gemm_bf16_hidden2.inc"
+#include "gemm_bf16_bits.inc"
 #include "gemm_f32_gathered.inc"
 
 __global__ void k_quantize_bf16(const float *__restrict__ p, size_t n, uint16_t *__restrict__ w16, float *__restrict__ q) {
@@ -553,13 +554,22 @@
         return ensure_batch(rows);
     }
     int write_predictions_gathered(const uint32_t *d_rows, const uint32_t *d_count, int max_rows, const uint16_t *d_s16, int pitch16, float *d_p,
-                                   hipStream_t st, int act_row0) override {
+                                   hipStream_t st, int act_row0, const PackedRows *packed) override {
         if (!rows_concurrent() || !d_s16 || pitch16 != kp[0]) return AZD_ERR_UNSUPPORTED;
+        if (packed && !packed_fits(packed->E, packed->pitch)) return AZD_ERR_UNSUPPORTED;
         if (act_row0 + max_rows > cap_batch) return AZD_ERR_CAPACITY;
         AZD_HIP(hipSetDevice(device));
         const uint16_t *x16 = d_s16;
         for (int l = 0; l < L; ++l) {
             const bool last = l == L - 1;
+            if (l == 0 && packed) {
+                uint16_t *y = d_act16[1] + (size_t)act_row0 * kp[1];
+                if (!launch_gemm16_bits(st, packed->bits, packed->pitch, packed->E, d_w16p + wp_off[0], kp[0], y, kp[1], max_rows, dims[1], kp[0],
+                                        d_params + b_off[0], d_count, d_rows))
+                    return AZD_ERR_HIP;
+                x16 = y;
+                continue;
+            }
             if (hidden_pair(l)) {
                 uint16_t *y2 = d_act16[(size_t)l + 2] + (size_t)act_row0 * HF_H;
                 launch_hidden2<true>(st, x16, HF_H, d_w16p + wp_off[(size_t)l], d_w16p + wp_off[(size_t)l + 1], HF_H, d_params + b_off[(size_t)l],
@@ -577,6 +587,52 @@
         }
         AZD_HIP(hipGetLastError());
         return AZD_OK;
+    }
+
+    bool packed_fits(int E, int pitch) const {
+        return E >= 1 && L >= 2 && dims[0] == 3 * E + 1 && pitch == dense_bits_pitch(E) && kp[0] / 8 <= pitch && gemm16_ksplit(dims[1], kp[0]) == 1;
+    }
+    bool packed_rows_ok(int E, int pitch) override {
+        if (!rows_concurrent() || !packed_fits(E, pitch) || hipSetDevice(device) != hipSuccess) return false;
+        return gemm16_bits_prepare(pitch);
+    }
+    int debug_gemm_bits(int E, int max_rows, const uint32_t *rows, int n_rows, const float *states, int n_state_rows, uint16_t *y_bits64, uint16_t *y_bits128,
+                        uint16_t *y_ref) override {
+        AZD_HIP(hipSetDevice(device));
+        const int pitch = dense_bits_pitch(E);
+        if (!bf16 || !d_w16p || !packed_rows_ok(E, pitch)) return AZD_ERR_UNSUPPORTED;
+        std::vector<uint8_t> packed_h((size_t)n_state_rows * pitch);
+        dense_pack_rows(E, n_state_rows, states, packed_h.data());
+        const uint8_t *packed = packed_h.data();
+        const int N = dims[1];
+        DevBuf<float> d_s;
+        DevBuf<uint32_t> d_r;
+        DevBuf<uint16_t> d_s16, d_y;
+        DevBuf<uint8_t> d_b;
+        const size_t ny = (size_t)max_rows * kp[1];
+        AZD_ST(alloc_set(d_s, (size_t)n_state_rows * dims[0], d_r, (size_t)max_rows + 1, d_s16, (size_t)n_state_rows * kp[0], d_y, 3 * ny, d_b,
+                         (size_t)n_state_rows * pitch));
+        const uint32_t count = (uint32_t)n_rows;
+        hipError_t he = hipMemcpy(d_s, states, (size_t)n_state_rows * dims[0] * 4, hipMemcpyHostToDevice);
+        if (he == hipSuccess) he = hipMemcpy(d_b, packed, (size_t)n_state_rows * pitch, hipMemcpyHostToDevice);
+        if (he == hipSuccess && n_rows > 0) he = hipMemcpy(d_r, rows, (size_t)n_rows * 4, hipMemcpyHostToDevice);
+        if (he == hipSuccess) he = hipMemcpy(d_r + max_rows, &count, 4, hipMemcpyHostToDevice);
+        if (he == hipSuccess) he = hipMemset(d_y, 0, 3 * ny * 2);
+        if (he != hipSuccess) return hip_fail(he, "azd_debug_gemm_bf16_bits: staging");
+        const size_t n = (size_t)n_state_rows * (kp[0] / 4);
+        k_rows_to_bf16<<<(unsigned)((n + 255) / 256), 256, 0, nullptr>>>(d_s, dims[0], n_state_rows, dims[0], d_s16, kp[0]);
+        for (int v = 0; v < 2; ++v)
+            if (!launch_gemm16_bits(nullptr, d_b, pitch, E, d_w16p + wp_off[0], kp[0], d_y + v * ny, kp[1], max_rows, N, kp[0], d_params + b_off[0], d_r + max_rows,
+                                    d_r, v == 0 ? 64 : 128))
+                return AZD_ERR_HIP;
+        launch_gemm16_ext(nullptr, d_s16, kp[0], d_w16p + wp_off[0], kp[0], d_y + 2 * ny, kp[1], max_rows, N, kp[0], AZD_ACT_RELU, 1, d_params + b_off[0], n_cus,
+                          d_r + max_rows, d_r, nullptr);
+        he = hipDeviceSynchronize();
+        if (he == hipSuccess) he = hipGetLastError();
+        uint16_t *outs[3] = {y_bits64, y_bits128, y_ref};
+        for (int v = 0; v < 3 && he == hipSuccess; ++v)
+            he = hipMemcpy2D(outs[v], (size_t)N * 2, d_y + v * ny, (size_t)kp[1] * 2, (size_t)N * 2, (size_t)max_rows, hipMemcpyDeviceToHost);
+        return he == hipSuccess ? AZD_OK : hip_fail(he, "azd_debug_gemm_bf16_bits");
     }
 
     int write_predictions_gathered_f32(const uint32_t *d_rows, const uint32_t *d_count, int max_rows, const float *d_s, int pitch, float *d_p,
@@ -619,7 +675,7 @@
             const size_t n = (size_t)n_state_rows * (kp[0] / 4);
             k_rows_to_bf16<<<(unsigned)((n + 255) / 256), 256, 0, nullptr>>>(d_s, dims[0], n_state_rows, dims[0], d_s16, kp[0]);
         }
-        s = bf16 ? write_predictions_gathered(d_r, d_r + max_rows, max_rows, d_s16, kp[0], d_p, nullptr, 0)
+        s = bf16 ? write_predictions_gathered(d_r, d_r + max_rows, max_rows, d_s16, kp[0], d_p, nullptr, 0, nullptr)
                  : write_predictions_gathered_f32(d_r, d_r + max_rows, max_rows, d_s, dims[0], d_p, nullptr, 0);
         if (s == AZD_OK) {
             he = hipDeviceSynchronize();
@@ -876,6 +932,13 @@
 
 }
 
+extern "C" int azd_dense_bits_pitch(int n) { return (n < 2 || n > 64) ? 0 : azd::dense_bits_pitch(n * (n - 1) / 2); }
+extern "C" int azd_dense_pack_rows(int n, int n_rows, const float *rows, uint8_t *out) {
+    if (n < 2 || n > 64 || n_rows < 0 || (n_rows > 0 && (!rows || !out))) return AZD_ERR_INVALID_ARGUMENT;
+    azd::dense_pack_rows(n * (n - 1) / 2, n_rows, rows, out);
+    return AZD_OK;
+}
+
 extern "C" int azd_debug_gemm_bf16(int device, int M, int N, int Kp, const void *d_a, const void *d_w, const float *d_bias, void *d_y, int ldy,
                                    int out_bf16, int act, int reps, float *ms) {
     if (M <= 0 || N <= 0 || Kp <= 0 || Kp % 64 != 0 || !d_a || !d_w || !d_y || reps < 1) return AZD_ERR_INVALID_ARGUMENT;
diff --git a/azdopt_amd/csrc/space_dense.inc b/azdopt_amd/csrc/space_dense.inc
--- a/azdopt_amd/csrc/space_dense.inc
+++ b/azdopt_amd/csrc/space_dense.inc
@@ -465,8 +465,7 @@
         if (LANE == 0) row[3 * E] = (uint16_t)bf16_bits((float)mask_count<KW>(st.rem) / (float)E);
     }
     static constexpr bool ROWS_DIRECT = true;
-    __device__ static void write_rows_direct(const Arenas &a, Lds &s, const uint32_t, const St &st, float *row, uint16_t *row16) {
-        const int E = a.E, S = 3 * E + 1;
+    __device__ static __forceinline__ unsigned long long *row_bitmaps(const Arenas &a, Lds &s, const St &st) {
         open_slots(a, s, st);
         unsigned long long *P = reinterpret_cast<unsigned long long *>(s.x);
         if (LANE < 32) P[LANE] = 0ull;
@@ -480,6 +479,54 @@
             }
         }
         LDS_SYNC();
+        return P;
+    }
+    static constexpr bool ROWS_BITS = true;
+    __device__ static void write_row_bits(const Arenas &a, Lds &s, const uint32_t, const St &st, uint8_t *bits) {
+        const int E = a.E;
+        const unsigned long long *P = row_bitmaps(a, s, st);
+        const unsigned long long *O = reinterpret_cast<const unsigned long long *>(s.slotmask);
+        const float last = (float)mask_count<KW>(st.rem) / (float)E;
+        auto bits64 = [](const unsigned long long *map, const int e) __attribute__((always_inline)) -> unsigned long long {
+            const int w = e >> 6, sh = e & 63;
+            const unsigned long long lo = map[w], hi = map[w + 1];
+            return sh ? (lo >> sh) | (hi << (64 - sh)) : lo;
+        };
+        auto word = [&](const int i) __attribute__((always_inline)) -> unsigned long long {
+            unsigned long long w = 0ull;
+            int sec = i >= 2 * E ? 2 : i >= E ? 1 : 0, e = i - sec * E, filled = 0;
+            if (i >= 3 * E) return w;
+            while (filled < 64 && sec < 3) {
+                const int n = E - e < 64 - filled ? E - e : 64 - filled;
+                const unsigned long long p = bits64(P, e), o = bits64(O, e);
+                unsigned long long b = sec == 0 ? p : sec == 1 ? (o & ~p) : (o & p);
+                if (n < 64) b &= (1ull << n) - 1ull;
+                w |= b << filled;
+                filled += n;
+                e += n;
+                if (e == E) {
+                    sec += 1;
+                    e = 0;
+                }
+            }
+            return w;
+        };
+        const int at_last = dense_bits_last(E);
+        for (int c = LANE; 16 * c < a.SB; c += 64) {
+            const unsigned long long w0 = word(128 * c), w1 = word(128 * c + 64);
+            uint32_t h[4] = {(uint32_t)w0, (uint32_t)(w0 >> 32), (uint32_t)w1, (uint32_t)(w1 >> 32)};
+#pragma unroll
+            for (int q = 0; q < 4; ++q)
+                if (16 * c + 4 * q == at_last) h[q] = __float_as_uint(last);
+            azd_f32x4 v;
+            __builtin_memcpy(&v, h, 16);
+            st_sc1_x4(reinterpret_cast<float *>(bits + 16 * c), v);
+        }
+        LDS_SYNC();
+    }
+    __device__ static void write_rows_direct(const Arenas &a, Lds &s, const uint32_t, const St &st, float *row, uint16_t *row16) {
+        const int E = a.E, S = 3 * E + 1;
+        unsigned long long *P = row_bitmaps(a, s, st);
         const float last = (float)mask_count<KW>(st.rem) / (float)E;
         auto bits8 = [](const unsigned long long *map, const int e) __attribute__((always_inline)) -> uint32_t {
             const int w = e >> 6, sh = e & 63;
diff --git a/azdopt_amd/csrc/space_ops.h b/azdopt_amd/csrc/space_ops.h
--- a/azdopt_amd/csrc/space_ops.h
+++ b/azdopt_amd/csrc/space_ops.h
@@ -87,5 +87,7 @@
 void launch_ext_hash_rows(const PersistArgs *d_args, const uint32_t *rows, const uint32_t *n, uint32_t cap, float *h_theta, void *stream);
 void launch_ext_deliver(const PoolArgs &pool, const Arenas &a, const uint32_t *rows, const uint32_t *home, const uint32_t *n, uint32_t cap,
                         const unsigned long long *t0, void *stream);
+void launch_dense_bits_from_rows(const Arenas &a, void *stream);
+void launch_dense_rows_from_bits(const Arenas &a, void *stream);
 
 }
diff --git a/azdopt_amd/csrc/tree_core.inc b/azdopt_amd/csrc/tree_core.inc
--- a/azdopt_amd/csrc/tree_core.inc
+++ b/azdopt_amd/csrc/tree_core.inc
@@ -523,7 +523,7 @@
 
 struct SpaceDefaults {
     static constexpr int CH = PRED_CHUNKS;
-    static constexpr bool ROWS_DIRECT = false, DEFER_ACT = false, TWO_PHASE_LOAD = false, REPLAY_BY_WORD = false, FRONTIER_SPILL = false,
+    static constexpr bool ROWS_DIRECT = false, ROWS_BITS = false, DEFER_ACT = false, TWO_PHASE_LOAD = false, REPLAY_BY_WORD = false, FRONTIER_SPILL = false,
                           EVALUATE_TAKES_HOOK = false, WEIGHTED_ROOTS = false, POOL_EVAL_GROUPS = false;
     template <class... A> __device__ static __forceinline__ void write_vec16(A &&...) {}
     template <class... A> __device__ static __forceinline__ void new_node_begin(A &&...) {}
@@ -1010,6 +1010,12 @@
     bool row_out = false;
     auto emit_row = [&]() __attribute__((always_inline)) {
         if constexpr (POOL && SP::ROWS_DIRECT) {
+            if constexpr (SP::ROWS_BITS) {
+                if (a.state_bits) {
+                    SP::write_row_bits(a, s, dyn, st, a.state_bits + (size_t)t * a.SB);
+                    return;
+                }
+            }
             SP::write_rows_direct(a, s, dyn, st, a.state_vecs + (size_t)t * a.S, a.state_vecs16 ? a.state_vecs16 + (size_t)t * a.S16 : nullptr);
             return;
         }
diff --git a/azdopt_amd/model.py b/azdopt_amd/model.py
--- a/azdopt_amd/model.py
+++ b/azdopt_amd/model.py
@@ -44,6 +44,18 @@
 
     def calls(self):
         return _lib.lib().azd_evaluator_calls(self._h)
+
+
+def dense_pack_rows(n, states):
+    E = n * (n - 1) // 2
+    states = np.ascontiguousarray(states, np.float32).reshape(-1, 3 * E + 1)
+    pitch = _lib.lib().azd_dense_bits_pitch(n)
+    if pitch <= 0:
+        raise ValueError("dense_pack_rows: n must be 2..64")
+    out = np.zeros((states.shape[0], pitch), np.uint8)
+    _lib.check(_lib.lib().azd_dense_pack_rows(n, states.shape[0], _lib.ptr(states) if states.size else None, _lib.ptr(out) if out.size else None),
+               "azd_dense_pack_rows")
+    return out
 
 
 class TrivialModel(NablaModel):
@@ -114,6 +126,16 @@
                                                                    states.shape[0], _lib.ptr(predictions)),
                    "azd_debug_write_predictions_gathered")
 
+    def debug_gemm_bf16_bits(self, n, rows, states, max_rows=None):
+        states = np.ascontiguousarray(states, np.float32).reshape(-1, self.state_dim)
+        rows = np.ascontiguousarray(rows, np.uint32)
+        max_rows = states.shape[0] if max_rows is None else max_rows
+        outs = [np.zeros((max_rows, self.hidden[0]), np.uint16) for _ in range(3)]
+        _lib.check(_lib.lib().azd_debug_gemm_bf16_bits(self._h, n, max_rows, _lib.ptr(rows) if rows.size else None, rows.size, _lib.ptr(states),
+                                                       states.shape[0], _lib.ptr(outs[0]), _lib.ptr(outs[1]), _lib.ptr(outs[2])),
+                   "azd_debug_gemm_bf16_bits")
+        return outs
+
     def set_params(self, p):
         p = np.ascontiguousarray(p, np.float32)
         assert p.size == self.num_params()
diff --git a/include/azdopt_amd.h b/include/azdopt_amd.h
--- a/include/azdopt_amd.h
+++ b/include/azdopt_amd.h
@@ -525,6 +525,10 @@
 
 int azd_debug_gemm_bf16(int device, int M, int N, int Kp, const void *d_a, const void *d_w, const float *d_bias, void *d_y, int ldy,
                         int out_bf16, int act, int reps, float *ms);
+int azd_dense_bits_pitch(int n);
+int azd_dense_pack_rows(int n, int n_rows, const float *rows, uint8_t *out);
+int azd_debug_gemm_bf16_bits(azd_evaluator *ev, int n, int max_rows, const uint32_t *rows, int n_rows, const float *states, int n_state_rows,
+                             uint16_t *y_bits64, uint16_t *y_bits128, uint16_t *y_ref);
 
 #ifdef __cplusplus
 }
```

After: 38.50 million. About the same (-0.8%).
